# PhilipWilliamVentura/multimodal-financial-analysis-tool-using-paligemma

Hardware: AMD Instinct MI355X
Metric: decode tokens/sec per GPU + prefill ms (224px img + 32-tok prompt), PaliGemma-3B (higher is better)
Workload: dtype bf16; 1 GPU; configs[1]: paligemma-3b-pt-224 greedy KV-cached decode, batch 1, after a 256-image-token + 32-text-token prefill; batch_per_gpu=1, global_batch=1, prompt_len=288, images_gathered=1, parallelism=replicas x1 (weights RCCL-broadcast), hipgraph=True, steps_per_graph_launch=1

## Files before the change

### include/pgmi.h

```cpp
#ifndef PGMI_H
#define PGMI_H

#include <stddef.h>
#include <stdint.h>

#ifdef __cplusplus
extern "C" {
#endif

#define PGMI_OK 0
#define PGMI_E_ARG -1
#define PGMI_E_STATE -2
#define PGMI_E_HIP -3
#define PGMI_E_NOMEM -4

#define PGMI_DTYPE_BF16 0
#define PGMI_DTYPE_F16 1
#define PGMI_DTYPE_F32 2

typedef struct pgmi_ctx pgmi_ctx;

typedef struct pgmi_config {
    int v_hidden, v_intermediate, v_layers, v_heads, v_channels, v_image, v_patch;
    float v_ln_eps;
    int t_vocab, t_hidden, t_intermediate, t_layers, t_heads, t_kv_heads, t_head_dim, t_max_pos;
    float t_rms_eps, t_rope_theta;
    int projection_dim;
    int64_t image_token_index;
    int64_t pad_token_id;
    int max_batch;
    int max_seq;
    int max_kv;
} pgmi_config;

const char* pgmi_last_error(void);
const char* pgmi_version(void);

int pgmi_create(int device, const pgmi_config* cfg, pgmi_ctx** out);
int pgmi_destroy(pgmi_ctx* ctx);

int64_t pgmi_weights_bytes(const pgmi_ctx* ctx);
int pgmi_weight_count(const pgmi_ctx* ctx);
int pgmi_weight_info(const pgmi_ctx* ctx, int idx, const char** name, int64_t* offset_bytes, int64_t* shape4,
                     int* ndim);
int pgmi_bind_weights(pgmi_ctx* ctx, void* dev_slab);
int pgmi_load_weight(pgmi_ctx* ctx, const char* name, const void* src, int src_dtype, int src_on_device,
                     void* stream);
int pgmi_load_safetensors(pgmi_ctx* ctx, const char* path, int* n_loaded, int* n_skipped, void* stream);
int pgmi_safetensors_count(const char* path, int* n);
int pgmi_safetensors_entry(const char* path, int i, char* name, int name_cap, int* dtype, int64_t* shape4, int* ndim,
                           int64_t* begin, int64_t* end);
int pgmi_fill_synthetic(pgmi_ctx* ctx, const char* name, uint64_t key, float scale, float offset, void* stream);
uint64_t pgmi_synthetic_key(const char* name, uint64_t seed);
int pgmi_set_rope_inv_freq(pgmi_ctx* ctx, const float* inv_freq);
int pgmi_set_rope_table(pgmi_ctx* ctx, const uint16_t* cos_tab, const uint16_t* sin_tab, int max_pos);
int pgmi_prepare(pgmi_ctx* ctx);

int64_t pgmi_kv_bytes(const pgmi_ctx* ctx, int batch, int max_tokens);

int pgmi_vision(pgmi_ctx* ctx, const void* pixels, int pixel_dtype, int B, void* feats, void* stream);
int pgmi_project(pgmi_ctx* ctx, const void* feats, int rows, void* out, void* stream);
int pgmi_embed(pgmi_ctx* ctx, const int64_t* ids, int rows, void* out, void* stream);
int pgmi_lm_forward(pgmi_ctx* ctx, const int64_t* ids, const void* image_feats, int n_img_rows, const void* embeds,
                    int B, int L, const int64_t* positions, void* kv, int kv_batch, int kv_max, int kv_start,
                    float* logits, int logits_rows, void* stream);
int pgmi_decode(pgmi_ctx* ctx, const int64_t* ids, int B, void* kv, int kv_batch, int kv_max, int kv_len,
                int position, float* logits, int64_t* next_ids, int use_graph, void* stream);
int pgmi_decode_steps(pgmi_ctx* ctx, int64_t* ids, int B, void* kv, int kv_batch, int kv_max, int kv_len,
                      int position, int n_steps, float* logits, int64_t* tokens, int use_graph, void* stream);
int pgmi_lm_forward_ragged(pgmi_ctx* ctx, const int64_t* ids, const void* image_feats, int n_img_rows,
                           const void* embeds, int B, int L, const int64_t* positions, const int32_t* lens, void* kv,
                           int kv_batch, int kv_max, int kv_start, float* logits, int logits_rows, void* stream);
int pgmi_decode_ragged(pgmi_ctx* ctx, const int64_t* ids, int B, void* kv, int kv_batch, int kv_max,
                       const int32_t* kv_lens, const int32_t* positions, int n_steps, float* logits, int64_t* next_ids,
                       int64_t* tokens, int use_graph, void* stream);
int pgmi_decode_embeds(pgmi_ctx* ctx, const void* embeds, int B, void* kv, int kv_batch, int kv_max, int kv_len,
                       int position, float* logits, int64_t* next_ids, int use_graph, void* stream);
int pgmi_decode_embeds_dev(pgmi_ctx* ctx, const void* embeds, int B, void* kv, int kv_batch, int kv_max, int kv_len,
                           const void* position, int position_dtype, const void* mask, int mask_dtype,
                           int64_t mask_b_stride, float* logits, int64_t* next_ids, int use_graph, void* stream);
int pgmi_set_prefill_graph(pgmi_ctx* ctx, int on);
#define PGMI_GRAPH_CACHE_MAX 64
int pgmi_graph_count(const pgmi_ctx* ctx, int which);
int pgmi_set_decode_staged_norm(pgmi_ctx* ctx, int on);
int pgmi_lm_head(pgmi_ctx* ctx, const void* normed, int rows, float* logits, void* stream);
int pgmi_lm_logprobs(pgmi_ctx* ctx, const void* normed, int rows, const int64_t* labels, int64_t ignore_index,
                     float* logprob, float* lse, void* stream);
int pgmi_logprobs(pgmi_ctx* ctx, const float* logits, int rows, int V, const int64_t* ids, int64_t ignore_index,
                  float* logprob, float* lse, void* stream);
int pgmi_lm_final_hidden(pgmi_ctx* ctx, void* out, int rows, void* stream);

#define PGMI_COMM_ID_BYTES 128
int pgmi_comm_unique_id(void* id_out);
int pgmi_comm_init(int device, int nranks, int rank, const void* id, void** comm_out);
int pgmi_comm_destroy(void* comm);
int pgmi_broadcast_weights(pgmi_ctx* ctx, void* comm, int root, void* stream);

int pgmi_argmax(pgmi_ctx* ctx, const float* logits, int rows, int V, int64_t* out, void* stream);

int pgmi_eos_update(pgmi_ctx* ctx, int64_t* next_ids, int32_t* finished, int B, int64_t eos_id, int64_t pad_id,
                    int32_t* n_alive, void* stream);

int pgmi_decode_kernel(pgmi_ctx* ctx, int which, int layer, int B, void* stream);

int pgmi_preprocess(pgmi_ctx* ctx, const void* src_hwc, int H, int W, int out_h, int out_w, float* out_chw,
                    void* stream);

int pgmi_prefill_kernel(pgmi_ctx* ctx, int which, int layer, int rows, void* stream);

int pgmi_prefill_probe(pgmi_ctx* ctx, int on);
int pgmi_prefill_probe_times(pgmi_ctx* ctx, float* us, int n);
int pgmi_tune_gemm(int cfg, int split);
int pgmi_tune_gemm_shape(int M, int N, int K, int dual, int cfg, int split);

int pgmi_debug_gemm_tiles(int n_mt, int n_nt, int S, int BM, int BN, int K, int* mt, int* nt, int* z);
int pgmi_debug_gemm_plan(int M, int N, int K, int dual, int* cfg, int* bm, int* bn, int* split);

int pgmi_tune_attention(int variant);

int pgmi_sample_top_p(pgmi_ctx* ctx, const float* x, int rows, int V, float temperature, float top_p,
                      const float* u, int64_t* out, float* kept_mass, void* stream);

int pgmi_op_gemm(pgmi_ctx* ctx, const void* A, const void* W, int M, int N, int K, int epi, const void* bias,
                 const void* res, void* out, void* stream);
int pgmi_op_lm_logprobs(pgmi_ctx* ctx, const void* normed, const void* W, int rows, int V, int K,
                        const int64_t* labels, int64_t ignore_index, float* logprob, float* lse, void* stream);
int pgmi_op_gemm_strided(pgmi_ctx* ctx, const void* A, int lda, const void* W, int ldw, int M, int N, int K, int epi,
                         const void* bias, const void* res, void* out, void* stream);
int pgmi_op_rmsnorm(pgmi_ctx* ctx, const void* x, const void* w, int rows, int D, float eps, void* out,
                    void* stream);
int pgmi_op_layernorm(pgmi_ctx* ctx, const void* x, const void* w, const void* b, int rows, int D, float eps,
                      void* out, void* stream);
int pgmi_op_add(pgmi_ctx* ctx, const void* a, const void* b, int64_t n, void* out, void* stream);
int pgmi_op_patch_embed(pgmi_ctx* ctx, const void* pixels, int pixel_dtype, int B, int C, int H, int P,
                        const void* conv_w, const void* conv_b, const void* pos, int D, void* out, void* stream);
int pgmi_op_attention(pgmi_ctx* ctx, const void* q, const void* k, const void* v, void* o, int B, int Lq, int Lk,
                      int H, int Hkv, int head_dim, float scale, void* stream);
int pgmi_op_attention_ex(pgmi_ctx* ctx, const void* q, const void* k, const void* v, void* o, int B, int Lq, int Lk,
                         int H, int Hkv, int head_dim, int kv_layout, float scale, int scale_div, const void* mask,
                         int mask_dtype, int64_t m_b_stride, int64_t m_h_stride, int64_t m_q_stride, void* probs,
                         void* stream);
int pgmi_op_rope(pgmi_ctx* ctx, const void* x, const void* cos_rows, const void* sin_rows, int64_t rows, int heads,
                 int head_dim, void* out, void* stream);
int pgmi_op_scale(pgmi_ctx* ctx, const void* x, float a, int64_t n, void* out, void* stream);
int pgmi_op_gemv_res(pgmi_ctx* ctx, const void* x, const void* W, int B, int N, int K, void* h_inout,
                     void* stream);

#ifdef __cplusplus
}
#endif
#endif
```

### multimodal-financial-analysis-tool-using-paligemma_amd/csrc/engine.hip

```cpp
#include <algorithm>
#include <cmath>
#include <cstdio>
#include <cstdlib>
#include <cstring>
#include <map>
#include <string>
#include <unordered_map>
#include <vector>

#include <dlfcn.h>

#include <rccl/rccl.h>

#include "../../include/pgmi.h"
#include "common.h"
#include "launch.h"
#include "safetensors_hdr.h"

using namespace pgmi;

static thread_local std::string g_err;

constexpr int kPrefillGroup = 8;

static int fail(int code, const std::string& msg) {
    g_err = msg;
    return code;
}

#define HIPCHK(expr)                                                                       \
    do {                                                                                   \
        hipError_t e_ = (expr);                                                            \
        if (e_ != hipSuccess) return fail(PGMI_E_HIP, std::string(#expr) + ": " + hipGetErrorString(e_)); \
    } while (0)

static int launcher_error() {
    const char* what = "";
    const hipError_t e = pgmi::launch_error_take(&what);
    if (e == hipSuccess) return 0;
    return fail(PGMI_E_HIP, std::string("kernel launch: ") + what + ": " + hipGetErrorString(e));
}

#define LAUNCHCHK()                                                                        \
    do {                                                                                   \
        if (int r_ = launcher_error()) return r_;                                          \
        hipError_t e_ = hipGetLastError();                                                 \
        if (e_ != hipSuccess) return fail(PGMI_E_HIP, std::string("kernel launch: ") + hipGetErrorString(e_)); \
    } while (0)

struct Slot {
    std::string name;
    int64_t off;
    int64_t shape[4];
    int ndim;
    int64_t numel;
};

struct GraphCache {
    std::map<std::vector<intptr_t>, hipGraphExec_t> map;
    void clear() {
        for (auto& kv : map)
            if (kv.second) (void)hipGraphExecDestroy(kv.second);
        map.clear();
    }
};

struct VisionLayerW {
    const uint16_t *qkv_w, *qkv_b, *out_w, *out_b, *ln1_w, *ln1_b, *fc1_w, *fc1_b, *fc2_w, *fc2_b, *ln2_w, *ln2_b;
};
struct TextLayerW {
    const uint16_t *qkv, *o, *gate_up, *down, *in_norm, *post_norm;
    const uint16_t *mf_gate_up = nullptr, *mf_qkv = nullptr, *mf_o = nullptr, *mf_down = nullptr;
};
struct WeightTable {
    const uint16_t *patch_conv_w, *patch_b, *pos_emb, *post_ln_w, *post_ln_b, *proj_w, *proj_b, *embed, *final_norm;
    std::vector<VisionLayerW> v;
    std::vector<TextLayerW> t;
};

struct pgmi_ctx {
    pgmi_config c;
    int device;
    std::vector<Slot> slots;
    std::unordered_map<std::string, int> index;
    int64_t slab_bytes = 0;
    uint8_t* slab = nullptr;
    WeightTable w;
    std::vector<float> inv_freq;
    std::vector<uint16_t> host_cos, host_sin;
    bool prepared = false;
    std::vector<void*> allocs;
    uint16_t* patch_w = nullptr;
    int kpad = 0;
    uint16_t* cosT = nullptr;
    uint16_t* sinT = nullptr;
    uint16_t *Hs, *Tn, *QKV, *Qr, *AO, *ACT, *lastrows;
    long tn_rows = 0;
    int64_t* dpos;
    int64_t* dids_tmp;
    uint16_t *vX, *vT, *vQKV, *vAO, *vH, *vP;
    float* ws;
    size_t ws_bytes;
    uint16_t *dH, *dQ, *dAO, *dACT;
    uint16_t* dHn;
    float* dSS;
    uint16_t* mfw = nullptr;
    bool mfw_dirty = false;
    float *opart, *pmax, *dlogits, *amax_v;
    int *pidx, *amax_i;
    int max_chunks;
    StepState* step;
    StepState* pstep;
    StepState* rstep;
    int* d_rlens;
    int64_t* d_ids;
    uint16_t* d_emb;
    float* d_mask;
    float* d_zero;
    int64_t* d_next;
    unsigned* lm_done;
    hipStream_t cap_stream = nullptr;
    GraphCache pgraphs, dgraphs;
    bool prefill_graph = true;
    int mf_staged = -1;
    bool step_known = false;
    int step_kv = 0, step_pos = 0;
    bool rstep_known = false;
    int rstep_B = 0;
    int rstep_kv[kMaxRows] = {0}, rstep_pos[kMaxRows] = {0};
    std::vector<hipEvent_t> probe_ev;
    bool probe_on = false;
    bool graph_before_probe = true;
};

namespace {

int n_img(const pgmi_config& c) { return (c.v_image / c.v_patch) * (c.v_image / c.v_patch); }

void add_slot(pgmi_ctx* x, const std::string& name, std::initializer_list<int64_t> shape) {
    Slot s;
    s.name = name;
    s.ndim = (int)shape.size();
    s.numel = 1;
    int i = 0;
    for (int64_t d : shape) { s.shape[i++] = d; s.numel *= d; }
    for (; i < 4; ++i) s.shape[i] = 1;
    s.off = x->slab_bytes;
    x->slab_bytes += (s.numel * 2 + 255) / 256 * 256;
    x->index[name] = (int)x->slots.size();
    x->slots.push_back(s);
}

void build_layout(pgmi_ctx* x) {
    const pgmi_config& c = x->c;
    const int64_t D = c.v_hidden, I = c.v_intermediate, P = c.v_patch, C = c.v_channels, N = n_img(c);
    const std::string vp = "vision_tower.vision_model.";
    add_slot(x, vp + "embeddings.patch_embedding.weight", {D, C, P, P});
    add_slot(x, vp + "embeddings.patch_embedding.bias", {D});
    add_slot(x, vp + "embeddings.position_embedding.weight", {N, D});
    for (int i = 0; i < c.v_layers; ++i) {
        const std::string lp = vp + "encoder.layers." + std::to_string(i) + ".";
        for (const char* nm : {"q_proj", "k_proj", "v_proj"}) add_slot(x, lp + "self_attn." + nm + ".weight", {D, D});
        for (const char* nm : {"q_proj", "k_proj", "v_proj"}) add_slot(x, lp + "self_attn." + nm + ".bias", {D});
        add_slot(x, lp + "self_attn.out_proj.weight", {D, D});
        add_slot(x, lp + "self_attn.out_proj.bias", {D});
        add_slot(x, lp + "layer_norm1.weight", {D});
        add_slot(x, lp + "layer_norm1.bias", {D});
        add_slot(x, lp + "mlp.fc1.weight", {I, D});
        add_slot(x, lp + "mlp.fc1.bias", {I});
        add_slot(x, lp + "mlp.fc2.weight", {D, I});
        add_slot(x, lp + "mlp.fc2.bias", {D});
        add_slot(x, lp + "layer_norm2.weight", {D});
        add_slot(x, lp + "layer_norm2.bias", {D});
    }
    add_slot(x, vp + "post_layernorm.weight", {D});
    add_slot(x, vp + "post_layernorm.bias", {D});
    add_slot(x, "multi_modal_projector.linear.weight", {c.projection_dim, D});
    add_slot(x, "multi_modal_projector.linear.bias", {c.projection_dim});
    const int64_t H = c.t_hidden, TI = c.t_intermediate, V = c.t_vocab, HD = c.t_head_dim;
    add_slot(x, "language_model.model.embed_tokens.weight", {V, H});
    for (int i = 0; i < c.t_layers; ++i) {
        const std::string lp = "language_model.model.layers." + std::to_string(i) + ".";
        add_slot(x, lp + "self_attn.q_proj.weight", {c.t_heads * HD, H});
        add_slot(x, lp + "self_attn.k_proj.weight", {c.t_kv_heads * HD, H});
        add_slot(x, lp + "self_attn.v_proj.weight", {c.t_kv_heads * HD, H});
        add_slot(x, lp + "self_attn.o_proj.weight", {H, c.t_heads * HD});
        add_slot(x, lp + "mlp.gate_proj.weight", {TI, H});
        add_slot(x, lp + "mlp.up_proj.weight", {TI, H});
        add_slot(x, lp + "mlp.down_proj.weight", {H, TI});
        add_slot(x, lp + "input_layernorm.weight", {H});
        add_slot(x, lp + "post_attention_layernorm.weight", {H});
    }
    add_slot(x, "language_model.model.norm.weight", {H});
}

int bind_tables(pgmi_ctx* x) {
    std::string missing;
    auto W = [&](const std::string& name) -> const uint16_t* {
        auto it = x->index.find(name);
        if (it == x->index.end()) {
            if (missing.empty()) missing = name;
            return nullptr;
        }
        return reinterpret_cast<const uint16_t*>(x->slab + x->slots[it->second].off);
    };
    WeightTable& w = x->w;
    const std::string vp = "vision_tower.vision_model.", tp = "language_model.model.";
    w.patch_conv_w = W(vp + "embeddings.patch_embedding.weight");
    w.patch_b = W(vp + "embeddings.patch_embedding.bias");
    w.pos_emb = W(vp + "embeddings.position_embedding.weight");
    w.post_ln_w = W(vp + "post_layernorm.weight");
    w.post_ln_b = W(vp + "post_layernorm.bias");
    w.proj_w = W("multi_modal_projector.linear.weight");
    w.proj_b = W("multi_modal_projector.linear.bias");
    w.embed = W(tp + "embed_tokens.weight");
    w.final_norm = W(tp + "norm.weight");
    w.v.resize(x->c.v_layers);
    for (int i = 0; i < x->c.v_layers; ++i) {
        const std::string lp = vp + "encoder.layers." + std::to_string(i) + ".";
        w.v[i] = {W(lp + "self_attn.q_proj.weight"), W(lp + "self_attn.q_proj.bias"),
                  W(lp + "self_attn.out_proj.weight"), W(lp + "self_attn.out_proj.bias"),
                  W(lp + "layer_norm1.weight"), W(lp + "layer_norm1.bias"), W(lp + "mlp.fc1.weight"),
                  W(lp + "mlp.fc1.bias"), W(lp + "mlp.fc2.weight"), W(lp + "mlp.fc2.bias"),
                  W(lp + "layer_norm2.weight"), W(lp + "layer_norm2.bias")};
    }
    w.t.resize(x->c.t_layers);
    for (int i = 0; i < x->c.t_layers; ++i) {
        const std::string lp = tp + "layers." + std::to_string(i) + ".";
        TextLayerW& t = w.t[i];
        t.qkv = W(lp + "self_attn.q_proj.weight");
        t.o = W(lp + "self_attn.o_proj.weight");
        t.gate_up = W(lp + "mlp.gate_proj.weight");
        t.down = W(lp + "mlp.down_proj.weight");
        t.in_norm = W(lp + "input_layernorm.weight");
        t.post_norm = W(lp + "post_attention_layernorm.weight");
    }
    if (!missing.empty()) return fail(PGMI_E_STATE, "weight layout has no tensor named " + missing);
    return 0;
}

uint16_t host_f2bf(float f) {
    uint32_t u;
    std::memcpy(&u, &f, 4);
    u += 0x7FFFu + ((u >> 16) & 1u);
    return (uint16_t)(u >> 16);
}

float bf16_round_host(float f) {
    uint32_t u = (uint32_t)host_f2bf(f) << 16;
    float r;
    std::memcpy(&r, &u, 4);
    return r;
}

uint64_t fnv1a(const char* s) {
    uint64_t h = 0xCBF29CE484222325ULL;
    for (const unsigned char* p = (const unsigned char*)s; *p; ++p) { h ^= *p; h *= 0x100000001B3ULL; }
    return h;
}

uint64_t splitmix64_h(uint64_t x) {
    x += 0x9E3779B97F4A7C15ULL;
    x = (x ^ (x >> 30)) * 0xBF58476D1CE4E5B9ULL;
    x = (x ^ (x >> 27)) * 0x94D049BB133111EBULL;
    return x ^ (x >> 31);
}

__global__ void k_convert(const void* src, int dtype, long n, uint16_t* dst) {
    for (long i = blockIdx.x * (long)blockDim.x + threadIdx.x; i < n; i += (long)gridDim.x * blockDim.x) {
        if (dtype == PGMI_DTYPE_F32) dst[i] = f2bf(reinterpret_cast<const float*>(src)[i]);
        else dst[i] = f2bf((float)reinterpret_cast<const _Float16*>(src)[i]);
    }
}

int dalloc(pgmi_ctx* x, void** p, size_t bytes) {
    if (bytes == 0) bytes = 256;
    hipError_t e = hipMalloc(p, bytes);
    if (e != hipSuccess) return fail(PGMI_E_NOMEM, std::string("hipMalloc ") + std::to_string(bytes) + ": " + hipGetErrorString(e));
    x->allocs.push_back(*p);
    return 0;
}

template <typename T>
int dalloc_t(pgmi_ctx* x, T** p, size_t count) {
    return dalloc(x, reinterpret_cast<void**>(p), count * sizeof(T));
}

void build_rope_host(pgmi_ctx* x, std::vector<uint16_t>& cs, std::vector<uint16_t>& sn) {
    const int half = x->c.t_head_dim / 2, mp = x->c.t_max_pos;
    cs.resize((size_t)mp * half);
    sn.resize((size_t)mp * half);
    for (int p = 0; p < mp; ++p)
        for (int i = 0; i < half; ++i) {
            const float ang = (float)p * x->inv_freq[i];
            cs[(size_t)p * half + i] = host_f2bf((float)std::cos((double)ang));
            sn[(size_t)p * half + i] = host_f2bf((float)std::sin((double)ang));
        }
}

int ensure_prepared(pgmi_ctx* x) {
    (void)pgmi::launch_error_take(nullptr);
    if (!x->prepared) return fail(PGMI_E_STATE, "pgmi_prepare() has not been called");
    if (!x->slab) return fail(PGMI_E_STATE, "weights are not bound (pgmi_bind_weights)");
    return 0;
}

template <class F>
int run_graphed(pgmi_ctx* x, GraphCache& gc, hipStream_t s, const std::vector<intptr_t>& key, F body,
                bool sync_before_capture) {
    auto it = gc.map.find(key);
    if (it == gc.map.end()) {
        if (gc.map.size() >= PGMI_GRAPH_CACHE_MAX) gc.clear();
        gc.map[key] = nullptr;
        return body(s);
    }
    if (it->second) {
        HIPCHK(hipGraphLaunch(it->second, s));
        return 0;
    }
    hipGraph_t g = nullptr;
    hipGraphExec_t exec = nullptr;
    int rc = 0;
    hipError_t e = sync_before_capture ? hipStreamSynchronize(s) : hipSuccess;
    if (e == hipSuccess && (e = hipStreamBeginCapture(x->cap_stream, hipStreamCaptureModeThreadLocal)) == hipSuccess) {
        rc = body(x->cap_stream);
        const hipError_t end = hipStreamEndCapture(x->cap_stream, &g);
        if (rc == 0) e = end;
    }
    if (rc == 0 && e == hipSuccess) e = hipGraphInstantiate(&exec, g, nullptr, nullptr, 0);
    if (g) (void)hipGraphDestroy(g);
    if (rc == 0 && e == hipSuccess) e = hipGraphLaunch(exec, s);
    if (rc == 0 && e == hipSuccess) {
        gc.map[key] = exec;
        return 0;
    }
    if (exec) (void)hipGraphExecDestroy(exec);
    gc.map.erase(key);
    return rc ? rc : fail(PGMI_E_HIP, std::string("hipGraph capture: ") + hipGetErrorString(e));
}

template <class F>
int run_prefill(pgmi_ctx* x, hipStream_t s, const std::vector<intptr_t>& key, F body) {
    if (!x->prefill_graph) return body(s);
    return run_graphed(x, x->pgraphs, s, key, body, false);
}

}

namespace {
struct Rccl {
    void* h = nullptr;
    std::string why;
    ncclResult_t (*get_unique_id)(ncclUniqueId*) = nullptr;
    ncclResult_t (*comm_init_rank)(ncclComm_t*, int, ncclUniqueId, int) = nullptr;
    ncclResult_t (*comm_destroy)(ncclComm_t) = nullptr;
    ncclResult_t (*broadcast)(const void*, void*, size_t, ncclDataType_t, int, ncclComm_t, hipStream_t) = nullptr;
    const char* (*error_string)(ncclResult_t) = nullptr;
};

Rccl& rccl() {
    static Rccl r = [] {
        Rccl t;
        for (const char* n : {"librccl.so.1", "librccl.so", "/opt/rocm/lib/librccl.so.1"}) {
            if ((t.h = dlopen(n, RTLD_NOW | RTLD_LOCAL))) break;
            const char* e = dlerror();
            if (e) t.why = e;
        }
        if (t.h) {
            t.get_unique_id = reinterpret_cast<decltype(t.get_unique_id)>(dlsym(t.h, "ncclGetUniqueId"));
            t.comm_init_rank = reinterpret_cast<decltype(t.comm_init_rank)>(dlsym(t.h, "ncclCommInitRank"));
            t.comm_destroy = reinterpret_cast<decltype(t.comm_destroy)>(dlsym(t.h, "ncclCommDestroy"));
            t.broadcast = reinterpret_cast<decltype(t.broadcast)>(dlsym(t.h, "ncclBroadcast"));
            t.error_string = reinterpret_cast<decltype(t.error_string)>(dlsym(t.h, "ncclGetErrorString"));
        }
        return t;
    }();
    return r;
}
}

extern "C" {

const char* pgmi_last_error(void) { return g_err.c_str(); }
const char* pgmi_version(void) { return "pgmi 0.1.0 (gfx950)"; }

int pgmi_create(int device, const pgmi_config* cfg, pgmi_ctx** out) {
    if (!cfg || !out) return fail(PGMI_E_ARG, "null argument");
    const pgmi_config& c = *cfg;
    if (c.t_head_dim != 256) return fail(PGMI_E_ARG, "head_dim must be 256 (Gemma)");
    if (c.t_hidden != 2048) return fail(PGMI_E_ARG, "text hidden must be 2048 (decode kernels are specialised)");
    if (c.t_intermediate % 8 != 0 || c.v_intermediate % 8 != 0) return fail(PGMI_E_ARG, "intermediate sizes must be multiples of 8");
    if (c.v_hidden % c.v_heads != 0 || c.v_hidden / c.v_heads != 72) return fail(PGMI_E_ARG, "SigLIP head_dim must be 72");
    if (c.t_kv_heads != 1 || c.t_heads > 8)
        return fail(PGMI_E_ARG, "decode path is specialised for MQA with <= 8 query heads (num_key_value_heads = 1)");
    if (c.max_batch < 1 || c.max_batch > kMaxRows) return fail(PGMI_E_ARG, "max_batch must be in [1, 16]");
    if (c.v_hidden > 4096) return fail(PGMI_E_ARG, "v_hidden too large for the LayerNorm kernel");
    auto* x = new pgmi_ctx();
    x->c = c;
    if (x->c.max_kv <= 0) x->c.max_kv = c.t_max_pos;
    x->device = device;
    build_layout(x);
    x->inv_freq.resize(c.t_head_dim / 2);
    for (int i = 0; i < c.t_head_dim / 2; ++i) {
        const float e = (float)(2 * i) / (float)c.t_head_dim;
        const float p = (float)std::pow((double)c.t_rope_theta, (double)e);
        x->inv_freq[i] = 1.0f / p;
    }
    *out = x;
    return 0;
}

int pgmi_destroy(pgmi_ctx* x) {
    if (!x) return 0;
    for (auto& e : x->probe_ev) (void)hipEventDestroy(e);
    x->dgraphs.clear();
    x->pgraphs.clear();
    for (void* p : x->allocs) (void)hipFree(p);
    if (x->cap_stream) (void)hipStreamDestroy(x->cap_stream);
    delete x;
    return 0;
}

int64_t pgmi_weights_bytes(const pgmi_ctx* x) { return x ? x->slab_bytes : -1; }
int pgmi_weight_count(const pgmi_ctx* x) { return x ? (int)x->slots.size() : -1; }

int pgmi_weight_info(const pgmi_ctx* x, int idx, const char** name, int64_t* off, int64_t* shape4, int* ndim) {
    if (!x || idx < 0 || idx >= (int)x->slots.size()) return fail(PGMI_E_ARG, "weight index out of range");
    const Slot& s = x->slots[idx];
    if (name) *name = s.name.c_str();
    if (off) *off = s.off;
    if (shape4) for (int i = 0; i < 4; ++i) shape4[i] = s.shape[i];
    if (ndim) *ndim = s.ndim;
    return 0;
}

int pgmi_bind_weights(pgmi_ctx* x, void* slab) {
    if (!x || !slab) return fail(PGMI_E_ARG, "null argument");
    if (reinterpret_cast<uintptr_t>(slab) % 256 != 0) return fail(PGMI_E_ARG, "weight slab must be 256-byte aligned");
    x->slab = reinterpret_cast<uint8_t*>(slab);
    x->dgraphs.clear();
    x->pgraphs.clear();
    return bind_tables(x);
}

int pgmi_load_weight(pgmi_ctx* x, const char* name, const void* src, int dtype, int on_device, void* stream) {
    if (!x || !name || !src) return fail(PGMI_E_ARG, "null argument");
    if (!x->slab) return fail(PGMI_E_STATE, "weights are not bound");
    auto it = x->index.find(name);
    if (it == x->index.end()) return fail(PGMI_E_ARG, std::string("unknown weight ") + name);
    const Slot& s = x->slots[it->second];
    uint16_t* dst = reinterpret_cast<uint16_t*>(x->slab + s.off);
    hipStream_t st = (hipStream_t)stream;
    HIPCHK(hipSetDevice(x->device));
    if (dtype == PGMI_DTYPE_BF16) {
        HIPCHK(hipMemcpyAsync(dst, src, s.numel * 2, on_device ? hipMemcpyDeviceToDevice : hipMemcpyHostToDevice, st));
    } else if (dtype == PGMI_DTYPE_F32 || dtype == PGMI_DTYPE_F16) {
        if (on_device) {
            hipLaunchKernelGGL(k_convert, dim3(1024), dim3(256), 0, st, src, dtype, (long)s.numel, dst);
            LAUNCHCHK();
        } else {
            std::vector<uint16_t> tmp(s.numel);
            for (int64_t i = 0; i < s.numel; ++i) {
                float f = dtype == PGMI_DTYPE_F32 ? reinterpret_cast<const float*>(src)[i]
                                                 : (float)reinterpret_cast<const _Float16*>(src)[i];
                tmp[i] = host_f2bf(f);
            }
            HIPCHK(hipMemcpyAsync(dst, tmp.data(), s.numel * 2, hipMemcpyHostToDevice, st));
            HIPCHK(hipStreamSynchronize(st));
        }
    } else {
        return fail(PGMI_E_ARG, "unsupported dtype");
    }
    return 0;
}

int pgmi_safetensors_count(const char* path, int* n) {
    if (!path || !n) return fail(PGMI_E_ARG, "null argument");
    StFile f;
    if (!st_open(path, f)) return fail(PGMI_E_ARG, f.error);
    *n = (int)f.entries.size();
    return 0;
}

int pgmi_safetensors_entry(const char* path, int i, char* name, int name_cap, int* dtype, int64_t* shape4, int* ndim,
                           int64_t* begin, int64_t* end) {
    if (!path || !name || name_cap < 1 || !dtype || !shape4 || !ndim || !begin || !end)
        return fail(PGMI_E_ARG, "null argument");
    StFile f;
    if (!st_open(path, f)) return fail(PGMI_E_ARG, f.error);
    if (i < 0 || i >= (int)f.entries.size()) return fail(PGMI_E_ARG, "entry index out of range");
    const StEntry& e = f.entries[i];
    std::snprintf(name, (size_t)name_cap, "%s", e.name.c_str());
    *dtype = e.dtype == "BF16" ? PGMI_DTYPE_BF16 : e.dtype == "F16" ? PGMI_DTYPE_F16 : e.dtype == "F32" ? PGMI_DTYPE_F32 : -1;
    *ndim = (int)e.shape.size();
    for (int d = 0; d < 4; ++d) shape4[d] = d < *ndim ? e.shape[d] : 0;
    *begin = e.begin;
    *end = e.end;
    return 0;
}

int pgmi_load_safetensors(pgmi_ctx* x, const char* path, int* n_loaded, int* n_skipped, void* stream) {
    if (!x || !path) return fail(PGMI_E_ARG, "null argument");
    if (!x->slab) return fail(PGMI_E_STATE, "weights are not bound");
    HIPCHK(hipSetDevice(x->device));
    StFile f;
    if (!st_open(path, f)) return fail(PGMI_E_ARG, f.error);
    hipStream_t st = (hipStream_t)stream;
    void* tmp = nullptr;
    size_t tmp_bytes = 0;
    uint8_t* scratch = reinterpret_cast<uint8_t*>(x->ws);
    size_t scratch_bytes = x->ws ? x->ws_bytes : 0;
    int loaded = 0, skipped = 0;
    int rc = 0;
    for (const StEntry& e : f.entries) {
        auto it = x->index.find(e.name);
        if (it == x->index.end()) {
            ++skipped;
            continue;
        }
        const Slot& sl = x->slots[it->second];
        bool same = (int)e.shape.size() == sl.ndim;
        for (int d = 0; same && d < sl.ndim; ++d) same = e.shape[d] == sl.shape[d];
        if (!same) {
            rc = fail(PGMI_E_ARG, "shape mismatch for " + e.name);
            break;
        }
        const int eb = st_elem_bytes(e.dtype);
        if (eb == 0) {
            rc = fail(PGMI_E_ARG, "unsupported dtype " + e.dtype + " for " + e.name);
            break;
        }
        if (e.end - e.begin != sl.numel * eb) {
            rc = fail(PGMI_E_ARG, "byte size mismatch for " + e.name);
            break;
        }
        const uint8_t* src = f.map + f.data0 + e.begin;
        uint16_t* dst = reinterpret_cast<uint16_t*>(x->slab + sl.off);
        if (e.dtype == "BF16") {
            if (hipMemcpyAsync(dst, src, (size_t)sl.numel * 2, hipMemcpyHostToDevice, st) != hipSuccess) {
                rc = fail(PGMI_E_HIP, "upload of " + e.name);
                break;
            }
        } else {
            const int dt = e.dtype == "F32" ? PGMI_DTYPE_F32 : PGMI_DTYPE_F16;
            if (scratch_bytes < ((size_t)8 << 20)) {
                if (!tmp) {
                    tmp_bytes = (size_t)64 << 20;
                    if (hipMalloc(&tmp, tmp_bytes) != hipSuccess) {
                        rc = fail(PGMI_E_NOMEM, "conversion scratch");
                        break;
                    }
                }
                scratch = reinterpret_cast<uint8_t*>(tmp);
                scratch_bytes = tmp_bytes;
            }
            const int64_t per = (int64_t)(scratch_bytes / (size_t)eb);
            for (int64_t i0 = 0; i0 < sl.numel && rc == 0; i0 += per) {
                const int64_t n = std::min<int64_t>(per, sl.numel - i0);
                if (hipMemcpyAsync(scratch, src + i0 * eb, (size_t)n * eb, hipMemcpyHostToDevice, st) != hipSuccess) {
                    rc = fail(PGMI_E_HIP, "upload of " + e.name);
                    break;
                }
                hipLaunchKernelGGL(k_convert, dim3(1024), dim3(256), 0, st, scratch, dt, (long)n, dst + i0);
            }
            if (rc) break;
        }
        ++loaded;
    }
    const hipError_t se = hipStreamSynchronize(st);
    if (tmp) (void)hipFree(tmp);
    if (rc) return rc;
    if (se != hipSuccess) return fail(PGMI_E_HIP, std::string("safetensors upload: ") + hipGetErrorString(se));
    x->prepared = false;
    if (n_loaded) *n_loaded = loaded;
    if (n_skipped) *n_skipped = skipped;
    return 0;
}

uint64_t pgmi_synthetic_key(const char* name, uint64_t seed) { return splitmix64_h(seed ^ fnv1a(name)); }

int pgmi_fill_synthetic(pgmi_ctx* x, const char* name, uint64_t key, float scale, float offset, void* stream) {
    if (!x || !name) return fail(PGMI_E_ARG, "null argument");
    if (!x->slab) return fail(PGMI_E_STATE, "weights are not bound");
    auto it = x->index.find(name);
    if (it == x->index.end()) return fail(PGMI_E_ARG, std::string("unknown weight ") + name);
    const Slot& s = x->slots[it->second];
    HIPCHK(hipSetDevice(x->device));
    fill_synthetic((hipStream_t)stream, reinterpret_cast<uint16_t*>(x->slab + s.off), (long)s.numel, key, scale, offset);
    LAUNCHCHK();
    return 0;
}

int pgmi_set_rope_inv_freq(pgmi_ctx* x, const float* inv) {
    if (!x || !inv) return fail(PGMI_E_ARG, "null argument");
    for (int i = 0; i < x->c.t_head_dim / 2; ++i) x->inv_freq[i] = inv[i];
    x->host_cos.clear();
    x->host_sin.clear();
    x->prepared = false;
    return 0;
}

int pgmi_set_rope_table(pgmi_ctx* x, const uint16_t* cs, const uint16_t* sn, int max_pos) {
    if (!x || !cs || !sn) return fail(PGMI_E_ARG, "null argument");
    if (max_pos != x->c.t_max_pos) return fail(PGMI_E_ARG, "rope table must cover max_position_embeddings");
    const size_t n = (size_t)max_pos * (x->c.t_head_dim / 2);
    x->host_cos.assign(cs, cs + n);
    x->host_sin.assign(sn, sn + n);
    x->prepared = false;
    return 0;
}

int pgmi_prepare(pgmi_ctx* x) {
    if (!x) return fail(PGMI_E_ARG, "null argument");
    if (!x->slab) return fail(PGMI_E_STATE, "weights are not bound");
    HIPCHK(hipSetDevice(x->device));
    const pgmi_config& c = x->c;
    int rc;
    if (!x->cosT) {
        const int N = n_img(c);
        const size_t R = (size_t)c.max_batch * c.max_seq, RG = (size_t)std::min(c.max_batch, kPrefillGroup) * c.max_seq,
                     RV = (size_t)std::min(c.max_batch, kPrefillGroup) * N;
        const int H = c.t_hidden, QKVN = (c.t_heads + 2 * c.t_kv_heads) * c.t_head_dim;
        x->kpad = (c.v_channels * c.v_patch * c.v_patch + 63) / 64 * 64;
        if ((rc = dalloc_t(x, &x->patch_w, (size_t)c.v_hidden * x->kpad))) return rc;
        if ((rc = dalloc_t(x, &x->cosT, (size_t)c.t_max_pos * c.t_head_dim / 2))) return rc;
        if ((rc = dalloc_t(x, &x->sinT, (size_t)c.t_max_pos * c.t_head_dim / 2))) return rc;
        if ((rc = dalloc_t(x, &x->Hs, R * H))) return rc;
        if ((rc = dalloc_t(x, &x->Tn, R * H))) return rc;
        if ((rc = dalloc_t(x, &x->QKV, RG * QKVN))) return rc;
        if ((rc = dalloc_t(x, &x->Qr, RG * c.t_heads * c.t_head_dim))) return rc;
        if ((rc = dalloc_t(x, &x->AO, RG * H))) return rc;
        if ((rc = dalloc_t(x, &x->ACT, RG * c.t_intermediate))) return rc;
        if ((rc = dalloc_t(x, &x->lastrows, (size_t)c.max_batch * H))) return rc;
        if ((rc = dalloc_t(x, &x->dpos, R))) return rc;
        if ((rc = dalloc_t(x, &x->dids_tmp, R))) return rc;
        if ((rc = dalloc_t(x, &x->vX, RV * c.v_hidden))) return rc;
        if ((rc = dalloc_t(x, &x->vT, RV * c.v_hidden))) return rc;
        if ((rc = dalloc_t(x, &x->vQKV, RV * 3 * c.v_hidden))) return rc;
        if ((rc = dalloc_t(x, &x->vAO, RV * c.v_hidden))) return rc;
        if ((rc = dalloc_t(x, &x->vH, RV * c.v_intermediate))) return rc;
        if ((rc = dalloc_t(x, &x->vP, RV * x->kpad))) return rc;
        x->ws_bytes = (size_t)64 << 20;
        if ((rc = dalloc(x, reinterpret_cast<void**>(&x->ws), x->ws_bytes))) return rc;
        const int B = c.max_batch;
        if ((rc = dalloc_t(x, &x->dH, (size_t)B * H))) return rc;
        if ((rc = dalloc_t(x, &x->dQ, (size_t)B * c.t_heads * c.t_head_dim))) return rc;
        if ((rc = dalloc_t(x, &x->dAO, (size_t)B * H))) return rc;
        if ((rc = dalloc_t(x, &x->dACT, (size_t)B * c.t_intermediate))) return rc;
        if ((rc = dalloc_t(x, &x->dHn, (size_t)B * H))) return rc;
        if ((rc = dalloc_t(x, &x->dSS, (size_t)B * (H / 16)))) return rc;
        x->max_chunks = (c.max_kv + 63) / 64;
        if ((rc = dalloc_t(x, &x->opart, attention_decode_part_floats(B, c.t_kv_heads, x->max_chunks)))) return rc;
        if ((rc = dalloc_t(x, &x->pmax, (size_t)B * gemv_logits_blocks()))) return rc;
        if ((rc = dalloc_t(x, &x->dlogits, (size_t)B * c.t_vocab))) return rc;
        if ((rc = dalloc_t(x, &x->pidx, (size_t)B * gemv_logits_blocks()))) return rc;
        if ((rc = dalloc_t(x, &x->step, 1))) return rc;
        if ((rc = dalloc_t(x, &x->pstep, 1))) return rc;
        if ((rc = dalloc_t(x, &x->rstep, kMaxRows))) return rc;
        if ((rc = dalloc_t(x, &x->d_rlens, 2 * kMaxRows))) return rc;
        if ((rc = dalloc_t(x, &x->amax_v, (size_t)argmax_scratch_parts()))) return rc;
        if ((rc = dalloc_t(x, &x->amax_i, (size_t)argmax_scratch_parts()))) return rc;
        if ((rc = dalloc_t(x, &x->d_ids, (size_t)B))) return rc;
        if ((rc = dalloc_t(x, &x->d_emb, (size_t)B * H))) return rc;
        if ((rc = dalloc_t(x, &x->d_mask, (size_t)B * c.max_kv))) return rc;
        if ((rc = dalloc_t(x, &x->d_zero, 64))) return rc;
        HIPCHK(hipMemset(x->d_zero, 0, 64 * sizeof(float)));
        if ((rc = dalloc_t(x, &x->d_next, (size_t)B))) return rc;
        if ((rc = dalloc_t(x, &x->lm_done, 33 * 32))) return rc;
        HIPCHK(hipMemset(x->lm_done, 0, 33 * 32 * sizeof(unsigned)));
        HIPCHK(hipStreamCreateWithFlags(&x->cap_stream, hipStreamNonBlocking));
    }
    pad_rows(nullptr, x->w.patch_conv_w, c.v_hidden, c.v_channels * c.v_patch * c.v_patch, x->kpad, x->patch_w);
    LAUNCHCHK();
    x->mfw_dirty = c.max_batch >= gemv_mf_min_batch() && c.t_intermediate % 32 == 0 && c.t_hidden % 32 == 0;
    std::vector<uint16_t> cs, sn;
    if (!x->host_cos.empty()) {
        cs = x->host_cos;
        sn = x->host_sin;
    } else {
        build_rope_host(x, cs, sn);
    }
    HIPCHK(hipMemcpy(x->cosT, cs.data(), cs.size() * 2, hipMemcpyHostToDevice));
    HIPCHK(hipMemcpy(x->sinT, sn.data(), sn.size() * 2, hipMemcpyHostToDevice));
    HIPCHK(hipDeviceSynchronize());
    x->dgraphs.clear();
    x->pgraphs.clear();
    x->prepared = true;
    return 0;
}

int64_t pgmi_kv_bytes(const pgmi_ctx* x, int batch, int max_tokens) {
    if (!x) return -1;
    return (int64_t)x->c.t_layers * 2 * batch * max_tokens * x->c.t_kv_heads * x->c.t_head_dim * 2;
}

int pgmi_graph_count(const pgmi_ctx* x, int which) {
    if (!x) return -1;
    return (int)(which == 0 ? x->pgraphs : x->dgraphs).map.size();
}

static int vision_body(pgmi_ctx* x, hipStream_t s, const void* pixels, int dtype, int B, void* feats);

int pgmi_vision(pgmi_ctx* x, const void* pixels, int dtype, int B, void* feats, void* stream) {
    int rc;
    if ((rc = ensure_prepared(x))) return rc;
    const pgmi_config& c = x->c;
    if (B < 1 || B > c.max_batch) return fail(PGMI_E_ARG, "batch exceeds max_batch");
    if (!pixels || !feats) return fail(PGMI_E_ARG, "null argument");
    const std::vector<intptr_t> key{1, (intptr_t)pixels, dtype, B, (intptr_t)feats};
    const size_t px_img = (size_t)c.v_channels * c.v_image * c.v_image * (dtype == PGMI_DTYPE_F32 ? 4 : 2);
    const size_t ft_img = (size_t)n_img(c) * c.v_hidden * sizeof(uint16_t);
    rc = run_prefill(x, (hipStream_t)stream, key, [&](hipStream_t st) {
        for (int b0 = 0; b0 < B; b0 += kPrefillGroup) {
            const int r = vision_body(x, st, reinterpret_cast<const char*>(pixels) + b0 * px_img, dtype,
                                      std::min(kPrefillGroup, B - b0), reinterpret_cast<char*>(feats) + b0 * ft_img);
            if (r) return r;
        }
        return 0;
    });
    if (rc) return rc;
    LAUNCHCHK();
    return 0;
}

static int vision_body(pgmi_ctx* x, hipStream_t s, const void* pixels, int dtype, int B, void* feats) {
    const pgmi_config& c = x->c;
    const WeightTable& w = x->w;
    const int N = n_img(c), D = c.v_hidden, Iv = c.v_intermediate, rows = B * N;
    const float eps = c.v_ln_eps;
    patchify(s, pixels, dtype == PGMI_DTYPE_F32, B, c.v_channels, c.v_image, c.v_image, c.v_patch, x->kpad, x->vP);
    EpiArgs e{};
    e.bias = w.patch_b;
    e.pos = w.pos_emb;
    e.npos = N;
    e.out = x->vX;
    e.ldo = D;
    gemm(s, x->vP, x->kpad, x->patch_w, x->kpad, rows, D, x->kpad, EPI_BIAS_POS, e, x->ws, x->ws_bytes);
    const float scale = (float)std::pow((double)(D / c.v_heads), -0.5);
    if (c.v_layers > 0) layernorm(s, x->vX, w.v[0].ln1_w, w.v[0].ln1_b, eps, x->vT, rows, D);
    for (int i = 0; i < c.v_layers; ++i) {
        const bool last = i + 1 == c.v_layers;
        const VisionLayerW& l = w.v[i];
        EpiArgs q{};
        q.bias = l.qkv_b;
        q.out = x->vQKV;
        q.ldo = 3 * D;
        gemm(s, x->vT, D, l.qkv_w, D, rows, 3 * D, D, EPI_BIAS, q, x->ws, x->ws_bytes);
        AttnArgs a{};
        a.q = x->vQKV; a.q_b_stride = (long)N * 3 * D; a.q_row_stride = 3 * D; a.q_head_stride = 72;
        a.k = x->vQKV + D; a.k_b_stride = a.q_b_stride; a.k_row_stride = 3 * D; a.k_head_stride = 72;
        a.v = x->vQKV + 2 * D; a.v_b_stride = a.q_b_stride; a.v_row_stride = 3 * D; a.v_head_stride = 72;
        a.o = x->vAO; a.o_b_stride = (long)N * D; a.o_row_stride = D; a.o_head_stride = 72;
        a.Lq = N; a.Lk = N; a.G = 1; a.n_kv = c.v_heads; a.B = B; a.scale = scale;
        a.ws = x->ws; a.ws_floats = (long)(x->ws_bytes / sizeof(float));
        attention_prefill(s, 72, a);
        EpiArgs o{};
        o.bias = l.out_b;
        o.res = x->vX; o.ldr = D; o.out = x->vX; o.ldo = D;
        const int spo = gemm(s, x->vAO, D, l.out_w, D, rows, D, D, EPI_BIAS_RES, o, x->ws, x->ws_bytes, 0, true);
        splitk_res_norm(s, x->ws, spo, o.bias, x->vX, l.ln2_w, l.ln2_b, eps, x->vT, rows, D);
        EpiArgs f1{};
        f1.bias = l.fc1_b; f1.out = x->vH; f1.ldo = Iv;
        gemm(s, x->vT, D, l.fc1_w, D, rows, Iv, D, EPI_BIAS_GELU, f1, x->ws, x->ws_bytes);
        EpiArgs f2{};
        f2.bias = l.fc2_b; f2.res = x->vX; f2.ldr = D; f2.out = x->vX; f2.ldo = D;
        const int sp = gemm(s, x->vH, Iv, l.fc2_w, Iv, rows, D, Iv, EPI_BIAS_RES, f2, x->ws, x->ws_bytes, 0, true);
        splitk_res_norm(s, x->ws, sp, f2.bias, x->vX, last ? w.post_ln_w : w.v[i + 1].ln1_w,
                        last ? w.post_ln_b : w.v[i + 1].ln1_b, eps, last ? reinterpret_cast<uint16_t*>(feats) : x->vT,
                        rows, D);
    }
    if (c.v_layers == 0)
        layernorm(s, x->vX, w.post_ln_w, w.post_ln_b, eps, reinterpret_cast<uint16_t*>(feats), rows, D);
    LAUNCHCHK();
    return 0;
}

int pgmi_project(pgmi_ctx* x, const void* feats, int rows, void* out, void* stream) {
    int rc;
    if ((rc = ensure_prepared(x))) return rc;
    if (!feats || !out || rows < 1) return fail(PGMI_E_ARG, "bad argument");
    if (rows > x->c.max_batch * n_img(x->c)) return fail(PGMI_E_ARG, "rows exceed workspace capacity");
    EpiArgs e{};
    e.bias = x->w.proj_b;
    e.out = reinterpret_cast<uint16_t*>(out);
    e.ldo = x->c.projection_dim;
    const int grp = kPrefillGroup * n_img(x->c);
    for (int r0 = 0; r0 < rows; r0 += grp) {
        e.out = reinterpret_cast<uint16_t*>(out) + (size_t)r0 * x->c.projection_dim;
        gemm((hipStream_t)stream, reinterpret_cast<const uint16_t*>(feats) + (size_t)r0 * x->c.v_hidden, x->c.v_hidden,
             x->w.proj_w, x->c.v_hidden, std::min(grp, rows - r0), x->c.projection_dim, x->c.v_hidden, EPI_BIAS, e, x->ws,
             x->ws_bytes);
    }
    LAUNCHCHK();
    return 0;
}

int pgmi_embed(pgmi_ctx* x, const int64_t* ids, int rows, void* out, void* stream) {
    int rc;
    if ((rc = ensure_prepared(x))) return rc;
    if (!ids || !out) return fail(PGMI_E_ARG, "null argument");
    embed_rows((hipStream_t)stream, ids, rows, x->w.embed, x->c.t_hidden, 1.0f, INT64_MIN,
               reinterpret_cast<uint16_t*>(out));
    LAUNCHCHK();
    return 0;
}

static int lm_body(pgmi_ctx* x, hipStream_t s, const int64_t* ids, const void* image_feats, int n_img_rows,
                   const void* embeds, int B, int L, void* kv, int kv_batch, int kv_max, int kv_start, float* logits,
                   int logits_rows, bool ragged);
static int lm_rows(pgmi_ctx* x, hipStream_t s, int b0, int B, int L, void* kv, int kv_batch, int kv_max, int kv_start,
                   float* logits, int logits_rows, bool ragged);

static int lm_forward(pgmi_ctx* x, const int64_t* ids, const void* image_feats, int n_img_rows, const void* embeds,
                      int B, int L, const int64_t* positions, const int32_t* lens, bool ragged, void* kv, int kv_batch,
                      int kv_max, int kv_start, float* logits, int logits_rows, void* stream);

int pgmi_lm_forward(pgmi_ctx* x, const int64_t* ids, const void* image_feats, int n_img_rows, const void* embeds,
                    int B, int L, const int64_t* positions, void* kv, int kv_batch, int kv_max, int kv_start,
                    float* logits, int logits_rows, void* stream) {
    return lm_forward(x, ids, image_feats, n_img_rows, embeds, B, L, positions, nullptr, false, kv, kv_batch, kv_max,
                      kv_start, logits, logits_rows, stream);
}

int pgmi_lm_forward_ragged(pgmi_ctx* x, const int64_t* ids, const void* image_feats, int n_img_rows,
                           const void* embeds, int B, int L, const int64_t* positions, const int32_t* lens, void* kv,
                           int kv_batch, int kv_max, int kv_start, float* logits, int logits_rows, void* stream) {
    if (!lens) return fail(PGMI_E_ARG, "null argument");
    return lm_forward(x, ids, image_feats, n_img_rows, embeds, B, L, positions, lens, true, kv, kv_batch, kv_max,
                      kv_start, logits, logits_rows, stream);
}

static int lm_forward(pgmi_ctx* x, const int64_t* ids, const void* image_feats, int n_img_rows, const void* embeds,
                      int B, int L, const int64_t* positions, const int32_t* lens, bool ragged, void* kv, int kv_batch,
                      int kv_max, int kv_start, float* logits, int logits_rows, void* stream) {
    int rc;
    if ((rc = ensure_prepared(x))) return rc;
    const pgmi_config& c = x->c;
    if (B < 1 || B > c.max_batch || B > kv_batch) return fail(PGMI_E_ARG, "batch exceeds capacity");
    if (L < 1 || L > c.max_seq) return fail(PGMI_E_ARG, "sequence length exceeds max_seq");
    if (kv_start < 0 || kv_start + L > kv_max) return fail(PGMI_E_ARG, "KV cache capacity exceeded");
    if (!positions || !kv || !logits || (!embeds && !ids)) return fail(PGMI_E_ARG, "null argument");
    if (logits_rows < 0 || logits_rows > 2) return fail(PGMI_E_ARG, "logits_rows must be 0, 1 or 2");
    if (ragged) {
        if (embeds || !ids) return fail(PGMI_E_ARG, "ragged prefill takes token ids (pad slots enter as zero rows)");
        RowInts rl{}, rk{};
        for (int b = 0; b < B; ++b) {
            if (lens[b] < 1 || lens[b] > L) return fail(PGMI_E_ARG, "lens[b] must be in [1, L]");
            rl.v[b] = lens[b];
            rk.v[b] = kv_start + lens[b];
        }
        set_row_ints((hipStream_t)stream, x->d_rlens, rl, rk, B);
        LAUNCHCHK();
        if (logits_rows == 2) logits_rows = 1;
    }
    HIPCHK(hipMemcpyAsync(x->dpos, positions, (size_t)B * L * sizeof(int64_t), hipMemcpyHostToDevice,
                          (hipStream_t)stream));
    x->tn_rows = 0;
    const std::vector<intptr_t> key{2, (intptr_t)ids, (intptr_t)image_feats, n_img_rows, (intptr_t)embeds, B, L,
                                    (intptr_t)kv, kv_batch, kv_max, kv_start, (intptr_t)logits, logits_rows,
                                    (intptr_t)ragged};
    rc = run_prefill(x, (hipStream_t)stream, key, [&](hipStream_t st) {
        return lm_body(x, st, ids, image_feats, n_img_rows, embeds, B, L, kv, kv_batch, kv_max, kv_start, logits,
                       logits_rows, ragged);
    });
    if (rc) return rc;
    x->tn_rows = logits_rows == 2 && L > 1 ? 0 : (long)B * L;
    LAUNCHCHK();
    return 0;
}

static int lm_body(pgmi_ctx* x, hipStream_t s, const int64_t* ids, const void* image_feats, int n_img_rows,
                   const void* embeds, int B, int L, void* kv, int kv_batch, int kv_max, int kv_start, float* logits,
                   int logits_rows, bool ragged) {
    const pgmi_config& c = x->c;
    const int* rlens = ragged ? x->d_rlens : nullptr;
    const int H = c.t_hidden, R = B * L;
    const float normalizer = bf16_round_host(std::sqrt((float)H));
    const uint16_t* E = x->w.embed;
    if (embeds) {
        scale_rows(s, reinterpret_cast<const uint16_t*>(embeds), (long)R * H, normalizer, x->Hs);
    } else {
        merge_embed(s, ids, B, L, E, H, reinterpret_cast<const uint16_t*>(image_feats), image_feats ? n_img_rows : 0,
                    c.image_token_index, c.pad_token_id, (float)std::sqrt((double)H), normalizer, nullptr,
                    reinterpret_cast<int*>(x->dids_tmp), x->Hs, rlens);
    }
    for (int b0 = 0; b0 < B; b0 += kPrefillGroup) {
        const int r = lm_rows(x, s, b0, std::min(kPrefillGroup, B - b0), L, kv, kv_batch, kv_max, kv_start, logits,
                              logits_rows, ragged);
        if (r) return r;
    }
    return 0;
}

static int lm_rows(pgmi_ctx* x, hipStream_t s, int b0, int B, int L, void* kv, int kv_batch, int kv_max, int kv_start,
                   float* logits, int logits_rows, bool ragged) {
    const pgmi_config& c = x->c;
    const int* rlens = ragged ? x->d_rlens + b0 : nullptr;
    const int* rkeys = ragged ? x->d_rlens + kMaxRows + b0 : nullptr;
    const int H = c.t_hidden, R = B * L, NH = c.t_heads, NKV = c.t_kv_heads, HD = c.t_head_dim;
    const int QKVN = (NH + 2 * NKV) * HD;
    const float eps = c.t_rms_eps;
    const uint16_t* E = x->w.embed;
    uint16_t* const Hs = x->Hs + (size_t)b0 * L * H;
    uint16_t* const Tn = x->Tn + (size_t)b0 * L * H;
    uint16_t* const lastrows = x->lastrows + (size_t)b0 * H;
    const int64_t* const dpos = x->dpos + (size_t)b0 * L;
    logits += (size_t)b0 * (logits_rows == 0 ? L : 1) * c.t_vocab;
    const long kvd = (long)NKV * HD, kvb = (long)kv_max * kvd;
    uint16_t* kvp = reinterpret_cast<uint16_t*>(kv) + (long)b0 * kvb;
    const uint16_t* fnorm = x->w.final_norm;
    const bool last_only = logits_rows == 2 && L > 1 && c.t_layers > 0;
    rmsnorm(s, Hs, c.t_layers ? x->w.t[0].in_norm : fnorm, eps, Tn, R, H);
    for (int i = 0; i < c.t_layers; ++i) {
        const TextLayerW& w = x->w.t[i];
        uint16_t* Kc = kvp + ((long)(i * 2 + 0) * kv_batch) * kvb;
        uint16_t* Vc = kvp + ((long)(i * 2 + 1) * kv_batch) * kvb;
        EpiArgs q{};
        q.out = x->QKV; q.ldo = QKVN;
        q.rpos = dpos; q.cosT = x->cosT; q.sinT = x->sinT; q.max_pos = c.t_max_pos;
        q.q_out = x->Qr; q.kc = Kc; q.vc = Vc; q.kv_b_stride = kvb; q.kv_start = kv_start;
        q.L = L; q.nh = NH; q.nkv = NKV;
        if (HD != 256 || !gemm_qkv_rope(s, Tn, H, w.qkv, H, R, QKVN, H, q)) {
            int sp = gemm(s, Tn, H, w.qkv, H, R, QKVN, H, EPI_STORE, q, x->ws, x->ws_bytes, 0, true);
            rope_kv_append(s, x->QKV, x->ws, sp, B, L, NH, NKV, dpos, x->cosT, x->sinT, c.t_max_pos, x->Qr, Kc, Vc,
                           kvb, kv_start);
        }
        AttnArgs a{};
        a.q = x->Qr; a.q_b_stride = (long)L * NH * HD; a.q_row_stride = NH * HD; a.q_head_stride = HD;
        a.k = Kc; a.k_b_stride = kvb; a.k_row_stride = (int)kvd; a.k_head_stride = HD;
        a.v = Vc; a.v_b_stride = kvb; a.v_row_stride = (int)kvd; a.v_head_stride = HD;
        a.o = x->AO; a.o_b_stride = (long)L * H; a.o_row_stride = H; a.o_head_stride = HD;
        a.Lq = L; a.Lk = kv_start + L; a.G = NH / NKV; a.n_kv = NKV; a.B = B;
        a.scale = 1.0f / std::sqrt((float)HD);
        a.ws = x->ws; a.ws_floats = (long)(x->ws_bytes / sizeof(float));
        a.klen = rkeys;
        if (last_only && i + 1 == c.t_layers) {
            a.q = x->Qr + (size_t)(L - 1) * NH * HD;
            a.o = x->dAO; a.o_b_stride = (long)H;
            a.Lq = 1;
            HIPCHK(hipMemcpy2DAsync(lastrows, (size_t)H * 2, Hs + (size_t)(L - 1) * H, (size_t)L * H * 2,
                                    (size_t)H * 2, B, hipMemcpyDeviceToDevice, s));
            if (kv_start + L <= c.max_kv) {
                a.Lk = 0;
                HIPCHK(hipMemsetD32Async(reinterpret_cast<hipDeviceptr_t>(&x->pstep->kv_len), kv_start + L - 1, 1, s));
                a.mask = x->d_zero; a.mask_b_stride = 0; a.mask_k_stride = 0; a.mask_round = 1;
                attention_decode(s, a, x->pstep, kv_start + L, x->opart, x->max_chunks);
                gemv_o_attn(s, B, NH, x->opart, x->max_chunks, x->pstep, w.o, H, lastrows,
                            B >= gemv_mf_min_batch() ? x->dAO : nullptr);
            } else {
                attention_prefill(s, 256, a);
                gemv_res(s, B, NH * HD, x->dAO, w.o, H, lastrows, x->ws);
            }
            gemv_geglu(s, B, lastrows, w.post_norm, eps, w.gate_up, c.t_intermediate, x->dACT);
            gemv_res(s, B, c.t_intermediate, x->dACT, w.down, H, lastrows, x->ws);
            break;
        }
        attention_prefill(s, 256, a);
        EpiArgs o{};
        o.res = Hs; o.ldr = H; o.out = Hs; o.ldo = H;
        int sp = gemm(s, x->AO, H, w.o, H, R, H, NH * HD, EPI_RES, o, x->ws, x->ws_bytes, 0, true);
        splitk_res_norm(s, x->ws, sp, nullptr, Hs, w.post_norm, nullptr, eps, Tn, R, H);
        EpiArgs g{};
        g.out = x->ACT; g.ldo = c.t_intermediate;
        const bool probe = x->probe_on && (size_t)(4 * i + 3) < x->probe_ev.size();
        if (probe) gemm_probe_events(x->probe_ev[4 * i], x->probe_ev[4 * i + 1]);
        gemm(s, Tn, H, w.gate_up, H, R, c.t_intermediate, H, EPI_GEGLU, g, x->ws, x->ws_bytes, c.t_intermediate);
        EpiArgs d{};
        d.res = Hs; d.ldr = H; d.out = Hs; d.ldo = H;
        if (probe) gemm_probe_events(x->probe_ev[4 * i + 2], x->probe_ev[4 * i + 3]);
        sp = gemm(s, x->ACT, c.t_intermediate, w.down, c.t_intermediate, R, H, c.t_intermediate, EPI_RES, d, x->ws,
                  x->ws_bytes, 0, true);
        const bool last = i + 1 == c.t_layers;
        splitk_res_norm(s, x->ws, sp, nullptr, Hs, last ? fnorm : x->w.t[i + 1].in_norm, nullptr, eps, Tn, R, H);
    }
    if (logits_rows == 0) {
        EpiArgs l{};
        l.out_f32 = logits; l.ldo = c.t_vocab;
        gemm(s, Tn, H, E, H, R, c.t_vocab, H, EPI_F32, l, x->ws, x->ws_bytes);
    } else {
        if (ragged)
            gather_last_rows(s, Hs, B, L, H, rlens, lastrows);
        else if (!last_only)
            HIPCHK(hipMemcpy2DAsync(lastrows, (size_t)H * 2, Hs + (size_t)(L - 1) * H, (size_t)L * H * 2,
                                    (size_t)H * 2, B, hipMemcpyDeviceToDevice, s));
        int nparts = 0;
        gemv_logits(s, B, lastrows, fnorm, eps, E, c.t_vocab, logits, x->pmax, x->pidx, &nparts);
    }
    LAUNCHCHK();
    return 0;
}

static bool mf_staged(const pgmi_ctx* x) { return x->mf_staged > 0; }

static int decode_body(pgmi_ctx* x, hipStream_t s, const int64_t* ids, int B, void* kv, int kv_batch, int kv_max,
                       int launch_keys, float* logits, int64_t* next_ids, const uint16_t* embeds = nullptr,
                       int masked = 0, int64_t* hist = nullptr, bool ragged = false) {
    const pgmi_config& c = x->c;
    StepState* const st = ragged ? x->rstep : x->step;
    const int sts = ragged ? 1 : 0, adv_n = ragged ? B : 1;
    const int H = c.t_hidden, NH = c.t_heads, NKV = c.t_kv_heads, HD = c.t_head_dim;
    const float eps = c.t_rms_eps;
    const float normalizer = bf16_round_host(std::sqrt((float)H));
    const uint16_t* E = x->w.embed;
    const long kvd = (long)NKV * HD, kvb = (long)kv_max * kvd;
    uint16_t* kvp = reinterpret_cast<uint16_t*>(kv);
    const bool fold = !embeds && gemv_qkv_folds_embed(B) && c.t_layers > 0;
    const EmbedFold emb{ids, E, normalizer, c.pad_token_id, x->dH};
    if (embeds) scale_rows(s, embeds, (long)B * H, normalizer, x->dH);
    else if (!fold) embed_rows(s, ids, B, E, H, normalizer, c.pad_token_id, x->dH);
    const bool mf = B >= gemv_mf_min_batch() && !mf_staged(x);
    if (mf && c.t_layers > 0) rows_norm(s, x->dH, x->w.t[0].in_norm, eps, B, H, x->dHn);
    for (int i = 0; i < c.t_layers; ++i) {
        uint16_t* Kc = kvp + ((long)(i * 2 + 0) * kv_batch) * kvb;
        uint16_t* Vc = kvp + ((long)(i * 2 + 1) * kv_batch) * kvb;
        const TextLayerW& w = x->w.t[i];
        gemv_qkv(s, B, NH, NKV, mf ? x->dHn : x->dH, mf ? nullptr : w.in_norm, eps, w.qkv, x->cosT, x->sinT,
                 c.t_max_pos, st, x->dQ, Kc, Vc, kvb, x->ws, (fold && i == 0) ? &emb : nullptr, w.mf_qkv, sts);
        AttnArgs a{};
        a.q = x->dQ; a.q_b_stride = (long)NH * HD; a.q_row_stride = NH * HD; a.q_head_stride = HD;
        a.k = Kc; a.k_b_stride = kvb; a.k_row_stride = (int)kvd; a.k_head_stride = HD;
        a.v = Vc; a.v_b_stride = kvb; a.v_row_stride = (int)kvd; a.v_head_stride = HD;
        a.o = x->dAO; a.o_b_stride = (long)H; a.o_row_stride = H; a.o_head_stride = HD;
        a.Lq = 1; a.Lk = 0; a.G = NH / NKV; a.n_kv = NKV; a.B = B; a.scale = 1.0f / std::sqrt((float)HD);
        if (masked) {
            a.mask = x->d_mask; a.mask_b_stride = c.max_kv; a.mask_k_stride = 1; a.mask_round = masked == 1;
        } else {
            a.mask = x->d_zero; a.mask_b_stride = 0; a.mask_k_stride = 0; a.mask_round = 1;
        }
        attention_decode(s, a, st, launch_keys, x->opart, x->max_chunks, sts);
        gemv_o_attn(s, B, NH, x->opart, x->max_chunks, st, w.o, H, x->dH, B >= gemv_mf_min_batch() ? x->dAO : nullptr,
                    mf ? x->dSS : nullptr, w.mf_o, sts);
        if (mf) {
            gemv_geglu(s, B, x->dH, w.post_norm, eps, w.gate_up, c.t_intermediate, x->dACT, x->dSS, w.mf_gate_up);
            gemv_res_norm(s, B, c.t_intermediate, x->dACT, w.down, H, x->dH, x->ws,
                          i + 1 < c.t_layers ? x->w.t[i + 1].in_norm : nullptr, eps, x->dHn, w.mf_down);
            continue;
        }
        gemv_geglu(s, B, x->dH, w.post_norm, eps, w.gate_up, c.t_intermediate, x->dACT);
        gemv_res(s, B, c.t_intermediate, x->dACT, w.down, H, x->dH, x->ws);
    }
    int nparts = 0;
    int64_t* nx = next_ids ? next_ids : x->d_next;
    if (!gemv_logits(s, B, x->dH, x->w.final_norm, eps, E, c.t_vocab, logits, x->pmax, x->pidx, &nparts, x->lm_done, nx,
                     st, hist, adv_n))
        argmax_finish(s, B, x->pmax, x->pidx, nparts, nx, st, hist, adv_n);
    return launcher_error();
}

int pgmi_prefill_probe(pgmi_ctx* x, int on) {
    if (!x) return fail(PGMI_E_ARG, "null context");
    if (on && x->probe_ev.empty()) {
        x->probe_ev.resize((size_t)4 * x->c.t_layers);
        for (auto& e : x->probe_ev) HIPCHK(hipEventCreate(&e));
    }
    if (on && !x->probe_on) x->graph_before_probe = x->prefill_graph;
    if (!on && x->probe_on) x->prefill_graph = x->graph_before_probe;
    x->probe_on = on != 0;
    if (x->probe_on) x->prefill_graph = false;
    x->pgraphs.clear();
    return 0;
}

int pgmi_prefill_probe_times(pgmi_ctx* x, float* us, int n) {
    if (!x || !us) return fail(PGMI_E_ARG, "null argument");
    if (x->probe_ev.empty()) return fail(PGMI_E_STATE, "pgmi_prefill_probe(ctx, 1) has not been called");
    const int L = x->c.t_layers;
    if (n < 2 * L) return fail(PGMI_E_ARG, "us needs 2 x layers entries");
    HIPCHK(hipEventSynchronize(x->probe_ev.back()));
    for (int i = 0; i < L; ++i) {
        float a = 0.f, b = 0.f;
        HIPCHK(hipEventElapsedTime(&a, x->probe_ev[4 * i], x->probe_ev[4 * i + 1]));
        HIPCHK(hipEventElapsedTime(&b, x->probe_ev[4 * i + 2], x->probe_ev[4 * i + 3]));
        us[i] = a * 1e3f;
        us[L + i] = b * 1e3f;
    }
    return 0;
}

int pgmi_set_decode_staged_norm(pgmi_ctx* x, int on) {
    if (!x) return fail(PGMI_E_ARG, "null context");
    x->mf_staged = on < 0 ? -1 : on != 0;
    x->dgraphs.clear();
    return 0;
}

int pgmi_set_prefill_graph(pgmi_ctx* x, int on) {
    if (!x) return fail(PGMI_E_ARG, "null context");
    if (x->probe_on) x->graph_before_probe = on != 0;
    else x->prefill_graph = on != 0;
    x->pgraphs.clear();
    return 0;
}

struct DevStepIn {
    const void* pos = nullptr;
    int pos_dtype = 0;
    const void* mask = nullptr;
    int mask_dtype = 0;
    long mask_b_stride = 0;
};

static int ensure_mf_image(pgmi_ctx* x, hipStream_t s) {
    if (!x->mfw_dirty) return 0;
    const pgmi_config& c = x->c;
    const size_t I = c.t_intermediate, H = c.t_hidden, QKVN = (size_t)(c.t_heads + 2 * c.t_kv_heads) * c.t_head_dim,
                 OK = (size_t)c.t_heads * c.t_head_dim, per = 2 * I * H + QKVN * H + H * OK + H * I;
    x->mfw_dirty = false;
    if (!x->mfw) {
        void* p = nullptr;
        if (hipMalloc(&p, per * c.t_layers * sizeof(uint16_t)) != hipSuccess) {
            (void)hipGetLastError();
            return 0;
        }
        x->allocs.push_back(p);
        x->mfw = reinterpret_cast<uint16_t*>(p);
        x->dgraphs.clear();
    }
    for (int i = 0; i < c.t_layers; ++i) {
        TextLayerW& w = x->w.t[i];
        uint16_t *gu = x->mfw + per * i, *qkv = gu + 2 * I * H, *o = qkv + QKVN * H, *down = o + H * OK;
        mf_swizzle(s, w.gate_up, (int)(2 * I), (int)H, gu);
        mf_swizzle(s, w.qkv, (int)QKVN, (int)H, qkv, true);
        mf_swizzle(s, w.o, (int)H, (int)OK, o);
        mf_swizzle(s, w.down, (int)H, (int)I, down);
        w.mf_gate_up = gu; w.mf_qkv = qkv; w.mf_o = o; w.mf_down = down;
    }
    LAUNCHCHK();
    return 0;
}

static int decode_step(pgmi_ctx* x, const int64_t* ids, const void* embeds, int B, void* kv, int kv_batch, int kv_max,
                       int kv_len, int position, float* logits, int64_t* next_ids, int use_graph, void* stream,
                       const DevStepIn* dev = nullptr, int n_steps = 1, int64_t* tokens = nullptr,
                       const int32_t* r_kv = nullptr, const int32_t* r_pos = nullptr) {
    int rc;
    const bool ragged = r_kv != nullptr;
    if ((rc = ensure_prepared(x))) return rc;
    const pgmi_config& c = x->c;
    if (B < 1 || B > c.max_batch || B > kv_batch) return fail(PGMI_E_ARG, "batch exceeds capacity");
    if (n_steps < 1) return fail(PGMI_E_ARG, "n_steps must be >= 1");
    if (n_steps > 1 && (!ids || embeds || dev)) return fail(PGMI_E_ARG, "multi-step decode: token ids only");
    if (ragged) {
        if (!r_pos) return fail(PGMI_E_ARG, "null argument");
        kv_len = 0;
        for (int b = 0; b < B; ++b) {
            if (r_kv[b] < 0 || (long)r_kv[b] + n_steps - 1 >= kv_max)
                return fail(PGMI_E_ARG, "KV cache capacity exceeded (a row's kv_lens[b] + n_steps > kv_max)");
            kv_len = std::max(kv_len, (int)r_kv[b]);
        }
    }
    if (kv_len < 0 || (long)kv_len + n_steps - 1 >= kv_max) return fail(PGMI_E_ARG, "KV cache capacity exceeded");
    if (kv_max > c.max_kv) return fail(PGMI_E_ARG, "kv_max exceeds config max_kv");
    if ((!ids && !embeds) || !kv || !logits) return fail(PGMI_E_ARG, "null argument");
    hipStream_t s = (hipStream_t)stream;
    if (B >= gemv_mf_min_batch() && (rc = ensure_mf_image(x, s))) return rc;
    int masked = 0;
    if (dev) {
        set_step_dev(s, x->step, kv_len, dev->pos, dev->pos_dtype);
        if (dev->mask) {
            stage_mask(s, dev->mask, dev->mask_dtype, B, dev->mask_b_stride, kv_len + 1, x->d_mask, c.max_kv);
            masked = dev->mask_dtype == PGMI_DTYPE_F32 ? 2 : 1;
        }
    } else if (ragged) {
        bool same = x->rstep_known && x->rstep_B == B;
        for (int b = 0; same && b < B; ++b) same = x->rstep_kv[b] == r_kv[b] && x->rstep_pos[b] == r_pos[b];
        if (!same) {
            RowInts rk{}, rp{};
            for (int b = 0; b < B; ++b) { rk.v[b] = r_kv[b]; rp.v[b] = r_pos[b]; }
            set_step_rows(s, x->rstep, rk, rp, B);
        }
    } else if (!x->step_known || x->step_kv != kv_len || x->step_pos != position) {
        set_step(s, x->step, kv_len, position);
    }
    if (ragged) x->rstep_known = false;
    else x->step_known = false;
    auto advanced = [&]() {
        if (ragged) {
            x->rstep_known = true;
            x->rstep_B = B;
            for (int b = 0; b < B; ++b) {
                x->rstep_kv[b] = r_kv[b] + n_steps;
                x->rstep_pos[b] = r_pos[b] + n_steps;
            }
            return;
        }
        x->step_known = dev == nullptr;
        x->step_kv = kv_len + n_steps;
        x->step_pos = position + n_steps;
    };
    const uint16_t* erows = nullptr;
    if (embeds) {
        HIPCHK(hipMemcpyAsync(x->d_emb, embeds, (size_t)B * c.t_hidden * 2, hipMemcpyDeviceToDevice, s));
        erows = x->d_emb;
    }
    int64_t* fb = next_ids ? next_ids : x->d_next;
    auto body = [&](hipStream_t st, const int64_t* first, int keys0, bool grow) -> int {
        for (int t = 0; t < n_steps; ++t) {
            const int r = decode_body(x, st, t == 0 ? first : fb, B, kv, kv_batch, kv_max, grow ? keys0 + t : keys0,
                                      logits, next_ids, erows, masked, tokens ? tokens + (long)t * B : nullptr,
                                      ragged);
            if (r) return r;
        }
        return 0;
    };
    if (!use_graph) {
        if ((rc = body(s, ids, kv_len + 1, true))) return rc;
        LAUNCHCHK();
        advanced();
        return 0;
    }
    const int64_t* gids = ids;
    if (!embeds && ids != next_ids) {
        HIPCHK(hipMemcpyAsync(x->d_ids, ids, (size_t)B * sizeof(int64_t), hipMemcpyDeviceToDevice, s));
        gids = x->d_ids;
    }
    if (embeds) gids = nullptr;
    const std::vector<intptr_t> key{
        B, (intptr_t)kv, kv_batch, kv_max, (intptr_t)logits, (intptr_t)next_ids,
        (intptr_t)gids,
        embeds != nullptr,
        masked,
        n_steps,
        (intptr_t)tokens,
        ragged};
    rc = run_graphed(x, x->dgraphs, s, key, [&](hipStream_t st) { return body(st, gids, kv_max, false); }, true);
    if (rc) return rc;
    LAUNCHCHK();
    advanced();
    return 0;
}

int pgmi_decode(pgmi_ctx* x, const int64_t* ids, int B, void* kv, int kv_batch, int kv_max, int kv_len, int position,
                float* logits, int64_t* next_ids, int use_graph, void* stream) {
    if (!ids) return fail(PGMI_E_ARG, "null argument");
    return decode_step(x, ids, nullptr, B, kv, kv_batch, kv_max, kv_len, position, logits, next_ids, use_graph, stream);
}

int pgmi_decode_steps(pgmi_ctx* x, int64_t* ids, int B, void* kv, int kv_batch, int kv_max, int kv_len, int position,
                      int n_steps, float* logits, int64_t* tokens, int use_graph, void* stream) {
    if (!ids) return fail(PGMI_E_ARG, "null argument");
    return decode_step(x, ids, nullptr, B, kv, kv_batch, kv_max, kv_len, position, logits, ids, use_graph, stream,
                       nullptr, n_steps, tokens);
}

int pgmi_decode_ragged(pgmi_ctx* x, const int64_t* ids, int B, void* kv, int kv_batch, int kv_max,
                       const int32_t* kv_lens, const int32_t* positions, int n_steps, float* logits, int64_t* next_ids,
                       int64_t* tokens, int use_graph, void* stream) {
    if (!ids || !kv_lens || !positions) return fail(PGMI_E_ARG, "null argument");
    if (n_steps > 1 && !next_ids) return fail(PGMI_E_ARG, "multi-step decode: next_ids carries the token fed back");
    if (x && (B < 1 || B > x->c.max_batch || B > kMaxRows)) return fail(PGMI_E_ARG, "batch exceeds capacity");
    return decode_step(x, ids, nullptr, B, kv, kv_batch, kv_max, 0, 0, logits, next_ids, use_graph, stream, nullptr,
                       n_steps, tokens, kv_lens, positions);
}

int pgmi_decode_embeds(pgmi_ctx* x, const void* embeds, int B, void* kv, int kv_batch, int kv_max, int kv_len,
                       int position, float* logits, int64_t* next_ids, int use_graph, void* stream) {
    if (!embeds) return fail(PGMI_E_ARG, "null argument");
    return decode_step(x, nullptr, embeds, B, kv, kv_batch, kv_max, kv_len, position, logits, next_ids, use_graph,
                       stream);
}

int pgmi_decode_embeds_dev(pgmi_ctx* x, const void* embeds, int B, void* kv, int kv_batch, int kv_max, int kv_len,
                           const void* position, int position_dtype, const void* mask, int mask_dtype,
                           int64_t mask_b_stride, float* logits, int64_t* next_ids, int use_graph, void* stream) {
    if (!embeds || !position) return fail(PGMI_E_ARG, "null argument");
    if (position_dtype != PGMI_DTYPE_BF16 && position_dtype != PGMI_DTYPE_F32 && position_dtype != 10 &&
        position_dtype != 11 && position_dtype != 12)
        return fail(PGMI_E_ARG, "position dtype must be bf16, fp32, fp64, int64 or int32");
    if (mask && mask_dtype != PGMI_DTYPE_BF16 && mask_dtype != PGMI_DTYPE_F32)
        return fail(PGMI_E_ARG, "mask dtype must be bf16 or fp32");
    if (B != 1) return fail(PGMI_E_ARG, "device-side positions: one sequence per step (B = 1)");
    DevStepIn d;
    d.pos = position; d.pos_dtype = position_dtype; d.mask = mask; d.mask_dtype = mask_dtype;
    d.mask_b_stride = (long)mask_b_stride;
    return decode_step(x, nullptr, embeds, B, kv, kv_batch, kv_max, kv_len, -1, logits, next_ids, use_graph, stream,
                       &d);
}

int pgmi_lm_head(pgmi_ctx* x, const void* normed, int rows, float* logits, void* stream) {
    int rc;
    if ((rc = ensure_prepared(x))) return rc;
    if (!normed || !logits) return fail(PGMI_E_ARG, "null argument");
    if (rows < 1) return fail(PGMI_E_ARG, "lm_head: no rows");
    const pgmi_config& c = x->c;
    EpiArgs l{};
    l.out_f32 = logits;
    l.ldo = c.t_vocab;
    gemm((hipStream_t)stream, reinterpret_cast<const uint16_t*>(normed), c.t_hidden, x->w.embed, c.t_hidden, rows,
         c.t_vocab, c.t_hidden, EPI_F32, l, x->ws, x->ws_bytes);
    LAUNCHCHK();
    return 0;
}

static int lm_logprobs_run(pgmi_ctx* x, const void* normed, const uint16_t* W, int rows, int V, int K,
                           const int64_t* labels, int64_t ignore_index, float* logprob, float* lse, void* stream) {
    if (!x->ws) return fail(PGMI_E_STATE, "workspace not allocated (pgmi_prepare)");
    if (V < 1 || K < 8 || K % 8 != 0) return fail(PGMI_E_ARG, "lm_logprobs: V >= 1 and K a positive multiple of 8");
    const size_t per_row = (size_t)((V + 63) / 64) * sizeof(float2) + sizeof(float);
    const int per = (int)std::min<size_t>((size_t)rows, x->ws_bytes / per_row);
    if (per < 1) return fail(PGMI_E_ARG, "lm_logprobs: vocabulary exceeds the scratch");
    float2* part = reinterpret_cast<float2*>(x->ws);
    float* lab = reinterpret_cast<float*>(reinterpret_cast<char*>(x->ws) + (size_t)per * (per_row - sizeof(float)));
    const uint16_t* A = reinterpret_cast<const uint16_t*>(normed);
    hipStream_t s = (hipStream_t)stream;
    for (int r0 = 0; r0 < rows; r0 += per) {
        const int nr = std::min(per, rows - r0);
        const int n_nt = gemm_lse_tiles(nr, V, K);
        if (n_nt < 1 || !gemm_lse(s, A + (size_t)r0 * K, K, W, K, nr, V, K, labels + r0, part, lab))
            return fail(PGMI_E_ARG, "lm_logprobs: the forced GEMM configuration has no log-sum-exp epilogue");
        lse_combine(s, part, n_nt, lab, labels + r0, nr, V, ignore_index, logprob + r0, lse ? lse + r0 : nullptr);
    }
    LAUNCHCHK();
    return 0;
}

int pgmi_lm_logprobs(pgmi_ctx* x, const void* normed, int rows, const int64_t* labels, int64_t ignore_index,
                     float* logprob, float* lse, void* stream) {
    if (!x || !normed || !labels || !logprob) return fail(PGMI_E_ARG, "null argument");
    if (rows < 1) return fail(PGMI_E_ARG, "lm_logprobs: no rows");
    int rc;
    if ((rc = ensure_prepared(x))) return rc;
    return lm_logprobs_run(x, normed, x->w.embed, rows, x->c.t_vocab, x->c.t_hidden, labels, ignore_index, logprob, lse,
                           stream);
}

int pgmi_logprobs(pgmi_ctx* x, const float* logits, int rows, int V, const int64_t* ids, int64_t ignore_index,
                  float* logprob, float* lse, void* stream) {
    if (!x || !logits || !ids || !logprob) return fail(PGMI_E_ARG, "null argument");
    if (rows < 1 || V < 1) return fail(PGMI_E_ARG, "logprobs: empty logits");
    if (!x->amax_v || !x->amax_i) return fail(PGMI_E_STATE, "logprobs scratch missing (pgmi_prepare)");
    static_assert(sizeof(float) == sizeof(int), "the argmax index scratch holds the partial sums");
    const int per = argmax_scratch_parts();
    for (int r0 = 0; r0 < rows; r0 += per)
        logprob_rows((hipStream_t)stream, logits + (size_t)r0 * V, std::min(per, rows - r0), V, ids + r0, ignore_index,
                     x->amax_v, reinterpret_cast<float*>(x->amax_i), logprob + r0, lse ? lse + r0 : nullptr);
    LAUNCHCHK();
    return 0;
}

int pgmi_lm_final_hidden(pgmi_ctx* x, void* out, int rows, void* stream) {
    int rc;
    if ((rc = ensure_prepared(x))) return rc;
    if (!out) return fail(PGMI_E_ARG, "null argument");
    if (rows < 1 || rows > x->c.max_batch * x->c.max_seq) return fail(PGMI_E_ARG, "rows exceed the prefill workspace");
    if (rows > x->tn_rows)
        return fail(PGMI_E_STATE, "the last pgmi_lm_forward did not keep these rows' final hidden states (logits_rows 2)");
    HIPCHK(hipMemcpyAsync(out, x->Tn, (size_t)rows * x->c.t_hidden * 2, hipMemcpyDeviceToDevice, (hipStream_t)stream));
    return 0;
}

#define RCCL_READY()                                                                       \
    do {                                                                                   \
        const Rccl& r_ = rccl();                                                           \
        if (!r_.get_unique_id || !r_.comm_init_rank || !r_.comm_destroy || !r_.broadcast || !r_.error_string) \
            return fail(PGMI_E_STATE, std::string("librccl could not be loaded (dlopen librccl.so.1): ") + \
                        (r_.h ? "missing nccl* symbols" : r_.why));                        \
    } while (0)

#define NCCLCHK(expr)                                                                      \
    do {                                                                                   \
        ncclResult_t r_ = (expr);                                                          \
        if (r_ != ncclSuccess) return fail(PGMI_E_HIP, std::string(#expr) + ": " + rccl().error_string(r_)); \
    } while (0)

int pgmi_comm_unique_id(void* id_out) {
    if (!id_out) return fail(PGMI_E_ARG, "null argument");
    RCCL_READY();
    static_assert(sizeof(ncclUniqueId) == PGMI_COMM_ID_BYTES, "ncclUniqueId size");
    ncclUniqueId id;
    NCCLCHK(rccl().get_unique_id(&id));
    std::memcpy(id_out, &id, sizeof(id));
    return 0;
}

int pgmi_comm_init(int device, int nranks, int rank, const void* id, void** comm_out) {
    if (!id || !comm_out) return fail(PGMI_E_ARG, "null argument");
    if (nranks < 1 || rank < 0 || rank >= nranks) return fail(PGMI_E_ARG, "bad rank / world size");
    RCCL_READY();
    int prev = 0;
    HIPCHK(hipGetDevice(&prev));
    HIPCHK(hipSetDevice(device));
    ncclUniqueId uid;
    std::memcpy(&uid, id, sizeof(uid));
    ncclComm_t comm = nullptr;
    const ncclResult_t r = rccl().comm_init_rank(&comm, nranks, uid, rank);
    HIPCHK(hipSetDevice(prev));
    if (r != ncclSuccess) return fail(PGMI_E_HIP, std::string("ncclCommInitRank: ") + rccl().error_string(r));
    *comm_out = comm;
    return 0;
}

int pgmi_comm_destroy(void* comm) {
    if (!comm) return 0;
    RCCL_READY();
    NCCLCHK(rccl().comm_destroy(reinterpret_cast<ncclComm_t>(comm)));
    return 0;
}

int pgmi_broadcast_weights(pgmi_ctx* x, void* comm, int root, void* stream) {
    if (!x || !comm) return fail(PGMI_E_ARG, "null argument");
    if (!x->slab) return fail(PGMI_E_STATE, "weights are not bound (pgmi_bind_weights)");
    RCCL_READY();
    int prev = 0;
    HIPCHK(hipGetDevice(&prev));
    HIPCHK(hipSetDevice(x->device));
    const ncclResult_t r = rccl().broadcast(x->slab, x->slab, (size_t)x->slab_bytes, ncclUint8, root,
                                            reinterpret_cast<ncclComm_t>(comm), (hipStream_t)stream);
    HIPCHK(hipSetDevice(prev));
    if (r != ncclSuccess) return fail(PGMI_E_HIP, std::string("ncclBroadcast: ") + rccl().error_string(r));
    x->prepared = false;
    return 0;
}

int pgmi_argmax(pgmi_ctx* x, const float* logits, int rows, int V, int64_t* out, void* stream) {
    if (!x || !logits || !out) return fail(PGMI_E_ARG, "null argument");
    if (rows <= 0 || V <= 0) return fail(PGMI_E_ARG, "argmax: empty logits");
    if (!x->amax_v) return fail(PGMI_E_STATE, "argmax scratch missing");
    argmax_rows((hipStream_t)stream, logits, rows, V, x->amax_v, x->amax_i, out);
    LAUNCHCHK();
    return 0;
}

int pgmi_eos_update(pgmi_ctx* x, int64_t* next_ids, int32_t* finished, int B, int64_t eos_id, int64_t pad_id,
                    int32_t* n_alive, void* stream) {
    if (!x || !next_ids || !finished) return fail(PGMI_E_ARG, "null argument");
    if (B <= 0) return fail(PGMI_E_ARG, "eos_update: empty batch");
    eos_update((hipStream_t)stream, next_ids, finished, B, eos_id, pad_id, n_alive);
    LAUNCHCHK();
    return 0;
}

int pgmi_decode_kernel(pgmi_ctx* x, int which, int layer, int B, void* stream) {
    int rc;
    if ((rc = ensure_prepared(x))) return rc;
    const pgmi_config& c = x->c;
    if (B < 1 || B > c.max_batch) return fail(PGMI_E_ARG, "batch exceeds max_batch");
    if (layer < 0 || layer >= c.t_layers) return fail(PGMI_E_ARG, "layer out of range");
    hipStream_t s = (hipStream_t)stream;
    const float eps = c.t_rms_eps;
    const int H = c.t_hidden;
    const TextLayerW& w = x->w.t[layer];
    switch (which) {
        case 1: gemv_res(s, B, c.t_heads * c.t_head_dim, x->dAO, w.o, H, x->dH, x->ws); break;
        case 2: gemv_geglu(s, B, x->dH, w.post_norm, eps, w.gate_up, c.t_intermediate, x->dACT); break;
        case 3: gemv_res(s, B, c.t_intermediate, x->dACT, w.down, H, x->dH, x->ws); break;
        case 4: {
            int nparts = 0;
            gemv_logits(s, B, x->dH, x->w.final_norm, eps, x->w.embed, c.t_vocab, x->dlogits, x->pmax, x->pidx,
                        &nparts);
            break;
        }
        default: return fail(PGMI_E_ARG, "unknown kernel id");
    }
    LAUNCHCHK();
    return 0;
}

int pgmi_preprocess(pgmi_ctx* x, const void* src_hwc, int H, int W, int out_h, int out_w, float* out_chw,
                    void* stream) {
    if (!x || !src_hwc || !out_chw) return fail(PGMI_E_ARG, "null argument");
    if (H < 1 || W < 1 || out_h < 1 || out_w < 1) return fail(PGMI_E_ARG, "empty image");
    if (!x->ws) return fail(PGMI_E_STATE, "workspace not allocated (pgmi_prepare)");
    if (preprocess_scratch_bytes(H, W, out_h, out_w) > x->ws_bytes)
        return fail(PGMI_E_ARG, "image too large for the preprocessing scratch");
    preprocess((hipStream_t)stream, reinterpret_cast<const uint8_t*>(src_hwc), H, W, out_h, out_w, out_chw, x->ws);
    LAUNCHCHK();
    return 0;
}

int pgmi_prefill_kernel(pgmi_ctx* x, int which, int layer, int rows, void* stream) {
    int rc;
    if ((rc = ensure_prepared(x))) return rc;
    const pgmi_config& c = x->c;
    if (rows < 1 || rows > std::min(c.max_batch, kPrefillGroup) * c.max_seq)
        return fail(PGMI_E_ARG, "rows exceed the prefill workspace (one group of 8 sequences)");
    if (layer < 0 || layer >= c.t_layers) return fail(PGMI_E_ARG, "layer out of range");
    hipStream_t s = (hipStream_t)stream;
    const int H = c.t_hidden;
    const TextLayerW& w = x->w.t[layer];
    switch (which) {
        case 0: {
            EpiArgs g{};
            g.out = x->ACT; g.ldo = c.t_intermediate;
            gemm(s, x->Tn, H, w.gate_up, H, rows, c.t_intermediate, H, EPI_GEGLU, g, x->ws, x->ws_bytes,
                 c.t_intermediate);
            break;
        }
        case 1: {
            EpiArgs d{};
            d.res = x->Hs; d.ldr = H; d.out = x->Hs; d.ldo = H;
            gemm(s, x->ACT, c.t_intermediate, w.down, c.t_intermediate, rows, H, c.t_intermediate, EPI_RES, d, x->ws,
                 x->ws_bytes, 0, true);
            break;
        }
        default: return fail(PGMI_E_ARG, "unknown kernel id");
    }
    LAUNCHCHK();
    return 0;
}

int pgmi_debug_gemm_tiles(int n_mt, int n_nt, int S, int BM, int BN, int K, int* mt, int* nt, int* z) {
    if (n_mt < 1 || n_nt < 1 || S < 1 || !mt || !nt || !z) return fail(PGMI_E_ARG, "bad argument");
    return gemm_tile_order(n_mt, n_nt, S, BM, BN, K, mt, nt, z);
}

int pgmi_debug_gemm_plan(int M, int N, int K, int dual, int* cfg, int* bm, int* bn, int* split) {
    if (M < 1 || N < 1 || K < 1 || !cfg || !bm || !bn || !split) return fail(PGMI_E_ARG, "bad argument");
    gemm_plan(M, N, K, dual, cfg, bm, bn, split);
    return 0;
}

int pgmi_tune_gemm(int cfg, int split) {
    if ((cfg >= 0 && !gemm_cfg_valid(cfg)) || split < 0 || split > 32) return fail(PGMI_E_ARG, "bad GEMM plan");
    gemm_force_plan(cfg, split);
    return 0;
}

int pgmi_tune_gemm_shape(int M, int N, int K, int dual, int cfg, int split) {
    if ((cfg >= 0 && !gemm_cfg_valid(cfg)) || split < 0 || split > 16) return fail(PGMI_E_ARG, "bad GEMM plan");
    if (gemm_force_shape(M, N, K, dual, cfg, split)) return fail(PGMI_E_ARG, "too many per-shape GEMM plans");
    return 0;
}

int pgmi_tune_attention(int variant) {
    static const int ok[] = {-1, 0, 7, 8, 41, 42, 21, 22, 44, 24, 9, 91, 92, 94, 81, 82};
    for (int v : ok)
        if (v == variant) {
            attention_force_variant(variant);
            return 0;
        }
    return fail(PGMI_E_ARG, "unknown attention variant");
}

int pgmi_sample_top_p(pgmi_ctx* x, const float* logits, int rows, int V, float temperature, float top_p,
                      const float* u, int64_t* out, float* kept_mass, void* stream) {
    if (!x || !logits || !u || !out) return fail(PGMI_E_ARG, "null argument");
    if (rows <= 0 || V <= 0) return fail(PGMI_E_ARG, "sample_top_p: empty probabilities");
    if (!(top_p >= 0.f)) return fail(PGMI_E_ARG, "sample_top_p: top_p must be >= 0");
    if (!x->ws) return fail(PGMI_E_STATE, "workspace not allocated (pgmi_prepare)");
    const int per = (int)std::min<size_t>((size_t)rows, x->ws_bytes / sample_scratch_bytes(1, V));
    if (per < 1) return fail(PGMI_E_ARG, "sample_top_p: vocabulary exceeds the scratch");
    for (int r0 = 0; r0 < rows; r0 += per) {
        const int nr = std::min(per, rows - r0);
        sample_top_p((hipStream_t)stream, logits + (size_t)r0 * V, nr, V, temperature, top_p, u + r0, x->ws,
                     out + r0, kept_mass ? kept_mass + r0 : nullptr);
    }
    LAUNCHCHK();
    return 0;
}

int pgmi_op_gemm(pgmi_ctx* x, const void* A, const void* Wt, int M, int N, int K, int epi, const void* bias,
                 const void* res, void* out, void* stream) {
    int rc;
    if ((rc = ensure_prepared(x))) return rc;
    if (K % 8 != 0) return fail(PGMI_E_ARG, "K must be a multiple of 8");
    EpiArgs e{};
    e.bias = reinterpret_cast<const uint16_t*>(bias);
    e.res = reinterpret_cast<const uint16_t*>(res);
    e.ldr = N;
    e.ldo = N;
    if (epi == EPI_F32) e.out_f32 = reinterpret_cast<float*>(out);
    else e.out = reinterpret_cast<uint16_t*>(out);
    gemm((hipStream_t)stream, reinterpret_cast<const uint16_t*>(A), K, reinterpret_cast<const uint16_t*>(Wt), K, M, N,
         K, (Epi)epi, e, x->ws, x->ws_bytes, epi == EPI_GEGLU ? N : 0);
    LAUNCHCHK();
    return 0;
}

int pgmi_op_lm_logprobs(pgmi_ctx* x, const void* normed, const void* W, int rows, int V, int K, const int64_t* labels,
                        int64_t ignore_index, float* logprob, float* lse, void* stream) {
    if (!x || !normed || !W || !labels || !logprob) return fail(PGMI_E_ARG, "null argument");
    if (rows < 1) return fail(PGMI_E_ARG, "lm_logprobs: no rows");
    int rc;
    if ((rc = ensure_prepared(x))) return rc;
    return lm_logprobs_run(x, normed, reinterpret_cast<const uint16_t*>(W), rows, V, K, labels, ignore_index, logprob,
                           lse, stream);
}

int pgmi_op_gemm_strided(pgmi_ctx* x, const void* A, int lda, const void* Wt, int ldw, int M, int N, int K, int epi,
                         const void* bias, const void* res, void* out, void* stream) {
    int rc;
    if ((rc = ensure_prepared(x))) return rc;
    if (K % 8 != 0 || lda < K || ldw < K || lda % 8 != 0 || ldw % 8 != 0)
        return fail(PGMI_E_ARG, "K, lda, ldw must be multiples of 8 with lda, ldw >= K");
    EpiArgs e{};
    e.bias = reinterpret_cast<const uint16_t*>(bias);
    e.res = reinterpret_cast<const uint16_t*>(res);
    e.ldr = N;
    e.ldo = N;
    if (epi == EPI_F32) e.out_f32 = reinterpret_cast<float*>(out);
    else e.out = reinterpret_cast<uint16_t*>(out);
    gemm((hipStream_t)stream, reinterpret_cast<const uint16_t*>(A), lda, reinterpret_cast<const uint16_t*>(Wt), ldw, M,
         N, K, (Epi)epi, e, x->ws, x->ws_bytes, epi == EPI_GEGLU ? N : 0);
    LAUNCHCHK();
    return 0;
}

int pgmi_op_rmsnorm(pgmi_ctx* x, const void* in, const void* w, int rows, int D, float eps, void* out, void* stream) {
    if (!x) return fail(PGMI_E_ARG, "null ctx");
    rmsnorm((hipStream_t)stream, reinterpret_cast<const uint16_t*>(in), reinterpret_cast<const uint16_t*>(w), eps,
            reinterpret_cast<uint16_t*>(out), rows, D);
    LAUNCHCHK();
    return 0;
}

int pgmi_op_layernorm(pgmi_ctx* x, const void* in, const void* w, const void* b, int rows, int D, float eps, void* out,
                      void* stream) {
// ... 132 lines not shown
```

### multimodal-financial-analysis-tool-using-paligemma_amd/csrc/gemv_body.h

```cpp
#pragma once
#include <type_traits>

#include "coh.h"
#include "common.h"
#include "launch.h"

namespace pgmi {

enum GemvMode : int { GV_QKV = 0, GV_RES = 1, GV_GEGLU = 2, GV_LOGITS = 3, GV_ORES = 4 };

struct GemvArgs {
    const uint16_t* x;
    const uint16_t* norm_w;
    float eps;
    const uint16_t* W;
    int n_units;
    int K;
    int nb;
    int I;
    uint16_t* out;
    float* logits;
    float* pmax;
    int* pidx;
    unsigned* done;
    int64_t* next;
    StepState* adv;
    int64_t* hist;
    const uint16_t* cosT;
    const uint16_t* sinT;
    int max_pos;
    const StepState* st;
    int st_stride;
    int adv_n;
    uint16_t* kc;
    uint16_t* vc;
    long kv_b_stride;
    int nkv;
    const float* part;
    int max_chunks;
    int G;
    uint16_t* o_out;
    const int64_t* ids;
    const uint16_t* E;
    float normalizer;
    int64_t pad_id;
    uint16_t* emb_out;
    float* ssq;
    const uint16_t* Wf;
};

template <int B, int KCH, int RPW, int MODE, int WK, bool XREG, int DEPTH = 1, bool EMB = false, bool RG = false>
__device__ __forceinline__ void gemv_block(const GemvArgs& a, const int blk, const int nblk, uint16_t* xs) {
    static_assert(!EMB || (MODE == GV_QKV && XREG && WK == 1), "embedding fold: register-held q|k|v input only");
    static_assert(!RG || MODE == GV_QKV || MODE == GV_ORES, "per-row step records: q|k|v and o_proj only");
    constexpr int NR = (MODE == GV_QKV || MODE == GV_GEGLU) ? 2 : 1;
    constexpr int KCW = KCH / WK;
    constexpr int NL = RPW * NR * KCW;
    constexpr int K = KCH * 512;
    constexpr int GPB = 4 / WK;
#ifndef PGMI_SMALL_NT
#define PGMI_SMALL_NT 1
#endif
    constexpr bool kSmallTemporal = !PGMI_SMALL_NT && (MODE == GV_QKV || MODE == GV_ORES);
    __shared__ float red[4][B];
    __shared__ float kred[WK > 1 ? 4 : 1][RPW * NR * B];

    const int tid = threadIdx.x, lane = tid & 63, wave = tid >> 6;
    const int wk = wave % WK, grp = wave / WK;
    const int stride = nblk * GPB * RPW;
    int bb = blk * GPB * RPW;
    const int bend = a.n_units;
    int ub = bb + grp * RPW;
    const int kofs = wk * KCW * 512 + 8 * lane;

    auto row_of = [&](int u, int j) -> long {
        if constexpr (MODE == GV_QKV) return (long)((u >> 7) * 256 + (u & 127) + j * 128);
        else if constexpr (MODE == GV_GEGLU) return (long)u + (long)j * a.I;
        else return (long)u;
    };

    uint4 w[DEPTH][NL];
    auto issue = [&](auto slot, int base) {
        constexpr int SL = decltype(slot)::value;
#pragma unroll
        for (int i = 0; i < RPW; ++i) {
            int u = base + i;
            if (u >= bend) u = bend - 1;
#pragma unroll
            for (int j = 0; j < NR; ++j) {
                const uint16_t* rp = a.W + row_of(u, j) * K + kofs;
#pragma unroll
                for (int c = 0; c < KCW; ++c)
                    w[SL][(i * NR + j) * KCW + c] = kSmallTemporal ? ldg16(rp + 512 * c) : ldg_nt(rp + 512 * c);
            }
        }
    };
    using S0 = std::integral_constant<int, 0>;
    using S1 = std::integral_constant<int, DEPTH - 1>;
    constexpr bool NORM = MODE != GV_RES && MODE != GV_ORES;
    uint4 xr[XREG ? B : 1][XREG ? KCW : 1];
    uint4 nw[XREG && NORM ? KCW : 1];
    auto load_x = [&]() {
        if constexpr (XREG && MODE != GV_ORES) {
#pragma unroll
            for (int b = 0; b < B; ++b) {
                const int bq = b < a.nb ? b : a.nb - 1;
                const uint16_t* xrow;
                if constexpr (EMB) {
                    const int64_t id = a.ids[bq];
                    xrow = a.E + (id == a.pad_id ? 0 : id) * (long)K;
                } else {
                    xrow = a.x + (long)bq * K;
                }
#pragma unroll
                for (int c = 0; c < KCW; ++c) xr[b][c] = ldx16<false>(xrow + kofs + 512 * c);
            }
            if (NORM && a.norm_w) {
#pragma unroll
                for (int c = 0; c < KCW; ++c) nw[c] = ldg16(a.norm_w + kofs + 512 * c);
            }
        }
    };
    constexpr bool XFIRST = MODE == GV_QKV;
    if constexpr (XFIRST) {
        load_x();
        issue(S0{}, ub);
        if constexpr (DEPTH == 2) issue(S1{}, ub + stride);
        asm volatile("" ::: "memory");
    } else {
        issue(S0{}, ub);
        if constexpr (DEPTH == 2) issue(S1{}, ub + stride);
        load_x();
    }

    if constexpr (MODE == GV_ORES) {
        const int nch0 = (a.st->kv_len + 1 + kAttnChunk - 1) / kAttnChunk;
        constexpr int CMAX = 12;
        const int nitems = a.nb * K / 8;
        for (int e8 = tid; e8 < nitems; e8 += 256) {
            const int b = e8 / (K / 8), e = (e8 % (K / 8)) * 8;
            const int h = e >> 8;
            const int nch = RG ? (a.st[b * a.st_stride].kv_len + 1 + kAttnChunk - 1) / kAttnChunk : nch0;
            const float* pb = a.part + (long)b * a.max_chunks * kAttnPartStride + h * 256 + (e & 255);
            const float* sp = a.part + (long)b * a.max_chunks * kAttnPartStride + 16 * 256 + h;
            float o[8];
#pragma unroll
            for (int j = 0; j < 8; ++j) o[j] = 0.f;
            float M = -INFINITY, S = 0.f;
            if (nch <= CMAX) {
                f32x4 x0[CMAX], x1[CMAX];
                float mc[CMAX], lc[CMAX];
#pragma unroll
                for (int c = 0; c < CMAX; ++c) {
                    const long cs = (long)(c < nch ? c : nch - 1) * kAttnPartStride;
                    x0[c] = ldxf4<false>(pb + cs);
                    x1[c] = ldxf4<false>(pb + cs + 4);
                    mc[c] = ldxf<false>(sp + cs);
                    lc[c] = ldxf<false>(sp + cs + 16);
                }
#pragma unroll
                for (int c = 0; c < CMAX; ++c)
                    if (c < nch) M = fmaxf(M, mc[c]);
#pragma unroll
                for (int c = 0; c < CMAX; ++c)
                    if (c < nch) {
                        const float w = expf(mc[c] - M);
                        S += w * lc[c];
#pragma unroll
                        for (int j = 0; j < 4; ++j) { o[j] += w * x0[c][j]; o[4 + j] += w * x1[c][j]; }
                    }
            } else {
                for (int c = 0; c < nch; ++c) M = fmaxf(M, ldxf<false>(sp + (long)c * kAttnPartStride));
                for (int c = 0; c < nch; ++c) {
                    const float w = expf(ldxf<false>(sp + (long)c * kAttnPartStride) - M);
                    S += w * ldxf<false>(sp + (long)c * kAttnPartStride + 16);
                    const f32x4 x0 = ldxf4<false>(pb + (long)c * kAttnPartStride);
                    const f32x4 x1 = ldxf4<false>(pb + (long)c * kAttnPartStride + 4);
#pragma unroll
                    for (int j = 0; j < 4; ++j) { o[j] += w * x0[j]; o[4 + j] += w * x1[j]; }
                }
            }
            u16x8 ob;
#pragma unroll
            for (int j = 0; j < 8; ++j) ob.v[j] = f2bf(o[j] / S);
            *reinterpret_cast<u16x8*>(xs + b * K + e) = ob;
            if (a.o_out && blk == 0) *reinterpret_cast<u16x8*>(a.o_out + (long)b * K + e) = ob;
        }
        for (int e8 = tid; e8 < (B - a.nb) * K / 8; e8 += 256)
            *reinterpret_cast<uint4*>(xs + a.nb * K + e8 * 8) = make_uint4(0, 0, 0, 0);
        __syncthreads();
    } else if constexpr (XREG) {
#pragma unroll
        for (int b = 0; b < B; ++b)
            if (b >= a.nb)
#pragma unroll
                for (int c = 0; c < KCW; ++c) xr[b][c] = make_uint4(0, 0, 0, 0);
        if constexpr (EMB) {
#pragma unroll
            for (int b = 0; b < B; ++b) {
                const bool pad = a.ids[b < a.nb ? b : a.nb - 1] == a.pad_id;
#pragma unroll
                for (int c = 0; c < KCW; ++c) {
                    const uint16_t* e = reinterpret_cast<const uint16_t*>(&xr[b][c]);
                    u16x8 o;
#pragma unroll
                    for (int j = 0; j < 8; ++j) o.v[j] = pad ? (uint16_t)0 : f2bf(bf2f(e[j]) * a.normalizer);
                    xr[b][c] = *reinterpret_cast<const uint4*>(&o);
                    if (blk == 0 && wave == 0 && b < a.nb)
                        *reinterpret_cast<uint4*>(a.emb_out + (long)b * K + kofs + 512 * c) = xr[b][c];
                }
            }
        }
        if (NORM && a.norm_w) {
#pragma unroll
            for (int b = 0; b < B; ++b) {
                float ss = 0.f;
#pragma unroll
                for (int c = 0; c < KCW; ++c) {
                    const uint16_t* e = reinterpret_cast<const uint16_t*>(&xr[b][c]);
#pragma unroll
                    for (int j = 0; j < 8; ++j) { const float f = bf2f(e[j]); ss += f * f; }
                }
                ss = wave_sum(ss);
                const float r = 1.0f / sqrtf(ss / (float)K + a.eps);
#pragma unroll
                for (int c = 0; c < KCW; ++c) {
                    const uint16_t* we = reinterpret_cast<const uint16_t*>(&nw[c]);
                    const uint16_t* e = reinterpret_cast<const uint16_t*>(&xr[b][c]);
                    u16x8 o;
#pragma unroll
                    for (int j = 0; j < 8; ++j) o.v[j] = f2bf((bf2f(e[j]) * r) * (1.0f + bf2f(we[j])));
                    xr[b][c] = *reinterpret_cast<const uint4*>(&o);
                }
            }
        }
    } else {
        float ss[B];
#pragma unroll
        for (int b = 0; b < B; ++b) ss[b] = 0.f;
        for (int c = tid * 8; c < K; c += 256 * 8) {
#pragma unroll
            for (int b = 0; b < B; ++b) {
                uint4 v = (b < a.nb) ? ldx16<false>(a.x + (long)b * K + c) : make_uint4(0, 0, 0, 0);
                *reinterpret_cast<uint4*>(xs + b * K + c) = v;
                if (a.norm_w) {
                    const uint16_t* e = reinterpret_cast<const uint16_t*>(&v);
#pragma unroll
                    for (int j = 0; j < 8; ++j) { float f = bf2f(e[j]); ss[b] += f * f; }
                }
            }
        }
        if (a.norm_w) {
#pragma unroll
            for (int b = 0; b < B; ++b) {
                float t = wave_sum(ss[b]);
                if (lane == 0) red[wave][b] = t;
            }
            __syncthreads();
            float r[B];
#pragma unroll
            for (int b = 0; b < B; ++b)
                r[b] = 1.0f / sqrtf((red[0][b] + red[1][b] + red[2][b] + red[3][b]) / (float)K + a.eps);
            for (int c = tid * 8; c < K; c += 256 * 8) {
                uint4 wv = ldg16(a.norm_w + c);
                const uint16_t* we = reinterpret_cast<const uint16_t*>(&wv);
#pragma unroll
                for (int b = 0; b < B; ++b) {
                    uint4 v = *reinterpret_cast<uint4*>(xs + b * K + c);
                    const uint16_t* e = reinterpret_cast<const uint16_t*>(&v);
                    u16x8 o;
#pragma unroll
                    for (int j = 0; j < 8; ++j) o.v[j] = f2bf((bf2f(e[j]) * r[b]) * (1.0f + bf2f(we[j])));
                    *reinterpret_cast<u16x8*>(xs + b * K + c) = o;
                }
            }
        }
        __syncthreads();
    }

    int kv_len = 0, pos = 0;
    int kv_len_r[RG ? B : 1], pos_r[RG ? B : 1];
    if constexpr (MODE == GV_QKV && RG) {
#pragma unroll
        for (int b = 0; b < B; ++b) {
            const StepState sb = a.st[(b < a.nb ? b : a.nb - 1) * a.st_stride];
            kv_len_r[b] = sb.kv_len;
            pos_r[b] = sb.position < 0 ? 0 : (sb.position > a.max_pos - 1 ? a.max_pos - 1 : sb.position);
        }
    } else if constexpr (MODE == GV_QKV) {
        kv_len = a.st->kv_len;
        pos = a.st->position;
        if (pos < 0) pos = 0;
        if (pos > a.max_pos - 1) pos = a.max_pos - 1;
    }
    float best[B];
    int besti[B];
#pragma unroll
    for (int b = 0; b < B; ++b) { best[b] = -INFINITY; besti[b] = 0x7fffffff; }

    auto step = [&](auto slot, auto issue_next) {
        constexpr int SL = decltype(slot)::value;
        constexpr bool ISSUE = decltype(issue_next)::value;
        float pre[RPW][B][2];
#pragma unroll
        for (int i = 0; i < RPW; ++i) {
            const int u = ub + i < bend ? ub + i : bend - 1;
#pragma unroll
            for (int b = 0; b < B; ++b) {
                const int bq = b < a.nb ? b : a.nb - 1;
                if constexpr (MODE == GV_RES || MODE == GV_ORES) {
                    pre[i][b][0] = bf2f(ldxh<false>(a.out + (long)bq * a.n_units + u));
                } else if constexpr (MODE == GV_QKV) {
                    const int pb_ = RG ? pos_r[RG ? b : 0] : pos;
                    pre[i][b][0] = bf2f(a.cosT[(long)pb_ * 128 + (u & 127)]);
                    pre[i][b][1] = bf2f(a.sinT[(long)pb_ * 128 + (u & 127)]);
                }
            }
        }
        float acc[RPW][NR][B];
#pragma unroll
        for (int i = 0; i < RPW; ++i)
#pragma unroll
            for (int j = 0; j < NR; ++j)
#pragma unroll
                for (int b = 0; b < B; ++b) acc[i][j][b] = 0.f;
#pragma unroll
        for (int c = 0; c < KCW; ++c) {
#pragma unroll
            for (int b = 0; b < B; ++b) {
                uint4 xv;
                if constexpr (XREG) xv = xr[b][c];
                else xv = *reinterpret_cast<const uint4*>(xs + b * K + kofs + 512 * c);
#pragma unroll
                for (int i = 0; i < RPW; ++i)
#pragma unroll
                    for (int j = 0; j < NR; ++j) acc[i][j][b] = dot8(w[SL][(i * NR + j) * KCW + c], xv, acc[i][j][b]);
            }
        }
        const int cur = ub;
        ub += stride;
        bb += stride;
        if constexpr (ISSUE) {
            if constexpr (DEPTH == 1) issue(slot, ub + (DEPTH - 1) * stride);
            else if (ub + (DEPTH - 1) * stride < bend) issue(slot, ub + (DEPTH - 1) * stride);
        }

#pragma unroll
        for (int i = 0; i < RPW; ++i)
#pragma unroll
            for (int j = 0; j < NR; ++j)
#pragma unroll
                for (int b = 0; b < B; ++b) acc[i][j][b] = wave_sum(acc[i][j][b]);
        if constexpr (WK > 1) {
            if (lane == 0) {
#pragma unroll
                for (int i = 0; i < RPW; ++i)
#pragma unroll
                    for (int j = 0; j < NR; ++j)
#pragma unroll
                        for (int b = 0; b < B; ++b) kred[wave][(i * NR + j) * B + b] = acc[i][j][b];
            }
            __syncthreads();
#pragma unroll
            for (int i = 0; i < RPW; ++i)
#pragma unroll
                for (int j = 0; j < NR; ++j)
#pragma unroll
                    for (int b = 0; b < B; ++b) {
                        float t = 0.f;
#pragma unroll
                        for (int q = 0; q < WK; ++q) t += kred[grp * WK + q][(i * NR + j) * B + b];
                        acc[i][j][b] = t;
                    }
            __syncthreads();
            if (wk != 0) return;
        }

#pragma unroll
        for (int i = 0; i < RPW; ++i) {
            const int u = cur + i;
            if (u >= bend) break;
#pragma unroll
            for (int b = 0; b < B; ++b) {
                if (b >= a.nb) break;
                if constexpr (MODE == GV_RES || MODE == GV_ORES) {
                    if (lane == 0) {
                        stxh<false>(a.out + (long)b * a.n_units + u, f2bf(rbf(acc[i][0][b]) + pre[i][b][0]));
                    }
                } else if constexpr (MODE == GV_GEGLU) {
                    if (lane == 0) {
                        const float g = rbf(gelu_tanh(rbf(acc[i][0][b])));
                        stxh<false>(a.out + (long)b * a.I + u, f2bf(g * rbf(acc[i][1][b])));
                    }
                } else if constexpr (MODE == GV_LOGITS) {
                    const float v = rbf(acc[i][0][b]);
                    if (lane == 0) a.logits[(long)b * a.n_units + u] = v;
                    if (v > best[b]) { best[b] = v; besti[b] = u; }
                } else {
                    if (lane == 0) {
                        const int hh = u >> 7, d = u & 127;
                        const int kvl = RG ? kv_len_r[RG ? b : 0] : kv_len;
                        const float x0 = rbf(acc[i][0][b]), x1 = rbf(acc[i][1][b]);
                        const int nh = a.I;
                        if (hh < nh + a.nkv) {
                            const float c = pre[i][b][0];
                            const float sn = pre[i][b][1];
                            const uint16_t o0 = f2bf(rbf(x0 * c) + rbf(-x1 * sn));
                            const uint16_t o1 = f2bf(rbf(x1 * c) + rbf(x0 * sn));
                            uint16_t* dst;
                            if (hh < nh) {
                                dst = a.out + (long)b * nh * 256 + hh * 256;
                            } else {
                                dst = a.kc + b * a.kv_b_stride + (long)kvl * (a.nkv * 256) + (hh - nh) * 256;
                            }
                            stxh<false>(dst + d, o0);
                            stxh<false>(dst + d + 128, o1);
                        } else {
                            uint16_t* dst = a.vc + b * a.kv_b_stride + (long)kvl * (a.nkv * 256) +
                                            (hh - nh - a.nkv) * 256;
                            stxh<false>(dst + d, f2bf(x0));
                            stxh<false>(dst + d + 128, f2bf(x1));
                        }
                    }
                }
            }
        }
    };
    using Yes = std::true_type;
    using No = std::false_type;
    if constexpr (DEPTH == 1) {
        while (bb + stride < bend) step(S0{}, Yes{});
        if (bb < bend) step(S0{}, No{});
    } else {
        while (bb < bend) {
            step(S0{}, Yes{});
            if (bb >= bend) break;
            step(S1{}, Yes{});
        }
    }

    if constexpr (MODE == GV_LOGITS) {
        __shared__ float bv[4][B];
        __shared__ int bi[4][B];
        if (lane == 0) {
#pragma unroll
            for (int b = 0; b < B; ++b) { bv[wave][b] = best[b]; bi[wave][b] = besti[b]; }
        }
        __syncthreads();
        if (tid == 0) {
#pragma unroll
            for (int b = 0; b < B; ++b) {
                if (b >= a.nb) break;
                float m = bv[0][b];
                int mi = bi[0][b];
                for (int q = 1; q < 4; ++q)
                    if (bv[q][b] > m || (bv[q][b] == m && bi[q][b] < mi)) { m = bv[q][b]; mi = bi[q][b]; }
                if (a.done) {
                    stf_coh(a.pmax + (long)b * nblk + blk, m);
                    sti_coh(a.pidx + (long)b * nblk + blk, mi);
                } else {
                    stxf<false>(a.pmax + (long)b * nblk + blk, m);
                    stxi<false>(a.pidx + (long)b * nblk + blk, mi);
                }
            }
        }
        if (a.done) {
            constexpr int NSH = 32, STR = 32;
            __shared__ int last;
            if (tid == 0) {
                asm volatile("s_waitcnt vmcnt(0)" ::: "memory");
                const int sh = blk % NSH;
                const unsigned shard_n = (unsigned)((nblk - sh + NSH - 1) / NSH);
                const unsigned n_sh = (unsigned)(nblk < NSH ? nblk : NSH);
                last = 0;
                if (__hip_atomic_fetch_add(a.done + (1 + sh) * STR, 1u, __ATOMIC_RELAXED, __HIP_MEMORY_SCOPE_AGENT) + 1 ==
                    shard_n)
                    last = __hip_atomic_fetch_add(a.done, 1u, __ATOMIC_RELAXED, __HIP_MEMORY_SCOPE_AGENT) + 1 == n_sh;
            }
            __syncthreads();
            if (last) {
                for (int b = 0; b < a.nb && b < B; ++b) {
                    float m = -INFINITY;
                    int mi = 0x7fffffff;
                    for (int i = tid; i < nblk; i += blockDim.x) {
                        const float v = ldf_coh(a.pmax + (long)b * nblk + i);
                        const int ix = ldi_coh(a.pidx + (long)b * nblk + i);
                        if (v > m || (v == m && ix < mi)) { m = v; mi = ix; }
                    }
#pragma unroll
                    for (int o = 32; o > 0; o >>= 1) {
                        const float v = __shfl_xor(m, o);
                        const int ix = __shfl_xor(mi, o);
                        if (v > m || (v == m && ix < mi)) { m = v; mi = ix; }
                    }
                    __syncthreads();
                    if (lane == 0) { bv[wave][0] = m; bi[wave][0] = mi; }
                    __syncthreads();
                    if (tid == 0) {
                        for (int q = 1; q < 4; ++q)
                            if (bv[q][0] > m || (bv[q][0] == m && bi[q][0] < mi)) { m = bv[q][0]; mi = bi[q][0]; }
                        a.next[b] = mi;
                        if (a.hist) a.hist[b] = mi;
                    }
                }
                if (tid == 0) {
                    if (a.adv) {
                        a.adv->kv_len += 1;
                        a.adv->position += 1;
                        for (int r = 1; r < a.adv_n; ++r) {
                            a.adv[r].kv_len += 1;
                            a.adv[r].position += 1;
                        }
                    }
                }
                if (tid <= NSH) __hip_atomic_store(a.done + tid * STR, 0u, __ATOMIC_RELAXED, __HIP_MEMORY_SCOPE_AGENT);
            }
        }
    }
}

template <int B, int KCH, int RPW, int MODE, int WK, bool XREG, int DEPTH, bool EMB = false, bool RG = false>
__global__ void __launch_bounds__(256) k_gemv(GemvArgs a) {
    extern __shared__ __attribute__((aligned(16))) uint16_t xs[];
    gemv_block<B, KCH, RPW, MODE, WK, XREG, DEPTH, EMB, RG>(a, blockIdx.x, gridDim.x, xs);
}

}
```

### multimodal-financial-analysis-tool-using-paligemma_amd/csrc/kernels_gemv.hip

```cpp
#include <cstdlib>

#include "gemv_body.h"

namespace pgmi {

int gemv_mf_min_batch();
void gemv_mf_qkv(hipStream_t s, const GemvArgs& a, float* ws);
void gemv_mf_geglu(hipStream_t s, const GemvArgs& a);
void gemv_mf_ores(hipStream_t s, const GemvArgs& a, uint16_t* o);
int gemv_mf_logits(hipStream_t s, const GemvArgs& a, int max_blocks);
void gemv_mf_res(hipStream_t s, const GemvArgs& a, float* ws);
void gemv_mf_res_norm(hipStream_t s, const GemvArgs& a, float* ws, const uint16_t* norm_w, float eps, uint16_t* hn);

static thread_local hipError_t g_launch_err = hipSuccess;
static thread_local const char* g_launch_what = "";

void launch_error_set(hipError_t e, const char* what) {
    if (g_launch_err != hipSuccess) return;
    g_launch_err = e;
    g_launch_what = what;
}

hipError_t launch_error_take(const char** what) {
    const hipError_t e = g_launch_err;
    if (what) *what = g_launch_what;
    g_launch_err = hipSuccess;
    return e;
}

template <int B, int KCH, int RPW, int MODE, int WK = 1, int DEPTH = 1, bool EMB = false, bool RG = false>
static void launch_gemv(hipStream_t s, const GemvArgs& a, int max_blocks = 0) {
    constexpr bool XREG = (MODE != GV_ORES) && B * (KCH / WK) <= 8;
    size_t lds = XREG ? 0 : (size_t)B * KCH * 512 * sizeof(uint16_t);
    static size_t attr = 0;
    if (lds > attr) {
        const hipError_t e = hipFuncSetAttribute(reinterpret_cast<const void*>(&k_gemv<B, KCH, RPW, MODE, WK, XREG, DEPTH, EMB, RG>),
                                                 hipFuncAttributeMaxDynamicSharedMemorySize, (int)lds);
        if (e != hipSuccess) {
            launch_error_set(e, "k_gemv: dynamic LDS size");
            return;
        }
        attr = lds;
    }
    constexpr int per_block = (4 / WK) * RPW;
    int blocks = (a.n_units + per_block - 1) / per_block;
    if (max_blocks > 0 && blocks > max_blocks) blocks = max_blocks;
    hipLaunchKernelGGL((k_gemv<B, KCH, RPW, MODE, WK, XREG, DEPTH, EMB, RG>), dim3(blocks), dim3(256), lds, s, a);
}

bool gemv_qkv_folds_embed(int B) { return B <= 2 && B < gemv_mf_min_batch(); }

void gemv_qkv(hipStream_t s, int B, int nh, int nkv, const uint16_t* h, const uint16_t* norm_w, float eps,
              const uint16_t* Wqkv, const uint16_t* cosT, const uint16_t* sinT, int max_pos, const StepState* st,
              uint16_t* q_out, uint16_t* kc, uint16_t* vc, long kv_b_stride, float* ws, const EmbedFold* emb,
              const uint16_t* Wf, int st_stride) {
    GemvArgs a{};
    a.x = h; a.norm_w = norm_w; a.eps = eps; a.W = Wqkv; a.n_units = (nh + 2 * nkv) * 128; a.K = 2048; a.nb = B;
    a.I = nh; a.out = q_out; a.cosT = cosT; a.sinT = sinT; a.max_pos = max_pos; a.st = st; a.kc = kc; a.vc = vc;
    a.kv_b_stride = kv_b_stride; a.nkv = nkv; a.st_stride = st_stride;
    const bool rg = st_stride != 0 && B > 1;
    if (emb) {
        a.ids = emb->ids; a.E = emb->E; a.normalizer = emb->normalizer; a.pad_id = emb->pad_id; a.emb_out = emb->h_out;
        if (B <= 1) launch_gemv<1, 4, 1, GV_QKV, 1, 1, true>(s, a);
        else if (rg) launch_gemv<2, 4, 1, GV_QKV, 1, 1, true, true>(s, a);
        else launch_gemv<2, 4, 1, GV_QKV, 1, 1, true>(s, a);
        return;
    }
#define L_(b_, kch, rpw, mode) launch_gemv<b_, kch, rpw, mode>(s, a)
    if (B >= gemv_mf_min_batch()) {
        a.Wf = Wf;
        gemv_mf_qkv(s, a, ws);
        return;
    }
    if (B <= 1) L_(1, 4, 1, GV_QKV);
    else if (rg) launch_gemv<2, 4, 1, GV_QKV, 1, 1, false, true>(s, a);
    else L_(2, 4, 1, GV_QKV);
}

void gemv_res(hipStream_t s, int B, int K, const uint16_t* x, const uint16_t* W, int N, uint16_t* h_inout,
              float* ws) {
    GemvArgs a{};
    a.x = x; a.norm_w = nullptr; a.W = W; a.n_units = N; a.K = K; a.nb = B; a.out = h_inout;
    if (B >= gemv_mf_min_batch() && K % 128 == 0 && ws) {
        gemv_mf_res(s, a, ws);
        return;
    }
    if (K == 2048) {
        if (B <= 1) L_(1, 4, 1, GV_RES);
        else if (B <= 2) L_(2, 4, 1, GV_RES);
        else if (B <= 4) L_(4, 4, 1, GV_RES);
        else if (B <= 8) L_(8, 4, 1, GV_RES);
        else {
            for (int b0 = 0; b0 < B; b0 += 8) {
                GemvArgs c = a;
                c.x = x + (long)b0 * K; c.out = h_inout + (long)b0 * N; c.nb = (B - b0) < 8 ? (B - b0) : 8;
                launch_gemv<8, 4, 1, GV_RES>(s, c);
            }
        }
    } else {
        for (int b0 = 0; b0 < B; b0 += 4) {
            const int nb = (B - b0) < 4 ? (B - b0) : 4;
            GemvArgs c = a;
            c.x = x + (long)b0 * K; c.out = h_inout + (long)b0 * N; c.nb = nb;
            if (nb <= 1) launch_gemv<1, 32, 1, GV_RES, 4>(s, c, 512);
            else if (nb <= 2) launch_gemv<2, 32, 2, GV_RES, 4>(s, c);
            else launch_gemv<4, 32, 2, GV_RES, 4>(s, c);
        }
    }
}

void gemv_res_norm(hipStream_t s, int B, int K, const uint16_t* x, const uint16_t* W, int N, uint16_t* h_inout,
                   float* ws, const uint16_t* norm_w, float eps, uint16_t* hn, const uint16_t* Wf) {
    if (B >= gemv_mf_min_batch() && K % 2048 == 0 && K / 2048 <= 8 && K > 2048 && ws) {
        GemvArgs a{};
        a.x = x; a.norm_w = nullptr; a.W = W; a.n_units = N; a.K = K; a.nb = B; a.out = h_inout;
        a.Wf = N % 16 == 0 ? Wf : nullptr;
        gemv_mf_res_norm(s, a, ws, norm_w, eps, hn);
        return;
    }
    gemv_res(s, B, K, x, W, N, h_inout, ws);
    if (norm_w) rows_norm(s, h_inout, norm_w, eps, B, N, hn);
}

void gemv_o_attn(hipStream_t s, int B, int G, const float* part, int max_chunks, const StepState* st,
                 const uint16_t* Wo, int N, uint16_t* h_inout, uint16_t* o_out, float* ssq, const uint16_t* Wf,
                 int st_stride) {
    GemvArgs a{};
    a.x = nullptr; a.norm_w = nullptr; a.W = Wo; a.n_units = N; a.K = G * 256; a.nb = B; a.out = h_inout;
    a.part = part; a.max_chunks = max_chunks; a.G = G; a.st = st; a.o_out = o_out;
    a.st_stride = st_stride;
    if (B >= gemv_mf_min_batch() && o_out) {
        a.ssq = ssq;
        a.Wf = N % 16 == 0 ? Wf : nullptr;
        gemv_mf_ores(s, a, o_out);
        return;
    }
    if (B <= 1) launch_gemv<1, 4, 2, GV_ORES>(s, a, 256);
    else if (B <= 2 && st_stride != 0) launch_gemv<2, 4, 2, GV_ORES, 1, 1, false, true>(s, a, 256);
    else if (B <= 2) launch_gemv<2, 4, 2, GV_ORES>(s, a, 256);
    else if (B <= 4) launch_gemv<4, 4, 1, GV_ORES>(s, a, 256);
    else if (B <= 8) launch_gemv<8, 4, 1, GV_ORES>(s, a, 256);
    else launch_error_set(hipErrorInvalidValue, "gemv_o_attn: more than 8 rows need the o_out buffer");
}

void gemv_geglu(hipStream_t s, int B, const uint16_t* h, const uint16_t* norm_w, float eps, const uint16_t* Wgu,
                int I, uint16_t* act, float* ssq, const uint16_t* Wf) {
    GemvArgs a{};
    a.x = h; a.norm_w = norm_w; a.eps = eps; a.W = Wgu; a.n_units = I; a.K = 2048; a.nb = B; a.I = I; a.out = act;
    if (B >= gemv_mf_min_batch()) {
        a.ssq = norm_w ? ssq : nullptr;
        a.Wf = I % 16 == 0 ? Wf : nullptr;
        gemv_mf_geglu(s, a);
        return;
    }
    if (B <= 1) launch_gemv<1, 4, 1, GV_GEGLU>(s, a, 1024);
    else L_(2, 4, 2, GV_GEGLU);
}

int gemv_logits_blocks() { return 2048; }

bool gemv_logits_folds(int B) { return B < gemv_mf_min_batch(); }

bool gemv_logits(hipStream_t s, int B, const uint16_t* h, const uint16_t* norm_w, float eps, const uint16_t* E,
                 int V, float* logits, float* pmax, int* pidx, int* nparts, unsigned* done, int64_t* next,
                 StepState* adv, int64_t* hist, int adv_n) {
    GemvArgs a{};
    a.x = h; a.norm_w = norm_w; a.eps = eps; a.W = E; a.n_units = V; a.K = 2048; a.nb = B; a.logits = logits;
    a.pmax = pmax; a.pidx = pidx;
    const int mb = gemv_logits_blocks();
    int blocks;
    if (B >= gemv_mf_min_batch()) {
        *nparts = gemv_mf_logits(s, a, mb);
        return false;
    }
    const bool fold = done && next && gemv_logits_folds(B);
    if (fold) {
        a.done = done;
        a.next = next;
        a.adv = adv;
        a.adv_n = adv_n;
        a.hist = hist;
    }
#define LG_(b_, rpw)                                                    \
    do {                                                                \
        blocks = (V + 4 * rpw - 1) / (4 * rpw);                         \
        if (blocks > mb) blocks = mb;                                   \
        launch_gemv<b_, 4, rpw, GV_LOGITS>(s, a, mb);                   \
    } while (0)
    if (B <= 1) LG_(1, 4);
    else LG_(2, 4);
    *nparts = blocks;
    return fold;
#undef LG_
#undef L_
}

}
```

### multimodal-financial-analysis-tool-using-paligemma_amd/csrc/launch.h

```cpp
#pragma once
#include <hip/hip_runtime.h>
#include <stdint.h>

namespace pgmi {

enum Epi : int {
    EPI_STORE = 0,
    EPI_BIAS = 1,
    EPI_BIAS_GELU = 2,
    EPI_BIAS_RES = 3,
    EPI_RES = 4,
    EPI_BIAS_POS = 5,
    EPI_F32 = 6,
    EPI_GEGLU = 7,
    EPI_ROPE = 8,
    EPI_LSE = 9,
};

struct EpiArgs {
    const uint16_t* bias = nullptr;
    const uint16_t* res = nullptr;
    int ldr = 0;
    const uint16_t* pos = nullptr;
    int npos = 0;
    uint16_t* out = nullptr;
    int ldo = 0;
    float* out_f32 = nullptr;
    const int64_t* rpos = nullptr;
    const uint16_t* cosT = nullptr;
    const uint16_t* sinT = nullptr;
    int max_pos = 0;
    uint16_t* q_out = nullptr;
    uint16_t* kc = nullptr;
    uint16_t* vc = nullptr;
    long kv_b_stride = 0;
    int kv_start = 0;
    int L = 1;
    int nh = 0;
    int nkv = 0;
    const int64_t* lse_labels = nullptr;
    float2* lse_part = nullptr;
    float* lse_lab = nullptr;
    int lse_nt = 0;
};

bool gemm_qkv_rope(hipStream_t s, const uint16_t* A, int lda, const uint16_t* W, int ldw, int M, int N, int K,
                   const EpiArgs& ea);
int gemm(hipStream_t s, const uint16_t* A, int lda, const uint16_t* W, int ldw, int M, int N, int K,
         Epi epi, const EpiArgs& ea, float* ws, size_t ws_bytes, int up_offset_rows = 0, bool defer = false);
size_t gemm_ws_bytes(int M, int N, int K);
int gemm_lse_tiles(int M, int N, int K);
bool gemm_lse(hipStream_t s, const uint16_t* A, int lda, const uint16_t* W, int ldw, int M, int N, int K,
              const int64_t* labels, float2* part, float* lab);
void lse_combine(hipStream_t s, const float2* part, int n_nt, const float* lab, const int64_t* labels, int rows, int N,
                 int64_t ignore_index, float* logprob, float* lse);
void gemm_force_plan(int cfg, int split);
int gemm_force_shape(int M, int N, int K, int dual, int cfg, int split);
void gemm_probe_events(hipEvent_t start, hipEvent_t stop);
int gemm_tile_order(int n_mt, int n_nt, int S, int BM, int BN, int K, int* mt, int* nt, int* z);
bool gemm_cfg_valid(int cfg);
void gemm_plan(int M, int N, int K, int dual, int* cfg, int* bm, int* bn, int* split);

void launch_error_set(hipError_t e, const char* what);
hipError_t launch_error_take(const char** what);
struct StepState {
    int kv_len;
    int position;
};

struct EmbedFold {
    const int64_t* ids;
    const uint16_t* E;
    float normalizer;
    int64_t pad_id;
    uint16_t* h_out;
};
bool gemv_qkv_folds_embed(int B);
void gemv_qkv(hipStream_t s, int B, int nh, int nkv, const uint16_t* h, const uint16_t* norm_w, float eps,
              const uint16_t* Wqkv, const uint16_t* cosT, const uint16_t* sinT, int max_pos, const StepState* st,
              uint16_t* q_out, uint16_t* kc, uint16_t* vc, long kv_b_stride, float* ws = nullptr,
              const EmbedFold* emb = nullptr, const uint16_t* Wf = nullptr,
              int st_stride = 0);
void gemv_res(hipStream_t s, int B, int K, const uint16_t* x, const uint16_t* W, int N, uint16_t* h_inout,
              float* ws);
void gemv_res_norm(hipStream_t s, int B, int K, const uint16_t* x, const uint16_t* W, int N, uint16_t* h_inout,
                   float* ws, const uint16_t* norm_w, float eps, uint16_t* hn, const uint16_t* Wf = nullptr);
void mf_swizzle(hipStream_t s, const uint16_t* W, int rows, int K, uint16_t* out, bool qkv = false);
void rows_norm(hipStream_t s, const uint16_t* x, const uint16_t* w, float eps, int nb, int K, uint16_t* out);
void gemv_o_attn(hipStream_t s, int B, int G, const float* part, int max_chunks, const StepState* st,
                 const uint16_t* Wo, int N, uint16_t* h_inout, uint16_t* o_out, float* ssq = nullptr,
                 const uint16_t* Wf = nullptr, int st_stride = 0);
void gemv_geglu(hipStream_t s, int B, const uint16_t* h, const uint16_t* norm_w, float eps,
                const uint16_t* Wgu, int I, uint16_t* act, float* ssq = nullptr, const uint16_t* Wf = nullptr);
int gemv_logits_blocks();
int gemv_mf_min_batch();
bool gemv_logits(hipStream_t s, int B, const uint16_t* h, const uint16_t* norm_w, float eps,
                 const uint16_t* E, int V, float* logits, float* pmax, int* pidx, int* nparts,
                 unsigned* done = nullptr, int64_t* next = nullptr, StepState* adv = nullptr,
                 int64_t* hist = nullptr, int adv_n = 1);
void argmax_finish(hipStream_t s, int B, const float* pmax, const int* pidx, int nparts, int64_t* out,
                   StepState* adv = nullptr, int64_t* hist = nullptr, int adv_n = 1);
int argmax_scratch_parts();
void argmax_rows(hipStream_t s, const float* x, int rows, int V, float* pmax, int* pidx, int64_t* out);
void logprob_rows(hipStream_t s, const float* x, int rows, int V, const int64_t* ids, int64_t ignore_index, float* pm,
                  float* ps, float* logprob, float* lse);
void eos_update(hipStream_t s, int64_t* next, int* finished, int B, int64_t eos, int64_t pad, int* n_alive);

struct AttnArgs {
    const uint16_t* q; long q_b_stride; int q_row_stride; int q_head_stride;
    const uint16_t* k; long k_b_stride; int k_row_stride; int k_head_stride;
    const uint16_t* v; long v_b_stride; int v_row_stride; int v_head_stride;
    uint16_t* o; long o_b_stride; int o_row_stride; int o_head_stride;
    int Lq;
    int Lk;
    int G;
    int n_kv;
    int B;
    float scale;
    float* ws;
    long ws_floats;
    const float* mask;
    long mask_b_stride;
    int mask_k_stride;
    int mask_round;
    const int* klen;
};
void attention_prefill(hipStream_t s, int head_dim, const AttnArgs& a);
void attention_decode(hipStream_t s, const AttnArgs& a, const StepState* st, int launch_keys, float* part,
                      int max_chunks, int st_stride = 0);
constexpr int kAttnChunk = 64;
constexpr int kAttnPartStride = 16 * 256 + 32;
size_t attention_decode_part_floats(int B, int n_kv, int max_chunks);
int attention_prefill_max_keys(int head_dim);
void attention_force_variant(int v);

struct ModAttnArgs {
    const uint16_t* q;
    const uint16_t* k;
    const uint16_t* v;
    long kv_b_stride, kv_h_stride, kv_row_stride;
    uint16_t* o;
    uint16_t* probs;
    const void* mask;
    long m_b_stride, m_h_stride, m_q_stride;
    int mask_f32;
    int B, Lq, Lk, H, Hkv, hd;
    float scale;
    int scale_div;
};
size_t attention_exact_lds(int Lk, int hd);
void attention_exact(hipStream_t s, const ModAttnArgs& a);
void rope_rows(hipStream_t s, const uint16_t* x, const uint16_t* cs, const uint16_t* sn, long rows, int heads, int hd,
               uint16_t* out);

void splitk_res_norm(hipStream_t s, const float* ws, int split, const uint16_t* bias, uint16_t* h, const uint16_t* w,
                     const uint16_t* b, float eps, uint16_t* out, int rows, int D);
void rmsnorm(hipStream_t s, const uint16_t* x, const uint16_t* w, float eps, uint16_t* out, int rows, int D);
void layernorm(hipStream_t s, const uint16_t* x, const uint16_t* w, const uint16_t* b, float eps, uint16_t* out,
               int rows, int D);
void embed_rows(hipStream_t s, const int64_t* ids, int rows, const uint16_t* E, int D, float normalizer,
                int64_t pad_id, uint16_t* out);
void merge_embed(hipStream_t s, const int64_t* ids, int B, int L, const uint16_t* E, int D,
                 const uint16_t* img, int n_img_rows, int64_t image_token, int64_t pad_id, float sqrt_h,
                 float normalizer, const uint16_t* embeds_in, int* scan_buf, uint16_t* out,
                 const int* lens = nullptr);
void gather_last_rows(hipStream_t s, const uint16_t* x, int B, int L, int D, const int* lens, uint16_t* out);
constexpr int kMaxRows = 16;
struct RowInts { int v[kMaxRows]; };
void set_step_rows(hipStream_t s, StepState* st, const RowInts& kv_lens, const RowInts& positions, int B);
void set_row_ints(hipStream_t s, int* dst, const RowInts& a, const RowInts& b2, int B);
void scale_rows(hipStream_t s, const uint16_t* x, long n, float normalizer, uint16_t* out);
void add_rows(hipStream_t s, const uint16_t* x, const uint16_t* y, long n, uint16_t* out);
void rope_kv_append(hipStream_t s, const uint16_t* qkv, const float* ws, int split, int B, int L, int nh, int nkv,
                    const int64_t* pos, const uint16_t* cosT, const uint16_t* sinT, int max_pos, uint16_t* q_out,
                    uint16_t* kcache, uint16_t* vcache, long kv_b_stride, int kv_start);
void patchify(hipStream_t s, const void* px, int px_is_f32, int B, int C, int H, int W, int P, int Kpad,
              uint16_t* out);
void fill_synthetic(hipStream_t s, uint16_t* dst, long n, uint64_t key, float scale, float offset);
void set_step(hipStream_t s, StepState* st, int kv_len, int position);
void set_step_dev(hipStream_t s, StepState* st, int kv_len, const void* pos, int dtype);
void stage_mask(hipStream_t s, const void* src, int dtype, int B, long b_stride, int n, float* dst, int ld);
size_t preprocess_scratch_bytes(int H, int W, int out_h, int out_w);
void preprocess(hipStream_t s, const uint8_t* src, int H, int W, int out_h, int out_w, float* out, void* scratch);
void pad_rows(hipStream_t s, const uint16_t* src, int rows, int K, int Kpad, uint16_t* dst);
size_t sample_scratch_bytes(int rows, int V);
void sample_top_p(hipStream_t s, const float* x, int rows, int V, float temperature, float top_p, const float* u,
                  void* scratch, int64_t* out, float* kept_mass);


bool gemv_logits_folds(int B);

}
```

### multimodal-financial-analysis-tool-using-paligemma_amd/pgmi/_native.py

```python
from __future__ import annotations

import ctypes
import os

import torch

_HERE = os.path.dirname(os.path.abspath(__file__))
LIB_PATH = os.environ.get("PGMI_LIB_PATH") or os.path.join(_HERE, "libpgmi.so")

PGMI_OK, PGMI_E_ARG, PGMI_E_STATE, PGMI_E_HIP, PGMI_E_NOMEM = 0, -1, -2, -3, -4
DTYPE_BF16, DTYPE_F16, DTYPE_F32 = 0, 1, 2

EPI = {"store": 0, "bias": 1, "bias_gelu": 2, "bias_res": 3, "res": 4, "bias_pos": 5, "f32": 6, "geglu": 7}


class PgmiConfig(ctypes.Structure):
    _fields_ = [
        ("v_hidden", ctypes.c_int), ("v_intermediate", ctypes.c_int), ("v_layers", ctypes.c_int),
        ("v_heads", ctypes.c_int), ("v_channels", ctypes.c_int), ("v_image", ctypes.c_int),
        ("v_patch", ctypes.c_int), ("v_ln_eps", ctypes.c_float),
        ("t_vocab", ctypes.c_int), ("t_hidden", ctypes.c_int), ("t_intermediate", ctypes.c_int),
        ("t_layers", ctypes.c_int), ("t_heads", ctypes.c_int), ("t_kv_heads", ctypes.c_int),
        ("t_head_dim", ctypes.c_int), ("t_max_pos", ctypes.c_int), ("t_rms_eps", ctypes.c_float),
        ("t_rope_theta", ctypes.c_float), ("projection_dim", ctypes.c_int),
        ("image_token_index", ctypes.c_int64), ("pad_token_id", ctypes.c_int64),
        ("max_batch", ctypes.c_int), ("max_seq", ctypes.c_int), ("max_kv", ctypes.c_int),
    ]


vp, i32, i64, f32, u64 = ctypes.c_void_p, ctypes.c_int, ctypes.c_int64, ctypes.c_float, ctypes.c_uint64

SIGNATURES = {
    "pgmi_last_error": (ctypes.c_char_p, []),
    "pgmi_version": (ctypes.c_char_p, []),
    "pgmi_create": (i32, [i32, ctypes.POINTER(PgmiConfig), ctypes.POINTER(vp)]),
    "pgmi_destroy": (i32, [vp]),
    "pgmi_weights_bytes": (i64, [vp]),
    "pgmi_weight_count": (i32, [vp]),
    "pgmi_weight_info": (i32, [vp, i32, ctypes.POINTER(ctypes.c_char_p), ctypes.POINTER(i64),
                               ctypes.POINTER(i64 * 4), ctypes.POINTER(i32)]),
    "pgmi_bind_weights": (i32, [vp, vp]),
    "pgmi_load_weight": (i32, [vp, ctypes.c_char_p, vp, i32, i32, vp]),
    "pgmi_fill_synthetic": (i32, [vp, ctypes.c_char_p, u64, f32, f32, vp]),
    "pgmi_load_safetensors": (i32, [vp, ctypes.c_char_p, ctypes.POINTER(i32), ctypes.POINTER(i32), vp]),
    "pgmi_safetensors_count": (i32, [ctypes.c_char_p, ctypes.POINTER(i32)]),
    "pgmi_safetensors_entry": (i32, [ctypes.c_char_p, i32, ctypes.c_char_p, i32, ctypes.POINTER(i32),
                                     ctypes.POINTER(i64 * 4), ctypes.POINTER(i32), ctypes.POINTER(i64),
                                     ctypes.POINTER(i64)]),
    "pgmi_synthetic_key": (u64, [ctypes.c_char_p, u64]),
    "pgmi_set_rope_inv_freq": (i32, [vp, ctypes.POINTER(f32)]),
    "pgmi_set_rope_table": (i32, [vp, vp, vp, i32]),
    "pgmi_prepare": (i32, [vp]),
    "pgmi_kv_bytes": (i64, [vp, i32, i32]),
    "pgmi_vision": (i32, [vp, vp, i32, i32, vp, vp]),
    "pgmi_project": (i32, [vp, vp, i32, vp, vp]),
    "pgmi_embed": (i32, [vp, vp, i32, vp, vp]),
    "pgmi_lm_forward": (i32, [vp, vp, vp, i32, vp, i32, i32, vp, vp, i32, i32, i32, vp, i32, vp]),
    "pgmi_decode": (i32, [vp, vp, i32, vp, i32, i32, i32, i32, vp, vp, i32, vp]),
    "pgmi_decode_steps": (i32, [vp, vp, i32, vp, i32, i32, i32, i32, i32, vp, vp, i32, vp]),
    "pgmi_lm_forward_ragged": (i32, [vp, vp, vp, i32, vp, i32, i32, vp, vp, vp, i32, i32, i32, vp, i32, vp]),
    "pgmi_decode_ragged": (i32, [vp, vp, i32, vp, i32, i32, vp, vp, i32, vp, vp, vp, i32, vp]),
    "pgmi_decode_embeds": (i32, [vp, vp, i32, vp, i32, i32, i32, i32, vp, vp, i32, vp]),
    "pgmi_decode_embeds_dev": (i32, [vp, vp, i32, vp, i32, i32, i32, vp, i32, vp, i32, i64, vp, vp, i32, vp]),
    "pgmi_set_prefill_graph": (i32, [vp, i32]),
    "pgmi_graph_count": (i32, [vp, i32]),
    "pgmi_set_decode_staged_norm": (i32, [vp, i32]),
    "pgmi_prefill_kernel": (i32, [vp, i32, i32, i32, vp]),
    "pgmi_debug_gemm_tiles": (i32, [i32, i32, i32, i32, i32, i32, vp, vp, vp]),
    "pgmi_debug_gemm_plan": (i32, [i32, i32, i32, i32, vp, vp, vp, vp]),
    "pgmi_prefill_probe": (i32, [vp, i32]),
    "pgmi_prefill_probe_times": (i32, [vp, ctypes.POINTER(f32), i32]),
    "pgmi_preprocess": (i32, [vp, vp, i32, i32, i32, i32, vp, vp]),
    "pgmi_argmax": (i32, [vp, vp, i32, i32, vp, vp]),
    "pgmi_lm_head": (i32, [vp, vp, i32, vp, vp]),
    "pgmi_lm_final_hidden": (i32, [vp, vp, i32, vp]),
    "pgmi_lm_logprobs": (i32, [vp, vp, i32, vp, i64, vp, vp, vp]),
    "pgmi_logprobs": (i32, [vp, vp, i32, i32, vp, i64, vp, vp, vp]),
    "pgmi_op_lm_logprobs": (i32, [vp, vp, vp, i32, i32, i32, vp, i64, vp, vp, vp]),
    "pgmi_comm_unique_id": (i32, [vp]),
    "pgmi_comm_init": (i32, [i32, i32, i32, vp, ctypes.POINTER(vp)]),
    "pgmi_comm_destroy": (i32, [vp]),
    "pgmi_broadcast_weights": (i32, [vp, vp, i32, vp]),
    "pgmi_eos_update": (i32, [vp, vp, vp, i32, i64, i64, vp, vp]),
    "pgmi_decode_kernel": (i32, [vp, i32, i32, i32, vp]),
    "pgmi_tune_gemm": (i32, [i32, i32]),
    "pgmi_tune_gemm_shape": (i32, [i32, i32, i32, i32, i32, i32]),
    "pgmi_tune_attention": (i32, [i32]),
    "pgmi_sample_top_p": (i32, [vp, vp, i32, i32, f32, f32, vp, vp, vp, vp]),
    "pgmi_op_gemm": (i32, [vp, vp, vp, i32, i32, i32, i32, vp, vp, vp, vp]),
    "pgmi_op_gemm_strided": (i32, [vp, vp, i32, vp, i32, i32, i32, i32, i32, vp, vp, vp, vp]),
    "pgmi_op_rmsnorm": (i32, [vp, vp, vp, i32, i32, f32, vp, vp]),
    "pgmi_op_layernorm": (i32, [vp, vp, vp, vp, i32, i32, f32, vp, vp]),
    "pgmi_op_attention": (i32, [vp, vp, vp, vp, vp, i32, i32, i32, i32, i32, i32, f32, vp]),
    "pgmi_op_add": (i32, [vp, vp, vp, i64, vp, vp]),
    "pgmi_op_patch_embed": (i32, [vp, vp, i32, i32, i32, i32, i32, vp, vp, vp, i32, vp, vp]),
    "pgmi_op_gemv_res": (i32, [vp, vp, vp, i32, i32, i32, vp, vp]),
    "pgmi_op_attention_ex": (i32, [vp, vp, vp, vp, vp, i32, i32, i32, i32, i32, i32, i32, f32, i32, vp, i32, i64, i64,
                                   i64, vp, vp]),
    "pgmi_op_rope": (i32, [vp, vp, vp, vp, i64, i32, i32, vp, vp]),
    "pgmi_op_scale": (i32, [vp, vp, f32, i64, vp, vp]),
}

_lib = None


class NativeError(RuntimeError):
    pass


def lib():
    global _lib
    if _lib is None:
        if not os.path.exists(LIB_PATH):
            raise NativeError(f"{LIB_PATH} not built: run `make -C csrc` or __graft_entry__.build()")
        L = ctypes.CDLL(LIB_PATH)
        for name, (res, args) in SIGNATURES.items():
            fn = getattr(L, name)
            fn.restype = res
            fn.argtypes = args
        _lib = L
    return _lib


def check(rc: int, what: str = ""):
    if rc == PGMI_OK:
        return
    msg = lib().pgmi_last_error().decode(errors="replace")
    text = f"{what}: {msg}" if what else msg
    if rc == PGMI_E_ARG:
        raise ValueError(text)
    if rc == PGMI_E_STATE:
        raise AssertionError(text)
    if rc == PGMI_E_NOMEM:
        raise MemoryError(text)
    raise NativeError(text)


def ptr(t) -> "int | None":
    return None if t is None else t.data_ptr()


def safetensors_index(path: str):
    L = lib()
    n = ctypes.c_int()
    check(L.pgmi_safetensors_count(path.encode(), ctypes.byref(n)), path)
    out = []
    for i in range(n.value):
        name = ctypes.create_string_buffer(1024)
        dt, nd = ctypes.c_int(), ctypes.c_int()
        shape, b, e = (i64 * 4)(), ctypes.c_int64(), ctypes.c_int64()
        check(L.pgmi_safetensors_entry(path.encode(), i, name, 1024, ctypes.byref(dt), ctypes.byref(shape),
                                       ctypes.byref(nd), ctypes.byref(b), ctypes.byref(e)), path)
        out.append((name.value.decode(), dt.value, tuple(shape[j] for j in range(nd.value)), b.value, e.value))
    return out


def stream_handle(device=None) -> int:
    if isinstance(device, torch.device) and device.index is not None:
        return torch._C._cuda_getCurrentRawStream(device.index)
    return torch.cuda.current_stream(device).cuda_stream
```

### multimodal-financial-analysis-tool-using-paligemma_amd/pgmi/engine.py

```python
from __future__ import annotations

import ctypes
import math
from typing import NamedTuple, Optional

import torch

from . import _native as N
from . import ragged as R


def config_dict(cfg) -> dict:
    if isinstance(cfg, dict):
        v, t = dict(cfg["vision_config"]), dict(cfg["text_config"])
        top = cfg
        get = top.get
    else:
        v = dict(vars(cfg.vision_config))
        t = dict(vars(cfg.text_config))
        top = vars(cfg)
        get = top.get
    pad = get("pad_token_id", None)
    return {
        "v_hidden": v.get("hidden_size", 768), "v_intermediate": v.get("intermediate_size", 3072),
# ... 272 lines not shown
            raise ValueError(f"need one id per row: {lb.numel()} != {x.shape[0]}")
        out = torch.empty(x.shape[0], dtype=torch.float32, device=self.device)
        lse = torch.empty_like(out) if return_lse else None
        N.check(self.lib.pgmi_logprobs(self.ctx, x.data_ptr(), x.shape[0], x.shape[1], lb.data_ptr(), int(ignore_index),
                                       out.data_ptr(), N.ptr(lse), self._s()), "pgmi_logprobs")
        return (out, lse) if return_lse else out

    @torch.no_grad()
    def shifted_logprobs(self, hidden: torch.Tensor, shift_labels: torch.Tensor, live: Optional[torch.Tensor] = None,
                         ignore_index: int = -100):
        shift = shift_labels.to(self.device, torch.int64)
        B, L1 = shift.shape
        L = L1 + 1
        if live is None:
            live = shift != ignore_index
        out = torch.zeros((B, L1), dtype=torch.float32, device=self.device)
        at = live.nonzero()
        if at.shape[0] == 0:
            return out, live, torch.full((), float("nan"), dtype=torch.float32, device=self.device)
        out[at[:, 0], at[:, 1]] = self.lm_logprobs(hidden.index_select(0, at[:, 0] * L + at[:, 1]),
                                                   shift[at[:, 0], at[:, 1]], ignore_index)
        return out, live, (-out.sum(dtype=torch.float64) / at.shape[0]).float()

    @torch.no_grad()
    def score(self, input_ids: torch.Tensor, pixel_values: Optional[torch.Tensor], labels: torch.Tensor,
              attention_mask: Optional[torch.Tensor] = None, ignore_index: int = -100) -> "Score":
        ids = input_ids.to(self.device, torch.int64)
        lab = labels.to(self.device, torch.int64)
        if tuple(lab.shape) != tuple(ids.shape):
            raise ValueError(f"labels {tuple(lab.shape)} do not match input_ids {tuple(ids.shape)}")
        lens = R.lengths_from_mask(attention_mask) if attention_mask is not None else None
        if lens is not None:
            ids, lens = R.right_pad(ids, attention_mask)
            lab, _ = R.right_pad(lab, attention_mask, pad_id=ignore_index)
        ids = ids.contiguous()
        B, L = ids.shape
        feats = self.project(self.vision(pixel_values)) if pixel_values is not None else None
        kv = self.scratch_kv(B, L)
        self.lm_forward(kv, 0, torch.arange(L).expand(B, L), ids=ids, image_feats=feats, logits_rows=1, lens=lens)
        hidden = self.final_hidden(B * L)
        shift = lab[:, 1:]
        live = shift != ignore_index
        if lens is not None:
            live &= (torch.arange(1, L, device=self.device)[None, :] < lens.to(self.device)[:, None])
        out, live, loss = self.shifted_logprobs(hidden, shift, live, ignore_index)
        return Score(out, out.sum(1), live.sum(1), loss)

    def decode(self, ids: torch.Tensor, kv: torch.Tensor, kv_len: int, position: int, logits: torch.Tensor = None,
               next_ids: torch.Tensor = None, graph: bool = False) -> torch.Tensor:
        self._ready()
        if ids.dtype is not torch.int64 or ids.device != self.device or not ids.is_contiguous():
            ids = ids.to(self.device, torch.int64).contiguous()
        ids = ids.view(-1)
        B = ids.numel()
        if logits is None:
            logits = torch.empty((B, self.cfgd["t_vocab"]), dtype=torch.float32, device=self.device)
        N.check(self.lib.pgmi_decode(self.ctx, ids.data_ptr(), B, kv.data_ptr(), kv.shape[2], kv.shape[3], kv_len,
                                     position, logits.data_ptr(), N.ptr(next_ids), int(graph), self._s()),
                "pgmi_decode")
        return logits

    def decode_steps(self, ids: torch.Tensor, kv: torch.Tensor, kv_len: int, position: int, n_steps: int,
                     logits: torch.Tensor = None, tokens: torch.Tensor = None, graph: bool = False) -> torch.Tensor:
        self._ready()
        if ids.dtype is not torch.int64 or ids.device != self.device or not ids.is_contiguous():
            raise ValueError("decode_steps: ids must be a contiguous int64 tensor on the engine's device (updated in place)")
        B = ids.numel()
        if logits is None:
            logits = torch.empty((B, self.cfgd["t_vocab"]), dtype=torch.float32, device=self.device)
        if tokens is not None and (tokens.dtype is not torch.int64 or tokens.device != self.device
                                   or not tokens.is_contiguous() or tokens.numel() < n_steps * B):
            raise ValueError("decode_steps: tokens must be a contiguous int64 (n_steps, B) tensor on the device")
        N.check(self.lib.pgmi_decode_steps(self.ctx, ids.data_ptr(), B, kv.data_ptr(), kv.shape[2], kv.shape[3], kv_len,
                                           position, int(n_steps), logits.data_ptr(), N.ptr(tokens), int(graph),
                                           self._s()), "pgmi_decode_steps")
        return logits

    def decode_ragged(self, ids: torch.Tensor, kv: torch.Tensor, kv_lens, positions, n_steps: int = 1,
                      logits: torch.Tensor = None, tokens: torch.Tensor = None, next_ids: torch.Tensor = None,
                      graph: bool = False) -> torch.Tensor:
        self._ready()
        if ids.dtype is not torch.int64 or ids.device != self.device or not ids.is_contiguous():
            if n_steps > 1 and next_ids is None:
                raise ValueError("decode_ragged: ids must be a contiguous int64 tensor on the engine's device "
                                 "(updated in place when n_steps > 1)")
            ids = ids.to(self.device, torch.int64).contiguous()
        ids = ids.view(-1)
        B = ids.numel()
        kl = torch.as_tensor(kv_lens).detach().to("cpu", torch.int32).reshape(-1).contiguous()
        ps = torch.as_tensor(positions).detach().to("cpu", torch.int32).reshape(-1).contiguous()
        if kl.numel() != B or ps.numel() != B:
            raise ValueError(f"decode_ragged: kv_lens / positions need {B} entries each")
        if n_steps > 1 and next_ids is None:
            next_ids = ids
        if logits is None:
            logits = torch.empty((B, self.cfgd["t_vocab"]), dtype=torch.float32, device=self.device)
        if tokens is not None and (tokens.dtype is not torch.int64 or tokens.device != self.device
                                   or not tokens.is_contiguous() or tokens.numel() < n_steps * B):
            raise ValueError("decode_ragged: tokens must be a contiguous int64 (n_steps, B) tensor on the device")
        N.check(self.lib.pgmi_decode_ragged(self.ctx, ids.data_ptr(), B, kv.data_ptr(), kv.shape[2], kv.shape[3],
                                            kl.data_ptr(), ps.data_ptr(), int(n_steps), logits.data_ptr(),
                                            N.ptr(next_ids), N.ptr(tokens), int(graph), self._s()),
                "pgmi_decode_ragged")
        return logits

    def decode_embeds(self, embeds: torch.Tensor, kv: torch.Tensor, kv_len: int, position: int,
                      logits: torch.Tensor = None, graph: bool = False) -> torch.Tensor:
        self._ready()
        e = embeds.to(self.device, torch.bfloat16).reshape(-1, self.cfgd["t_hidden"]).contiguous()
        B = e.shape[0]
        if logits is None:
            logits = torch.empty((B, self.cfgd["t_vocab"]), dtype=torch.float32, device=self.device)
        N.check(self.lib.pgmi_decode_embeds(self.ctx, e.data_ptr(), B, kv.data_ptr(), kv.shape[2], kv.shape[3], kv_len,
                                            position, logits.data_ptr(), None, int(graph), self._s()),
                "pgmi_decode_embeds")
        return logits

    _POS_DTYPES = {torch.bfloat16: 0, torch.float32: 2, torch.int64: 10, torch.int32: 11, torch.float64: 12}

    def decode_embeds_dev(self, embeds: torch.Tensor, kv: torch.Tensor, kv_len: int, position: torch.Tensor,
                          mask: torch.Tensor = None, logits: torch.Tensor = None, graph: bool = False,
                          next_ids: torch.Tensor = None) -> torch.Tensor:
        self._ready()
        e = embeds.to(self.device, torch.bfloat16).reshape(-1, self.cfgd["t_hidden"]).contiguous()
        if e.shape[0] != 1:
            raise ValueError("decode_embeds_dev: one sequence per step")
        p = position.to(self.device).reshape(-1)[:1]
        if p.dtype not in self._POS_DTYPES:
            p = p.to(torch.float64)
        p = p.contiguous()
        mp, mdt = None, N.DTYPE_BF16
        if mask is not None:
            m = mask.to(self.device).reshape(-1)
            if m.numel() != kv_len + 1:
                raise ValueError(f"mask has {m.numel()} keys, the step attends {kv_len + 1}")
            if m.dtype not in (torch.bfloat16, torch.float32):
                m = m.float()
            mp = m.contiguous()
            mdt = N.DTYPE_F32 if mp.dtype == torch.float32 else N.DTYPE_BF16
        if logits is None:
            logits = torch.empty((1, self.cfgd["t_vocab"]), dtype=torch.float32, device=self.device)
        N.check(self.lib.pgmi_decode_embeds_dev(self.ctx, e.data_ptr(), 1, kv.data_ptr(), kv.shape[2], kv.shape[3],
                                                kv_len, p.data_ptr(), self._POS_DTYPES[p.dtype], N.ptr(mp), mdt,
                                                mp.numel() if mp is not None else 0, logits.data_ptr(),
                                                N.ptr(next_ids), int(graph), self._s()),
                "pgmi_decode_embeds_dev")
        return logits

    def set_prefill_graph(self, on: bool) -> None:
        N.check(self.lib.pgmi_set_prefill_graph(self.ctx, int(bool(on))), "pgmi_set_prefill_graph")

    def set_decode_staged_norm(self, on: int) -> None:
        N.check(self.lib.pgmi_set_decode_staged_norm(self.ctx, int(on)), "pgmi_set_decode_staged_norm")

    def argmax(self, logits: torch.Tensor) -> torch.Tensor:
        l2 = logits.reshape(-1, logits.shape[-1]).contiguous()
        out = torch.empty(l2.shape[0], dtype=torch.int64, device=self.device)
        N.check(self.lib.pgmi_argmax(self.ctx, l2.data_ptr(), l2.shape[0], l2.shape[1], out.data_ptr(), self._s()))
        return out

    def sample_top_p(self, x: torch.Tensor, top_p: float, temperature: Optional[float] = None,
                     u: Optional[torch.Tensor] = None, generator: Optional[torch.Generator] = None,
                     return_kept_mass: bool = False):
        x2 = x.reshape(-1, x.shape[-1]).to(self.device, torch.float32).contiguous()
        rows, V = x2.shape
        if u is None:
            u = torch.rand(rows, device=self.device, generator=generator)
        u = u.to(self.device, torch.float32).reshape(-1).contiguous()
        if u.numel() != rows:
            raise ValueError(f"need one uniform per row: {u.numel()} != {rows}")
        out = torch.empty(rows, dtype=torch.int64, device=self.device)
        kept = torch.empty(rows, dtype=torch.float32, device=self.device) if return_kept_mass else None
        T = float(temperature) if temperature is not None and temperature > 0 else 0.0
        N.check(self.lib.pgmi_sample_top_p(self.ctx, x2.data_ptr(), rows, V, T, float(top_p), u.data_ptr(),
                                           out.data_ptr(), N.ptr(kept), self._s()), "pgmi_sample_top_p")
        return (out, kept) if return_kept_mass else out

    @torch.no_grad()
    def generate(self, input_ids: torch.Tensor, pixel_values: torch.Tensor, n_tokens: int, graph: bool = True,
                 kv: torch.Tensor = None, do_sample: bool = False, temperature: float = 0.8, top_p: float = 0.9,
                 generator: Optional[torch.Generator] = None, eos_token_id: Optional[int] = None,
                 pad_token_id: Optional[int] = None, sync_every: int = 16, return_lengths: bool = False,
                 attention_mask: Optional[torch.Tensor] = None, return_logprobs: bool = False):
        ids = input_ids.to(self.device, torch.int64)
        lens = R.lengths_from_mask(attention_mask) if attention_mask is not None else None
        if lens is not None:
            ids, lens = R.right_pad(ids, attention_mask)
            ids = ids.contiguous()
        B, L = ids.shape
        if kv is None:
            kv = self.new_kv(B, L + n_tokens + 1)
        feats = self.project(self.vision(pixel_values))
        logits = self.lm_forward(kv, 0, torch.arange(L).expand(B, L), ids=ids, image_feats=feats, logits_rows=2,
                                 lens=lens)
        toks = torch.empty((B, n_tokens), dtype=torch.int64, device=self.device)
        if do_sample:
            us = torch.rand((n_tokens, B), device=self.device, generator=generator)
            toks[:, 0] = self.sample_top_p(logits[:, 0], top_p, temperature, u=us[0])
        else:
            toks[:, 0] = self.argmax(logits[:, 0])
        if return_logprobs:
            lps = torch.zeros((B, n_tokens), dtype=torch.float32, device=self.device)
            lps[:, 0] = self.logprobs(logits[:, 0], toks[:, 0])
        bufs = self._gen_buf.get(B)
        if bufs is None:
            bufs = (torch.empty((B, self.cfgd["t_vocab"]), dtype=torch.float32, device=self.device),
                    torch.empty(B, dtype=torch.int64, device=self.device),
                    torch.empty(B, dtype=torch.int64, device=self.device),
                    torch.empty((self.GEN_CHUNK, B), dtype=torch.int64, device=self.device))
            self._gen_buf[B] = bufs
        step_logits, cur, nxt, rec = bufs
        cur.copy_(toks[:, 0])
        if lens is None:
            def step(t, next_ids, n=1, tokens=None):
                if tokens is not None:
                    self.decode_steps(cur, kv, L + t - 1, L + t, n, logits=step_logits, tokens=tokens, graph=graph)
                else:
                    self.decode(cur, kv, L + t - 1, L + t, logits=step_logits, next_ids=next_ids, graph=graph)
        else:
            lens = lens.to(torch.int32)

            def step(t, next_ids, n=1, tokens=None):
                self.decode_ragged(cur, kv, lens + (t - 1), lens + t, n, logits=step_logits, tokens=tokens,
                                   next_ids=next_ids, graph=graph)
        stop = eos_token_id is not None
        if stop:
            pad = int(eos_token_id if pad_token_id is None else pad_token_id)
            finished = torch.zeros(B, dtype=torch.int32, device=self.device)
            alive = torch.empty(1, dtype=torch.int32, device=self.device)
            self._eos_update(cur, finished, int(eos_token_id), pad, alive)
            toks[:, 0] = cur
        n_done = n_tokens
        if not do_sample and not stop and not return_logprobs and graph and n_tokens > 1 and B >= self.GEN_MIN_BATCH:
            t = 1
            while t < n_tokens:
                n = min(self.GEN_CHUNK, n_tokens - t)
                step(t, None, n, rec)
                toks[:, t:t + n] = rec[:n].t()
                t += n
        else:
            for t in range(1, n_tokens):
                if stop and (t - 1) % max(1, sync_every) == 0 and int(alive.item()) == 0:
                    n_done = t
                    break
                if do_sample:
                    step(t, nxt)
                    cur.copy_(self.sample_top_p(step_logits, top_p, temperature, u=us[t]))
                else:
                    step(t, cur)
                if return_logprobs:
                    lp = self.logprobs(step_logits, cur)
                    lps[:, t] = lp.masked_fill_(finished != 0, 0.0) if stop else lp
                if stop:
                    self._eos_update(cur, finished, int(eos_token_id), pad, alive)
                toks[:, t] = cur
        if not stop:
            ret = (toks, torch.full((B,), n_tokens, dtype=torch.int64, device=self.device)) if return_lengths else (toks,)
        else:
            toks = toks[:, :n_done]
            hit = toks == int(eos_token_id)
            first = torch.where(hit.any(1), hit.int().argmax(1) + 1,
                                torch.full_like(hit[:, 0], n_done, dtype=torch.int64))
            toks = toks[:, :int(first.max().item())].contiguous()
            ret = (toks, first.to(torch.int64)) if return_lengths else (toks,)
        if return_logprobs:
            ret = ret + (lps[:, :toks.shape[1]].contiguous(),)
        return ret if len(ret) > 1 else ret[0]

    def _eos_update(self, next_ids: torch.Tensor, finished: torch.Tensor, eos: int, pad: int,
                    n_alive: Optional[torch.Tensor]) -> None:
        N.check(self.lib.pgmi_eos_update(self.ctx, next_ids.data_ptr(), finished.data_ptr(), next_ids.numel(), eos, pad,
                                         n_alive.data_ptr() if n_alive is not None else None, self._s()),
                "pgmi_eos_update")
```

Baseline: 806.0 tokens/s.

## Pack decode GEMV weights into lossless 13-bit exponent-compressed images

Adds a lossless 13-bit packing of bf16 weights: sign and mantissa are kept at 8 bits, and the exponent is stored as a 5-bit offset from the tensor's maximum exponent. The packing is applied to the gate_up, down and lm_head matrices whenever every exponent fits, and the decode GEMV kernels decode the packed images on the fly. This targets the weight-bandwidth cost of batch-1 and batch-2 decode by reading about 19% fewer bytes per step. In exchange it needs extra device memory for the packed copies, a one-time scan and pack pass, and more ALU work in the GEMV inner loop.

```diff
diff --git a/include/pgmi.h b/include/pgmi.h
--- a/include/pgmi.h
+++ b/include/pgmi.h
@@ -83,6 +83,14 @@
 #define PGMI_GRAPH_CACHE_MAX 64
 int pgmi_graph_count(const pgmi_ctx* ctx, int which);
 int pgmi_set_decode_staged_norm(pgmi_ctx* ctx, int on);
+#define PGMI_PACKED_INFO_N 9
+int pgmi_set_decode_packed(pgmi_ctx* ctx, int on);
+int pgmi_decode_packed_info(const pgmi_ctx* ctx, int64_t* info, int n);
+int pgmi_decode_packed_tensor(const pgmi_ctx* ctx, int kind, int layer);
+int pgmi_pack13_scan(const uint16_t* w, int64_t n, int* e_hi, int* fits);
+int64_t pgmi_pack13_bytes(int64_t rows, int64_t K);
+int pgmi_pack13_encode(const uint16_t* w, int64_t rows, int64_t K, int e_hi, uint8_t* image);
+int pgmi_pack13_decode(const uint8_t* image, int64_t rows, int64_t K, int e_hi, uint16_t* w);
 int pgmi_lm_head(pgmi_ctx* ctx, const void* normed, int rows, float* logits, void* stream);
 int pgmi_lm_logprobs(pgmi_ctx* ctx, const void* normed, int rows, const int64_t* labels, int64_t ignore_index,
                      float* logprob, float* lse, void* stream);
@@ -102,6 +110,7 @@
                     int32_t* n_alive, void* stream);
 
 int pgmi_decode_kernel(pgmi_ctx* ctx, int which, int layer, int B, void* stream);
+int pgmi_debug_decode_buffer(pgmi_ctx* ctx, int which, void* buf, int64_t bytes, int write, void* stream);
 
 int pgmi_preprocess(pgmi_ctx* ctx, const void* src_hwc, int H, int W, int out_h, int out_w, float* out_chw,
                     void* stream);
diff --git a/multimodal-financial-analysis-tool-using-paligemma_amd/csrc/engine.hip b/multimodal-financial-analysis-tool-using-paligemma_amd/csrc/engine.hip
--- a/multimodal-financial-analysis-tool-using-paligemma_amd/csrc/engine.hip
+++ b/multimodal-financial-analysis-tool-using-paligemma_amd/csrc/engine.hip
@@ -15,6 +15,7 @@
 #include "../../include/pgmi.h"
 #include "common.h"
 #include "launch.h"
+#include "pack13.h"
 #include "safetensors_hdr.h"
 
 using namespace pgmi;
@@ -71,12 +72,17 @@
 struct TextLayerW {
     const uint16_t *qkv, *o, *gate_up, *down, *in_norm, *post_norm;
     const uint16_t *mf_gate_up = nullptr, *mf_qkv = nullptr, *mf_o = nullptr, *mf_down = nullptr;
+    PkW pk_gate_up, pk_down;
 };
 struct WeightTable {
     const uint16_t *patch_conv_w, *patch_b, *pos_emb, *post_ln_w, *post_ln_b, *proj_w, *proj_b, *embed, *final_norm;
     std::vector<VisionLayerW> v;
     std::vector<TextLayerW> t;
+    PkW pk_embed;
 };
+
+enum { PK_GATE_UP = 1, PK_DOWN = 2, PK_LM_HEAD = 4, PK_ALL = 7 };
+constexpr int kPkDefaultB1 = PK_ALL, kPkDefaultB2 = PK_LM_HEAD;
 
 struct pgmi_ctx {
     pgmi_config c;
@@ -106,6 +112,11 @@
     float* dSS;
     uint16_t* mfw = nullptr;
     bool mfw_dirty = false;
+    bool mfw_alloc_failed = false;
+    uint8_t* pk_buf[3] = {nullptr, nullptr, nullptr};
+    unsigned* pk_stat = nullptr;
+    int pk_mask = -1, pk_done = 0;
+    bool pk_alloc_failed = false;
     float *opart, *pmax, *dlogits, *amax_v;
     int *pidx, *amax_i;
     int max_chunks;
@@ -135,6 +146,22 @@
 
 namespace {
 
+int pk_mask_for(const pgmi_ctx* x, int B) {
+    return x->pk_mask >= 0 ? x->pk_mask : B <= 1 ? kPkDefaultB1 : kPkDefaultB2;
+}
+
+PkW pk_use(const pgmi_ctx* x, int B, int kind, const PkW& w) {
+    const bool on = B <= 2 && B < gemv_mf_min_batch() && (pk_mask_for(x, B) & x->pk_done & kind);
+    return on ? w : PkW{};
+}
+
+void pk_forget(pgmi_ctx* x) {
+    x->pk_done = 0;
+    x->pk_alloc_failed = false;
+    x->w.pk_embed = PkW{};
+    for (auto& t : x->w.t) t.pk_gate_up = t.pk_down = PkW{};
+}
+
 int n_img(const pgmi_config& c) { return (c.v_image / c.v_patch) * (c.v_image / c.v_patch); }
 
 void add_slot(pgmi_ctx* x, const std::string& name, std::initializer_list<int64_t> shape) {
@@ -438,6 +465,7 @@
     if (!x || !slab) return fail(PGMI_E_ARG, "null argument");
     if (reinterpret_cast<uintptr_t>(slab) % 256 != 0) return fail(PGMI_E_ARG, "weight slab must be 256-byte aligned");
     x->slab = reinterpret_cast<uint8_t*>(slab);
+    pk_forget(x);
     x->dgraphs.clear();
     x->pgraphs.clear();
     return bind_tables(x);
@@ -673,6 +701,7 @@
     pad_rows(nullptr, x->w.patch_conv_w, c.v_hidden, c.v_channels * c.v_patch * c.v_patch, x->kpad, x->patch_w);
     LAUNCHCHK();
     x->mfw_dirty = c.max_batch >= gemv_mf_min_batch() && c.t_intermediate % 32 == 0 && c.t_hidden % 32 == 0;
+    pk_forget(x);
     std::vector<uint16_t> cs, sn;
     if (!x->host_cos.empty()) {
         cs = x->host_cos;
@@ -951,8 +980,9 @@
                 attention_prefill(s, 256, a);
                 gemv_res(s, B, NH * HD, x->dAO, w.o, H, lastrows, x->ws);
             }
-            gemv_geglu(s, B, lastrows, w.post_norm, eps, w.gate_up, c.t_intermediate, x->dACT);
-            gemv_res(s, B, c.t_intermediate, x->dACT, w.down, H, lastrows, x->ws);
+            gemv_geglu(s, B, lastrows, w.post_norm, eps, w.gate_up, c.t_intermediate, x->dACT, nullptr, nullptr,
+                       pk_use(x, B, PK_GATE_UP, w.pk_gate_up));
+            gemv_res(s, B, c.t_intermediate, x->dACT, w.down, H, lastrows, x->ws, pk_use(x, B, PK_DOWN, w.pk_down));
             break;
         }
         attention_prefill(s, 256, a);
@@ -984,7 +1014,8 @@
             HIPCHK(hipMemcpy2DAsync(lastrows, (size_t)H * 2, Hs + (size_t)(L - 1) * H, (size_t)L * H * 2,
                                     (size_t)H * 2, B, hipMemcpyDeviceToDevice, s));
         int nparts = 0;
-        gemv_logits(s, B, lastrows, fnorm, eps, E, c.t_vocab, logits, x->pmax, x->pidx, &nparts);
+        gemv_logits(s, B, lastrows, fnorm, eps, E, c.t_vocab, logits, x->pmax, x->pidx, &nparts, nullptr, nullptr,
+                    nullptr, nullptr, 1, pk_use(x, B, PK_LM_HEAD, x->w.pk_embed));
     }
     LAUNCHCHK();
     return 0;
@@ -1036,13 +1067,14 @@
                           i + 1 < c.t_layers ? x->w.t[i + 1].in_norm : nullptr, eps, x->dHn, w.mf_down);
             continue;
         }
-        gemv_geglu(s, B, x->dH, w.post_norm, eps, w.gate_up, c.t_intermediate, x->dACT);
-        gemv_res(s, B, c.t_intermediate, x->dACT, w.down, H, x->dH, x->ws);
+        gemv_geglu(s, B, x->dH, w.post_norm, eps, w.gate_up, c.t_intermediate, x->dACT, nullptr, nullptr,
+                   pk_use(x, B, PK_GATE_UP, w.pk_gate_up));
+        gemv_res(s, B, c.t_intermediate, x->dACT, w.down, H, x->dH, x->ws, pk_use(x, B, PK_DOWN, w.pk_down));
     }
     int nparts = 0;
     int64_t* nx = next_ids ? next_ids : x->d_next;
     if (!gemv_logits(s, B, x->dH, x->w.final_norm, eps, E, c.t_vocab, logits, x->pmax, x->pidx, &nparts, x->lm_done, nx,
-                     st, hist, adv_n))
+                     st, hist, adv_n, pk_use(x, B, PK_LM_HEAD, x->w.pk_embed)))
         argmax_finish(s, B, x->pmax, x->pidx, nparts, nx, st, hist, adv_n);
     return launcher_error();
 }
@@ -1110,8 +1142,10 @@
         void* p = nullptr;
         if (hipMalloc(&p, per * c.t_layers * sizeof(uint16_t)) != hipSuccess) {
             (void)hipGetLastError();
+            x->mfw_alloc_failed = true;
             return 0;
         }
+        x->mfw_alloc_failed = false;
         x->allocs.push_back(p);
         x->mfw = reinterpret_cast<uint16_t*>(p);
         x->dgraphs.clear();
@@ -1126,6 +1160,188 @@
         w.mf_gate_up = gu; w.mf_qkv = qkv; w.mf_o = o; w.mf_down = down;
     }
     LAUNCHCHK();
+    return 0;
+}
+
+static void drop_small_batch_graphs(GraphCache& g) {
+    for (auto it = g.map.begin(); it != g.map.end();) {
+        if (!it->first.empty() && it->first[0] <= 2) {
+            if (it->second) (void)hipGraphExecDestroy(it->second);
+            it = g.map.erase(it);
+        } else {
+            ++it;
+        }
+    }
+}
+
+static int ensure_pk_image(pgmi_ctx* x, hipStream_t s, int B) {
+    const int want = pk_mask_for(x, B) & ~x->pk_done;
+    if (!want) return 0;
+    const pgmi_config& c = x->c;
+    if (c.t_hidden != 2048 || c.t_intermediate != 16384) {
+        x->pk_done |= want;
+        return 0;
+    }
+    hipStreamCaptureStatus cap = hipStreamCaptureStatusNone;
+    if (hipStreamIsCapturing(s, &cap) != hipSuccess || cap != hipStreamCaptureStatusNone) {
+        (void)hipGetLastError();
+        return 0;
+    }
+    const int L = c.t_layers;
+    const int64_t I = c.t_intermediate, H = c.t_hidden, V = c.t_vocab;
+    struct Cand { int kind; const uint16_t* W; int64_t rows, K; PkW* dst; uint8_t* out; };
+    std::vector<Cand> cands;
+    const int64_t gu_b = pk_image_bytes(2 * I, H), dn_b = pk_image_bytes(H, I), em_b = pk_image_bytes(V, H);
+    const int64_t kind_bytes[3] = {gu_b * L, dn_b * L, em_b};
+    int got = 0;
+    for (int k = 0; k < 3; ++k) {
+        if (!(want & (1 << k)) || kind_bytes[k] == 0) continue;
+        if (!x->pk_buf[k]) {
+            void* p = nullptr;
+            if (hipMalloc(&p, (size_t)kind_bytes[k]) != hipSuccess) {
+                (void)hipGetLastError();
+                x->pk_alloc_failed = true;
+                continue;
+            }
+            x->allocs.push_back(p);
+            x->pk_buf[k] = reinterpret_cast<uint8_t*>(p);
+        }
+        got |= 1 << k;
+    }
+    for (int i = 0; i < L; ++i) {
+        TextLayerW& w = x->w.t[i];
+        if (got & PK_GATE_UP) cands.push_back({PK_GATE_UP, w.gate_up, 2 * I, H, &w.pk_gate_up, x->pk_buf[0] + gu_b * i});
+        if (got & PK_DOWN) cands.push_back({PK_DOWN, w.down, H, I, &w.pk_down, x->pk_buf[1] + dn_b * i});
+    }
+    if (got & PK_LM_HEAD) cands.push_back({PK_LM_HEAD, x->w.embed, V, H, &x->w.pk_embed, x->pk_buf[2]});
+    if (!cands.empty()) {
+        const size_t n = cands.size(), cap_n = (size_t)2 * L + 1;
+        if (!x->pk_stat) {
+            void* p = nullptr;
+            HIPCHK(hipMalloc(&p, cap_n * 2 * sizeof(unsigned)));
+            x->allocs.push_back(p);
+            x->pk_stat = reinterpret_cast<unsigned*>(p);
+        }
+        std::vector<unsigned> st(2 * n);
+        for (size_t t = 0; t < n; ++t) { st[2 * t] = 0; st[2 * t + 1] = 0xFFFFFFFFu; }
+        HIPCHK(hipMemcpyAsync(x->pk_stat, st.data(), st.size() * sizeof(unsigned), hipMemcpyHostToDevice, s));
+        HIPCHK(hipStreamSynchronize(s));
+        for (size_t t = 0; t < n; ++t) pk_scan(s, cands[t].W, (long)(cands[t].rows * cands[t].K), x->pk_stat + 2 * t);
+        LAUNCHCHK();
+        HIPCHK(hipMemcpyAsync(st.data(), x->pk_stat, st.size() * sizeof(unsigned), hipMemcpyDeviceToHost, s));
+        HIPCHK(hipStreamSynchronize(s));
+        for (size_t t = 0; t < n; ++t) {
+            const int e_hi = (int)st[2 * t], e_lo = st[2 * t + 1] > 255u ? 256 : (int)st[2 * t + 1];
+            if (!pk_fits(e_hi, e_lo)) {
+                *cands[t].dst = PkW{};
+                continue;
+            }
+            pk_pack(s, cands[t].W, (long)cands[t].rows, (int)cands[t].K, e_hi, cands[t].out);
+            cands[t].dst->img = cands[t].out;
+            cands[t].dst->base2 = pk_base2(e_hi);
+        }
+        LAUNCHCHK();
+    }
+    x->pk_done |= want;
+    drop_small_batch_graphs(x->dgraphs);
+    return 0;
+}
+
+int pgmi_set_decode_packed(pgmi_ctx* x, int on) {
+    if (!x) return fail(PGMI_E_ARG, "null context");
+    if (on > PK_ALL) return fail(PGMI_E_ARG, "decode_packed: 0 off, 1..7 a mask of kinds (1 gate|up, 2 down, 4 lm_head), < 0 default");
+    x->pk_mask = on < 0 ? -1 : on;
+    drop_small_batch_graphs(x->dgraphs);
+    x->pgraphs.clear();
+    return 0;
+}
+
+int pgmi_decode_packed_info(const pgmi_ctx* x, int64_t* info, int n) {
+    if (!x || !info) return fail(PGMI_E_ARG, "null argument");
+    if (n < PGMI_PACKED_INFO_N) return fail(PGMI_E_ARG, "info needs PGMI_PACKED_INFO_N entries");
+    const pgmi_config& c = x->c;
+    const int64_t I = c.t_intermediate, H = c.t_hidden, V = c.t_vocab;
+    const bool shapes = H == 2048 && I == 16384;
+    int64_t np = 0, nr = 0, bp = 0, br = 0;
+    auto count = [&](int kind, const PkW& w, int64_t rows, int64_t K) {
+        if ((pk_mask_for(x, 1) & x->pk_done & kind) && w.img && shapes) { ++np; bp += pk_image_bytes(rows, K); }
+        else { ++nr; br += rows * K * 2; }
+    };
+    for (size_t i = 0; i < x->w.t.size(); ++i) {
+        count(PK_GATE_UP, x->w.t[i].pk_gate_up, 2 * I, H);
+        count(PK_DOWN, x->w.t[i].pk_down, H, I);
+    }
+    count(PK_LM_HEAD, x->w.pk_embed, V, H);
+    info[0] = pk_mask_for(x, 1); info[8] = pk_mask_for(x, 2); info[1] = np; info[2] = nr; info[3] = bp; info[4] = br;
+    info[5] = x->pk_alloc_failed; info[6] = x->mfw_alloc_failed; info[7] = x->pk_done;
+    return 0;
+}
+
+int pgmi_decode_packed_tensor(const pgmi_ctx* x, int kind, int layer) {
+    if (!x) return fail(PGMI_E_ARG, "null context");
+    if (kind != PK_GATE_UP && kind != PK_DOWN && kind != PK_LM_HEAD) return fail(PGMI_E_ARG, "kind: 1 gate|up, 2 down, 4 lm_head");
+    if (kind != PK_LM_HEAD && (layer < 0 || layer >= (int)x->w.t.size())) return fail(PGMI_E_ARG, "layer out of range");
+    const PkW& w = kind == PK_LM_HEAD ? x->w.pk_embed : kind == PK_GATE_UP ? x->w.t[layer].pk_gate_up : x->w.t[layer].pk_down;
+    return (pk_mask_for(x, 1) & x->pk_done & kind) && w.img ? 1 : 0;
+}
+
+int pgmi_pack13_scan(const uint16_t* w, int64_t n, int* e_hi, int* fits) {
+    if (!w || !e_hi || !fits) return fail(PGMI_E_ARG, "null argument");
+    if (n < 1) return fail(PGMI_E_ARG, "pack13: no values");
+    int hi = 0, lo = 256;
+    for (int64_t i = 0; i < n; ++i) {
+        const int ex = (w[i] >> 7) & 0xFF;
+        hi = std::max(hi, ex);
+        if (ex) lo = std::min(lo, ex);
+    }
+    *e_hi = hi;
+    *fits = pk_fits(hi, lo) ? 1 : 0;
+    return 0;
+}
+
+int64_t pgmi_pack13_bytes(int64_t rows, int64_t K) {
+    if (rows < 1 || K < kPkSegK || K % kPkSegK != 0) return -1;
+    return pk_image_bytes(rows, K);
+}
+
+static const uint8_t* pk_host_seg(const uint8_t* image, int64_t seg) { return image + seg * kPkSegBytes; }
+
+int pgmi_pack13_encode(const uint16_t* w, int64_t rows, int64_t K, int e_hi, uint8_t* image) {
+    if (!w || !image) return fail(PGMI_E_ARG, "null argument");
+    if (pgmi_pack13_bytes(rows, K) < 0) return fail(PGMI_E_ARG, "pack13: K must be a positive multiple of 2048, rows >= 1");
+    if (e_hi < 0 || e_hi > 255) return fail(PGMI_E_ARG, "pack13: e_hi is an exponent field (0..255)");
+    for (int64_t seg = 0; seg < rows * (K / kPkSegK); ++seg)
+        for (int l = 0; l < 64; ++l) {
+            uint4 f[4];
+            for (int ch = 0; ch < 4; ++ch) std::memcpy(&f[ch], w + seg * kPkSegK + 512 * ch + 8 * l, 16);
+            const PkSeg sg = pk_encode(f, e_hi);
+            uint8_t* d = image + seg * kPkSegBytes;
+            std::memcpy(d + pk_off_a(l), &sg.a, 16);
+            std::memcpy(d + pk_off_b(l), &sg.b, 16);
+            std::memcpy(d + pk_off_n(l), &sg.n, 16);
+            std::memcpy(d + pk_off_h(l), &sg.h, 4);
+        }
+    return 0;
+}
+
+int pgmi_pack13_decode(const uint8_t* image, int64_t rows, int64_t K, int e_hi, uint16_t* w) {
+    if (!w || !image) return fail(PGMI_E_ARG, "null argument");
+    if (pgmi_pack13_bytes(rows, K) < 0) return fail(PGMI_E_ARG, "pack13: K must be a positive multiple of 2048, rows >= 1");
+    if (e_hi < 0 || e_hi > 255) return fail(PGMI_E_ARG, "pack13: e_hi is an exponent field (0..255)");
+    const unsigned b2 = pk_base2(e_hi);
+    for (int64_t seg = 0; seg < rows * (K / kPkSegK); ++seg)
+        for (int l = 0; l < 64; ++l) {
+            const uint8_t* d = pk_host_seg(image, seg);
+            PkSeg sg;
+            std::memcpy(&sg.a, d + pk_off_a(l), 16);
+            std::memcpy(&sg.b, d + pk_off_b(l), 16);
+            std::memcpy(&sg.n, d + pk_off_n(l), 16);
+            std::memcpy(&sg.h, d + pk_off_h(l), 4);
+            for (int ch = 0; ch < 4; ++ch) {
+                const uint4 f = pk_chunk(sg, ch, b2);
+                std::memcpy(w + seg * kPkSegK + 512 * ch + 8 * l, &f, 16);
+            }
+        }
     return 0;
 }
 
@@ -1154,6 +1370,7 @@
     if ((!ids && !embeds) || !kv || !logits) return fail(PGMI_E_ARG, "null argument");
     hipStream_t s = (hipStream_t)stream;
     if (B >= gemv_mf_min_batch() && (rc = ensure_mf_image(x, s))) return rc;
+    if (B < gemv_mf_min_batch() && (rc = ensure_pk_image(x, s, B))) return rc;
     int masked = 0;
     if (dev) {
         set_step_dev(s, x->step, kv_len, dev->pos, dev->pos_dtype);
@@ -1439,20 +1656,44 @@
     hipStream_t s = (hipStream_t)stream;
     const float eps = c.t_rms_eps;
     const int H = c.t_hidden;
+    if (which >= 2 && B < gemv_mf_min_batch() && (rc = ensure_pk_image(x, s, B))) return rc;
     const TextLayerW& w = x->w.t[layer];
     switch (which) {
         case 1: gemv_res(s, B, c.t_heads * c.t_head_dim, x->dAO, w.o, H, x->dH, x->ws); break;
-        case 2: gemv_geglu(s, B, x->dH, w.post_norm, eps, w.gate_up, c.t_intermediate, x->dACT); break;
-        case 3: gemv_res(s, B, c.t_intermediate, x->dACT, w.down, H, x->dH, x->ws); break;
+        case 2:
+            gemv_geglu(s, B, x->dH, w.post_norm, eps, w.gate_up, c.t_intermediate, x->dACT, nullptr, nullptr,
+                       pk_use(x, B, PK_GATE_UP, w.pk_gate_up));
+            break;
+        case 3:
+            gemv_res(s, B, c.t_intermediate, x->dACT, w.down, H, x->dH, x->ws, pk_use(x, B, PK_DOWN, w.pk_down));
+            break;
         case 4: {
             int nparts = 0;
             gemv_logits(s, B, x->dH, x->w.final_norm, eps, x->w.embed, c.t_vocab, x->dlogits, x->pmax, x->pidx,
-                        &nparts);
+                        &nparts, nullptr, nullptr, nullptr, nullptr, 1, pk_use(x, B, PK_LM_HEAD, x->w.pk_embed));
             break;
         }
         default: return fail(PGMI_E_ARG, "unknown kernel id");
     }
     LAUNCHCHK();
+    return 0;
+}
+
+int pgmi_debug_decode_buffer(pgmi_ctx* x, int which, void* buf, int64_t bytes, int write, void* stream) {
+    int rc;
+    if (!x || !buf) return fail(PGMI_E_ARG, "null argument");
+    if ((rc = ensure_prepared(x))) return rc;
+    const pgmi_config& c = x->c;
+    void* p;
+    int64_t cap;
+    switch (which) {
+        case 0: p = x->dH; cap = (int64_t)c.max_batch * c.t_hidden * 2; break;
+        case 1: p = x->dACT; cap = (int64_t)c.max_batch * c.t_intermediate * 2; break;
+        case 2: p = x->dlogits; cap = (int64_t)c.max_batch * c.t_vocab * 4; break;
+        default: return fail(PGMI_E_ARG, "decode buffer: 0 h, 1 act, 2 logits");
+    }
+    if (bytes < 1 || bytes > cap) return fail(PGMI_E_ARG, "decode buffer: byte count outside the buffer");
+    HIPCHK(hipMemcpyAsync(write ? p : buf, write ? buf : p, (size_t)bytes, hipMemcpyDeviceToDevice, (hipStream_t)stream));
     return 0;
 }
 
diff --git a/multimodal-financial-analysis-tool-using-paligemma_amd/csrc/gemv_body.h b/multimodal-financial-analysis-tool-using-paligemma_amd/csrc/gemv_body.h
--- a/multimodal-financial-analysis-tool-using-paligemma_amd/csrc/gemv_body.h
+++ b/multimodal-financial-analysis-tool-using-paligemma_amd/csrc/gemv_body.h
@@ -4,6 +4,7 @@
 #include "coh.h"
 #include "common.h"
 #include "launch.h"
+#include "pack13.h"
 
 namespace pgmi {
 
@@ -47,10 +48,15 @@
     uint16_t* emb_out;
     float* ssq;
     const uint16_t* Wf;
+    const uint8_t* Wp;
+    unsigned pk_base2;
 };
 
-template <int B, int KCH, int RPW, int MODE, int WK, bool XREG, int DEPTH = 1, bool EMB = false, bool RG = false>
+template <int B, int KCH, int RPW, int MODE, int WK, bool XREG, int DEPTH = 1, bool EMB = false, bool RG = false,
+          bool PK = false>
 __device__ __forceinline__ void gemv_block(const GemvArgs& a, const int blk, const int nblk, uint16_t* xs) {
+    static_assert(!PK || ((MODE == GV_GEGLU || MODE == GV_RES || MODE == GV_LOGITS) && (KCH / WK) % 4 == 0 && DEPTH == 1),
+                  "13-bit image: the streaming modes, whole 2048-weight segments per wave");
     static_assert(!EMB || (MODE == GV_QKV && XREG && WK == 1), "embedding fold: register-held q|k|v input only");
     static_assert(!RG || MODE == GV_QKV || MODE == GV_ORES, "per-row step records: q|k|v and o_proj only");
     constexpr int NR = (MODE == GV_QKV || MODE == GV_GEGLU) ? 2 : 1;
@@ -79,7 +85,9 @@
         else return (long)u;
     };
 
-    uint4 w[DEPTH][NL];
+    constexpr int NSEG = PK ? KCW / 4 : 1;
+    uint4 w[PK ? 1 : DEPTH][PK ? 1 : NL];
+    PkSeg wp[PK ? RPW * NR * NSEG : 1];
     auto issue = [&](auto slot, int base) {
         constexpr int SL = decltype(slot)::value;
 #pragma unroll
@@ -88,10 +96,23 @@
             if (u >= bend) u = bend - 1;
 #pragma unroll
             for (int j = 0; j < NR; ++j) {
-                const uint16_t* rp = a.W + row_of(u, j) * K + kofs;
-#pragma unroll
-                for (int c = 0; c < KCW; ++c)
-                    w[SL][(i * NR + j) * KCW + c] = kSmallTemporal ? ldg16(rp + 512 * c) : ldg_nt(rp + 512 * c);
+                if constexpr (PK) {
+                    const uint8_t* sp = a.Wp + (row_of(u, j) * (KCH / 4) + wk * NSEG) * (long)kPkSegBytes;
+#pragma unroll
+                    for (int g = 0; g < NSEG; ++g) {
+                        PkSeg& d = wp[(i * NR + j) * NSEG + g];
+                        const uint8_t* q = sp + g * kPkSegBytes;
+                        d.a = ldg_nt(q + pk_off_a(lane));
+                        d.b = ldg_nt(q + pk_off_b(lane));
+                        d.n = ldg_nt(q + pk_off_n(lane));
+                        d.h = __builtin_nontemporal_load(reinterpret_cast<const unsigned*>(q + pk_off_h(lane)));
+                    }
+                } else {
+                    const uint16_t* rp = a.W + row_of(u, j) * K + kofs;
+#pragma unroll
+                    for (int c = 0; c < KCW; ++c)
+                        w[SL][(i * NR + j) * KCW + c] = kSmallTemporal ? ldg16(rp + 512 * c) : ldg_nt(rp + 512 * c);
+                }
             }
         }
     };
@@ -326,6 +347,11 @@
                 for (int b = 0; b < B; ++b) acc[i][j][b] = 0.f;
 #pragma unroll
         for (int c = 0; c < KCW; ++c) {
+            uint4 wc[PK ? RPW * NR : 1];
+            if constexpr (PK) {
+#pragma unroll
+                for (int r = 0; r < RPW * NR; ++r) wc[r] = pk_chunk(wp[r * NSEG + c / 4], c % 4, a.pk_base2);
+            }
 #pragma unroll
             for (int b = 0; b < B; ++b) {
                 uint4 xv;
@@ -334,7 +360,10 @@
 #pragma unroll
                 for (int i = 0; i < RPW; ++i)
 #pragma unroll
-                    for (int j = 0; j < NR; ++j) acc[i][j][b] = dot8(w[SL][(i * NR + j) * KCW + c], xv, acc[i][j][b]);
+                    for (int j = 0; j < NR; ++j) {
+                        if constexpr (PK) acc[i][j][b] = dot8(wc[i * NR + j], xv, acc[i][j][b]);
+                        else acc[i][j][b] = dot8(w[SL][(i * NR + j) * KCW + c], xv, acc[i][j][b]);
+                    }
             }
         }
         const int cur = ub;
@@ -519,10 +548,11 @@
     }
 }
 
-template <int B, int KCH, int RPW, int MODE, int WK, bool XREG, int DEPTH, bool EMB = false, bool RG = false>
+template <int B, int KCH, int RPW, int MODE, int WK, bool XREG, int DEPTH, bool EMB = false, bool RG = false,
+          bool PK = false>
 __global__ void __launch_bounds__(256) k_gemv(GemvArgs a) {
     extern __shared__ __attribute__((aligned(16))) uint16_t xs[];
-    gemv_block<B, KCH, RPW, MODE, WK, XREG, DEPTH, EMB, RG>(a, blockIdx.x, gridDim.x, xs);
+    gemv_block<B, KCH, RPW, MODE, WK, XREG, DEPTH, EMB, RG, PK>(a, blockIdx.x, gridDim.x, xs);
 }
 
 }
diff --git a/multimodal-financial-analysis-tool-using-paligemma_amd/csrc/kernels_gemv.hip b/multimodal-financial-analysis-tool-using-paligemma_amd/csrc/kernels_gemv.hip
--- a/multimodal-financial-analysis-tool-using-paligemma_amd/csrc/kernels_gemv.hip
+++ b/multimodal-financial-analysis-tool-using-paligemma_amd/csrc/kernels_gemv.hip
@@ -28,13 +28,13 @@
     return e;
 }
 
-template <int B, int KCH, int RPW, int MODE, int WK = 1, int DEPTH = 1, bool EMB = false, bool RG = false>
+template <int B, int KCH, int RPW, int MODE, int WK = 1, int DEPTH = 1, bool EMB = false, bool RG = false, bool PK = false>
 static void launch_gemv(hipStream_t s, const GemvArgs& a, int max_blocks = 0) {
     constexpr bool XREG = (MODE != GV_ORES) && B * (KCH / WK) <= 8;
     size_t lds = XREG ? 0 : (size_t)B * KCH * 512 * sizeof(uint16_t);
     static size_t attr = 0;
     if (lds > attr) {
-        const hipError_t e = hipFuncSetAttribute(reinterpret_cast<const void*>(&k_gemv<B, KCH, RPW, MODE, WK, XREG, DEPTH, EMB, RG>),
+        const hipError_t e = hipFuncSetAttribute(reinterpret_cast<const void*>(&k_gemv<B, KCH, RPW, MODE, WK, XREG, DEPTH, EMB, RG, PK>),
                                                  hipFuncAttributeMaxDynamicSharedMemorySize, (int)lds);
         if (e != hipSuccess) {
             launch_error_set(e, "k_gemv: dynamic LDS size");
@@ -45,7 +45,13 @@
     constexpr int per_block = (4 / WK) * RPW;
     int blocks = (a.n_units + per_block - 1) / per_block;
     if (max_blocks > 0 && blocks > max_blocks) blocks = max_blocks;
-    hipLaunchKernelGGL((k_gemv<B, KCH, RPW, MODE, WK, XREG, DEPTH, EMB, RG>), dim3(blocks), dim3(256), lds, s, a);
+    hipLaunchKernelGGL((k_gemv<B, KCH, RPW, MODE, WK, XREG, DEPTH, EMB, RG, PK>), dim3(blocks), dim3(256), lds, s, a);
+}
+
+template <int B, int KCH, int RPW, int MODE, int WK = 1>
+static void launch_gemv_pk(hipStream_t s, const GemvArgs& a, int max_blocks = 0) {
+    if (a.Wp) launch_gemv<B, KCH, RPW, MODE, WK, 1, false, false, true>(s, a, max_blocks);
+    else launch_gemv<B, KCH, RPW, MODE, WK>(s, a, max_blocks);
 }
 
 bool gemv_qkv_folds_embed(int B) { return B <= 2 && B < gemv_mf_min_batch(); }
@@ -78,7 +84,7 @@
 }
 
 void gemv_res(hipStream_t s, int B, int K, const uint16_t* x, const uint16_t* W, int N, uint16_t* h_inout,
-              float* ws) {
+              float* ws, PkW pk) {
     GemvArgs a{};
     a.x = x; a.norm_w = nullptr; a.W = W; a.n_units = N; a.K = K; a.nb = B; a.out = h_inout;
     if (B >= gemv_mf_min_batch() && K % 128 == 0 && ws) {
@@ -102,8 +108,9 @@
             const int nb = (B - b0) < 4 ? (B - b0) : 4;
             GemvArgs c = a;
             c.x = x + (long)b0 * K; c.out = h_inout + (long)b0 * N; c.nb = nb;
-            if (nb <= 1) launch_gemv<1, 32, 1, GV_RES, 4>(s, c, 512);
-            else if (nb <= 2) launch_gemv<2, 32, 2, GV_RES, 4>(s, c);
+            if (B <= 2 && K == 16384) { c.Wp = pk.img; c.pk_base2 = pk.base2; }
+            if (nb <= 1) launch_gemv_pk<1, 32, 1, GV_RES, 4>(s, c, 512);
+            else if (nb <= 2) launch_gemv_pk<2, 32, 2, GV_RES, 4>(s, c);
             else launch_gemv<4, 32, 2, GV_RES, 4>(s, c);
         }
     }
@@ -144,7 +151,7 @@
 }
 
 void gemv_geglu(hipStream_t s, int B, const uint16_t* h, const uint16_t* norm_w, float eps, const uint16_t* Wgu,
-                int I, uint16_t* act, float* ssq, const uint16_t* Wf) {
+                int I, uint16_t* act, float* ssq, const uint16_t* Wf, PkW pk) {
     GemvArgs a{};
     a.x = h; a.norm_w = norm_w; a.eps = eps; a.W = Wgu; a.n_units = I; a.K = 2048; a.nb = B; a.I = I; a.out = act;
     if (B >= gemv_mf_min_batch()) {
@@ -153,8 +160,9 @@
         gemv_mf_geglu(s, a);
         return;
     }
-    if (B <= 1) launch_gemv<1, 4, 1, GV_GEGLU>(s, a, 1024);
-    else L_(2, 4, 2, GV_GEGLU);
+    a.Wp = pk.img; a.pk_base2 = pk.base2;
+    if (B <= 1) launch_gemv_pk<1, 4, 1, GV_GEGLU>(s, a, 1024);
+    else launch_gemv_pk<2, 4, 2, GV_GEGLU>(s, a);
 }
 
 int gemv_logits_blocks() { return 2048; }
@@ -163,7 +171,7 @@
 
 bool gemv_logits(hipStream_t s, int B, const uint16_t* h, const uint16_t* norm_w, float eps, const uint16_t* E,
                  int V, float* logits, float* pmax, int* pidx, int* nparts, unsigned* done, int64_t* next,
-                 StepState* adv, int64_t* hist, int adv_n) {
+                 StepState* adv, int64_t* hist, int adv_n, PkW pk) {
     GemvArgs a{};
     a.x = h; a.norm_w = norm_w; a.eps = eps; a.W = E; a.n_units = V; a.K = 2048; a.nb = B; a.logits = logits;
     a.pmax = pmax; a.pidx = pidx;
@@ -173,6 +181,7 @@
         *nparts = gemv_mf_logits(s, a, mb);
         return false;
     }
+    a.Wp = pk.img; a.pk_base2 = pk.base2;
     const bool fold = done && next && gemv_logits_folds(B);
     if (fold) {
         a.done = done;
@@ -185,7 +194,7 @@
     do {                                                                \
         blocks = (V + 4 * rpw - 1) / (4 * rpw);                         \
         if (blocks > mb) blocks = mb;                                   \
-        launch_gemv<b_, 4, rpw, GV_LOGITS>(s, a, mb);                   \
+        launch_gemv_pk<b_, 4, rpw, GV_LOGITS>(s, a, mb);                \
     } while (0)
     if (B <= 1) LG_(1, 4);
     else LG_(2, 4);
diff --git a/multimodal-financial-analysis-tool-using-paligemma_amd/csrc/kernels_pack.hip b/multimodal-financial-analysis-tool-using-paligemma_amd/csrc/kernels_pack.hip
--- /dev/null
+++ b/multimodal-financial-analysis-tool-using-paligemma_amd/csrc/kernels_pack.hip
@@ -0,0 +1,60 @@
+#include "launch.h"
+#include "pack13.h"
+
+namespace pgmi {
+
+__global__ void __launch_bounds__(256) k_pk_scan(const uint16_t* __restrict__ W, long n16, unsigned* __restrict__ stat) {
+    unsigned hi = 0, lo = 0xFFFFFFFFu;
+    for (long i = (long)blockIdx.x * blockDim.x + threadIdx.x; i < n16; i += (long)gridDim.x * blockDim.x) {
+        const uint4 v = ldg16(W + i * 8);
+        const uint16_t* e = reinterpret_cast<const uint16_t*>(&v);
+#pragma unroll
+        for (int j = 0; j < 8; ++j) {
+            const unsigned ex = (e[j] >> 7) & 0xFFu;
+            hi = ex > hi ? ex : hi;
+            if (ex) lo = ex < lo ? ex : lo;
+        }
+    }
+#pragma unroll
+    for (int o = 32; o > 0; o >>= 1) {
+        const unsigned h2 = __shfl_xor(hi, o, 64), l2 = __shfl_xor(lo, o, 64);
+        hi = h2 > hi ? h2 : hi;
+        lo = l2 < lo ? l2 : lo;
+    }
+    if ((threadIdx.x & 63) == 0) {
+        atomicMax(stat, hi);
+        atomicMin(stat + 1, lo);
+    }
+}
+
+__global__ void __launch_bounds__(256) k_pk_pack(const uint16_t* __restrict__ W, long n_items, int e_hi,
+                                                 uint8_t* __restrict__ out) {
+    const long t = (long)blockIdx.x * blockDim.x + threadIdx.x;
+    if (t >= n_items) return;
+    const int l = (int)(t & 63);
+    const long seg = t >> 6;
+    const uint16_t* src = W + seg * kPkSegK + 8 * l;
+    uint4 f[4];
+#pragma unroll
+    for (int c = 0; c < 4; ++c) f[c] = ldg16(src + 512 * c);
+    const PkSeg s = pk_encode(f, e_hi);
+    uint8_t* dst = out + seg * kPkSegBytes;
+    *reinterpret_cast<uint4*>(dst + pk_off_a(l)) = s.a;
+    *reinterpret_cast<uint4*>(dst + pk_off_b(l)) = s.b;
+    *reinterpret_cast<uint4*>(dst + pk_off_n(l)) = s.n;
+    *reinterpret_cast<unsigned*>(dst + pk_off_h(l)) = s.h;
+}
+
+void pk_scan(hipStream_t s, const uint16_t* W, long numel, unsigned* stat) {
+    const long n16 = numel / 8;
+    long blocks = (n16 + 255) / 256;
+    if (blocks > 2048) blocks = 2048;
+    hipLaunchKernelGGL(k_pk_scan, dim3((unsigned)blocks), dim3(256), 0, s, W, n16, stat);
+}
+
+void pk_pack(hipStream_t s, const uint16_t* W, long rows, int K, int e_hi, uint8_t* out) {
+    const long n = rows * (K / kPkSegK) * 64;
+    hipLaunchKernelGGL(k_pk_pack, dim3((unsigned)((n + 255) / 256)), dim3(256), 0, s, W, n, e_hi, out);
+}
+
+}
diff --git a/multimodal-financial-analysis-tool-using-paligemma_amd/csrc/launch.h b/multimodal-financial-analysis-tool-using-paligemma_amd/csrc/launch.h
--- a/multimodal-financial-analysis-tool-using-paligemma_amd/csrc/launch.h
+++ b/multimodal-financial-analysis-tool-using-paligemma_amd/csrc/launch.h
@@ -81,8 +81,14 @@
               uint16_t* q_out, uint16_t* kc, uint16_t* vc, long kv_b_stride, float* ws = nullptr,
               const EmbedFold* emb = nullptr, const uint16_t* Wf = nullptr,
               int st_stride = 0);
+struct PkW {
+    const uint8_t* img = nullptr;
+    unsigned base2 = 0;
+};
+void pk_scan(hipStream_t s, const uint16_t* W, long numel, unsigned* stat);
+void pk_pack(hipStream_t s, const uint16_t* W, long rows, int K, int e_hi, uint8_t* out);
 void gemv_res(hipStream_t s, int B, int K, const uint16_t* x, const uint16_t* W, int N, uint16_t* h_inout,
-              float* ws);
+              float* ws, PkW pk = {});
 void gemv_res_norm(hipStream_t s, int B, int K, const uint16_t* x, const uint16_t* W, int N, uint16_t* h_inout,
                    float* ws, const uint16_t* norm_w, float eps, uint16_t* hn, const uint16_t* Wf = nullptr);
 void mf_swizzle(hipStream_t s, const uint16_t* W, int rows, int K, uint16_t* out, bool qkv = false);
@@ -91,13 +97,14 @@
                  const uint16_t* Wo, int N, uint16_t* h_inout, uint16_t* o_out, float* ssq = nullptr,
                  const uint16_t* Wf = nullptr, int st_stride = 0);
 void gemv_geglu(hipStream_t s, int B, const uint16_t* h, const uint16_t* norm_w, float eps,
-                const uint16_t* Wgu, int I, uint16_t* act, float* ssq = nullptr, const uint16_t* Wf = nullptr);
+                const uint16_t* Wgu, int I, uint16_t* act, float* ssq = nullptr, const uint16_t* Wf = nullptr,
+                PkW pk = {});
 int gemv_logits_blocks();
 int gemv_mf_min_batch();
 bool gemv_logits(hipStream_t s, int B, const uint16_t* h, const uint16_t* norm_w, float eps,
                  const uint16_t* E, int V, float* logits, float* pmax, int* pidx, int* nparts,
                  unsigned* done = nullptr, int64_t* next = nullptr, StepState* adv = nullptr,
-                 int64_t* hist = nullptr, int adv_n = 1);
+                 int64_t* hist = nullptr, int adv_n = 1, PkW pk = {});
 void argmax_finish(hipStream_t s, int B, const float* pmax, const int* pidx, int nparts, int64_t* out,
                    StepState* adv = nullptr, int64_t* hist = nullptr, int adv_n = 1);
 int argmax_scratch_parts();
diff --git a/multimodal-financial-analysis-tool-using-paligemma_amd/csrc/pack13.h b/multimodal-financial-analysis-tool-using-paligemma_amd/csrc/pack13.h
--- /dev/null
+++ b/multimodal-financial-analysis-tool-using-paligemma_amd/csrc/pack13.h
@@ -0,0 +1,83 @@
+#pragma once
+#include "common.h"
+
+namespace pgmi {
+
+#define PK_HD __host__ __device__ __forceinline__
+
+constexpr int kPkSegK = 2048;
+constexpr int kPkSegBytes = 3328;
+constexpr unsigned kPkExpMask = 0x7F807F80u;
+
+struct PkSeg {
+    uint4 a, b, n;
+    unsigned h;
+};
+
+typedef unsigned short pk_u16x2 __attribute__((ext_vector_type(2)));
+
+PK_HD unsigned pk_base2(int e_hi) {
+    const unsigned b = (unsigned)(e_hi - 31) & 0xFFFFu;
+    return b | (b << 16);
+}
+
+PK_HD bool pk_fits(int e_hi, int e_lo_nonzero) {
+    return e_lo_nonzero > 255 || e_lo_nonzero >= e_hi - 30;
+}
+
+PK_HD unsigned pk_shl(unsigned v, int s) { return s >= 0 ? v << (s & 31) : v >> ((-s) & 31); }
+
+PK_HD unsigned pk_word(const uint4& v, int i) { return i == 0 ? v.x : i == 1 ? v.y : i == 2 ? v.z : v.w; }
+
+PK_HD unsigned pk_spread(unsigned S, int odd) {
+#if defined(__HIP_DEVICE_COMPILE__)
+    return __builtin_amdgcn_perm(S, S, odd ? 0x03030202u : 0x01010000u);
+#else
+    const unsigned lo = (S >> (odd ? 16 : 0)) & 0xFFu, hi = (S >> (odd ? 24 : 8)) & 0xFFu;
+    return lo | (lo << 8) | (hi << 16) | (hi << 24);
+#endif
+}
+
+PK_HD unsigned pk_pair(const PkSeg& s, int c, int p, unsigned base2) {
+    const unsigned G = pk_spread(pk_word(c < 2 ? s.a : s.b, (c & 1) * 2 + (p >> 1)), p & 1);
+    const unsigned n = pk_shl(pk_word(s.n, c), 7 - 4 * p) & 0x07800780u;
+    const unsigned u7 = (pk_shl(s.h, 11 - 4 * c - p) & 0x08000800u) | n;
+    const pk_u16x2 u = __builtin_bit_cast(pk_u16x2, u7);
+    const pk_u16x2 one = __builtin_elementwise_min(u, (pk_u16x2)(0x80));
+    const pk_u16x2 e = one * __builtin_bit_cast(pk_u16x2, base2) + u;
+    return (__builtin_bit_cast(unsigned, e) & kPkExpMask) | (G & ~kPkExpMask);
+}
+
+PK_HD uint4 pk_chunk(const PkSeg& s, int c, unsigned base2) {
+    return make_uint4(pk_pair(s, c, 0, base2), pk_pair(s, c, 1, base2), pk_pair(s, c, 2, base2),
+                      pk_pair(s, c, 3, base2));
+}
+
+PK_HD PkSeg pk_encode(const uint4 (&f)[4], int e_hi) {
+    unsigned sm[8] = {0, 0, 0, 0, 0, 0, 0, 0}, nib[4] = {0, 0, 0, 0}, h = 0;
+    for (int c = 0; c < 4; ++c)
+        for (int j = 0; j < 8; ++j) {
+            const unsigned w = (pk_word(f[c], j >> 1) >> (16 * (j & 1))) & 0xFFFFu;
+            const unsigned ex = (w >> 7) & 0xFFu;
+            const unsigned u = ex ? (unsigned)((int)ex - (e_hi - 31)) & 31u : 0u;
+            sm[c * 2 + (j >> 2)] |= (((w >> 8) & 0x80u) | (w & 0x7Fu)) << (8 * (j & 3));
+            const int p = j >> 1, odd = j & 1;
+            nib[c] |= (u & 15u) << (16 * odd + 4 * p);
+            h |= (u >> 4) << (16 * odd + 4 * c + p);
+        }
+    PkSeg s;
+    s.a = make_uint4(sm[0], sm[1], sm[2], sm[3]);
+    s.b = make_uint4(sm[4], sm[5], sm[6], sm[7]);
+    s.n = make_uint4(nib[0], nib[1], nib[2], nib[3]);
+    s.h = h;
+    return s;
+}
+
+PK_HD int pk_off_a(int l) { return 16 * l; }
+PK_HD int pk_off_b(int l) { return 1024 + 16 * l; }
+PK_HD int pk_off_n(int l) { return 2048 + 16 * l; }
+PK_HD int pk_off_h(int l) { return 3072 + 4 * l; }
+
+inline int64_t pk_image_bytes(int64_t rows, int64_t K) { return rows * (K / kPkSegK) * kPkSegBytes; }
+
+}
diff --git a/multimodal-financial-analysis-tool-using-paligemma_amd/pgmi/_native.py b/multimodal-financial-analysis-tool-using-paligemma_amd/pgmi/_native.py
--- a/multimodal-financial-analysis-tool-using-paligemma_amd/pgmi/_native.py
+++ b/multimodal-financial-analysis-tool-using-paligemma_amd/pgmi/_native.py
@@ -65,6 +65,13 @@
     "pgmi_set_prefill_graph": (i32, [vp, i32]),
     "pgmi_graph_count": (i32, [vp, i32]),
     "pgmi_set_decode_staged_norm": (i32, [vp, i32]),
+    "pgmi_set_decode_packed": (i32, [vp, i32]),
+    "pgmi_decode_packed_info": (i32, [vp, ctypes.POINTER(i64), i32]),
+    "pgmi_decode_packed_tensor": (i32, [vp, i32, i32]),
+    "pgmi_pack13_scan": (i32, [vp, i64, ctypes.POINTER(i32), ctypes.POINTER(i32)]),
+    "pgmi_pack13_bytes": (i64, [i64, i64]),
+    "pgmi_pack13_encode": (i32, [vp, i64, i64, i32, vp]),
+    "pgmi_pack13_decode": (i32, [vp, i64, i64, i32, vp]),
     "pgmi_prefill_kernel": (i32, [vp, i32, i32, i32, vp]),
     "pgmi_debug_gemm_tiles": (i32, [i32, i32, i32, i32, i32, i32, vp, vp, vp]),
     "pgmi_debug_gemm_plan": (i32, [i32, i32, i32, i32, vp, vp, vp, vp]),
@@ -83,6 +90,7 @@
     "pgmi_broadcast_weights": (i32, [vp, vp, i32, vp]),
     "pgmi_eos_update": (i32, [vp, vp, vp, i32, i64, i64, vp, vp]),
     "pgmi_decode_kernel": (i32, [vp, i32, i32, i32, vp]),
+    "pgmi_debug_decode_buffer": (i32, [vp, i32, vp, i64, i32, vp]),
     "pgmi_tune_gemm": (i32, [i32, i32]),
     "pgmi_tune_gemm_shape": (i32, [i32, i32, i32, i32, i32, i32]),
     "pgmi_tune_attention": (i32, [i32]),
@@ -115,7 +123,12 @@
             raise NativeError(f"{LIB_PATH} not built: run `make -C csrc` or __graft_entry__.build()")
         L = ctypes.CDLL(LIB_PATH)
         for name, (res, args) in SIGNATURES.items():
-            fn = getattr(L, name)
+            try:
+                fn = getattr(L, name)
+            except AttributeError:
+                if os.environ.get("PGMI_LIB_PATH"):
+                    continue
+                raise
             fn.restype = res
             fn.argtypes = args
         _lib = L
diff --git a/multimodal-financial-analysis-tool-using-paligemma_amd/pgmi/engine.py b/multimodal-financial-analysis-tool-using-paligemma_amd/pgmi/engine.py
--- a/multimodal-financial-analysis-tool-using-paligemma_amd/pgmi/engine.py
+++ b/multimodal-financial-analysis-tool-using-paligemma_amd/pgmi/engine.py
@@ -448,6 +448,33 @@
 
     def set_decode_staged_norm(self, on: int) -> None:
         N.check(self.lib.pgmi_set_decode_staged_norm(self.ctx, int(on)), "pgmi_set_decode_staged_norm")
+
+    def set_decode_packed(self, on: int) -> None:
+        N.check(self.lib.pgmi_set_decode_packed(self.ctx, int(on)), "pgmi_set_decode_packed")
+
+    def decode_packed_info(self) -> dict:
+        v = (ctypes.c_int64 * 9)()
+        N.check(self.lib.pgmi_decode_packed_info(self.ctx, v, 9), "pgmi_decode_packed_info")
+        return {"mask": v[0], "mask_b2": v[8], "packed": v[1], "raw": v[2], "packed_bytes": v[3], "raw_bytes": v[4],
+                "alloc_failed": bool(v[5]), "mf_alloc_failed": bool(v[6]), "scanned": v[7]}
+
+    def decode_packed_tensor(self, kind: int, layer: int = 0) -> bool:
+        rc = self.lib.pgmi_decode_packed_tensor(self.ctx, int(kind), int(layer))
+        if rc < 0:
+            N.check(rc, "pgmi_decode_packed_tensor")
+        return rc == 1
+
+    def decode_kernel(self, which: int, layer: int, B: int) -> None:
+        self._ready()
+        N.check(self.lib.pgmi_decode_kernel(self.ctx, int(which), int(layer), int(B), self._s()), "pgmi_decode_kernel")
+
+    def decode_buffer(self, which: int, t: torch.Tensor, write: bool = False) -> torch.Tensor:
+        self._ready()
+        if t.device != self.device or not t.is_contiguous():
+            raise ValueError("decode_buffer: a contiguous tensor on the engine's device")
+        N.check(self.lib.pgmi_debug_decode_buffer(self.ctx, int(which), t.data_ptr(), t.numel() * t.element_size(),
+                                                  int(bool(write)), self._s()), "pgmi_debug_decode_buffer")
+        return t
 
     def argmax(self, logits: torch.Tensor) -> torch.Tensor:
         l2 = logits.reshape(-1, logits.shape[-1]).contiguous()
diff --git a/multimodal-financial-analysis-tool-using-paligemma_amd/pgmi/packed.py b/multimodal-financial-analysis-tool-using-paligemma_amd/pgmi/packed.py
--- /dev/null
+++ b/multimodal-financial-analysis-tool-using-paligemma_amd/pgmi/packed.py
@@ -0,0 +1,41 @@
+from __future__ import annotations
+
+import numpy as np
+
+KINDS = {"gate_up": 1, "down": 2, "lm_head": 4}
+ALL_KINDS = 7
+SEG_WEIGHTS, SEG_BYTES = 2048, 3328
+
+
+def exponent_fields(bits: np.ndarray) -> np.ndarray:
+    return (np.asarray(bits, np.uint16).astype(np.int32) >> 7) & 0xFF
+
+
+def e_hi_np(bits: np.ndarray) -> int:
+    return int(exponent_fields(bits).max())
+
+
+def fits_np(bits: np.ndarray) -> bool:
+    e = exponent_fields(bits)
+    hi = int(e.max())
+    return not bool(((e >= 1) & (e <= hi - 31)).any())
+
+
+def pack_np(bits: np.ndarray, e_hi: int):
+    b = np.asarray(bits, np.uint16).astype(np.int32)
+    e = (b >> 7) & 0xFF
+    code = np.where(e == 0, 31, e_hi - e)
+    if ((code < 0) | (code > 31) | ((e != 0) & (code == 31))).any():
+        raise ValueError("tensor does not fit the 5-bit exponent code")
+    sm = ((b >> 8) & 0x80) | (b & 0x7F)
+    return sm.astype(np.uint8), code.astype(np.uint8)
+
+
+def unpack_np(sm: np.ndarray, code: np.ndarray, e_hi: int) -> np.ndarray:
+    s, c = sm.astype(np.int32), code.astype(np.int32)
+    e = np.where(c == 31, 0, e_hi - c)
+    return (((s & 0x80) << 8) | (e << 7) | (s & 0x7F)).astype(np.uint16)
+
+
+def image_bytes(rows: int, K: int) -> int:
+    return rows * (K // SEG_WEIGHTS) * SEG_BYTES
```

Measured after the change: 862.3 tokens/s (median of 6 runs). +7.0%, better.
